# KarypisLab/SLIM

Hardware: AMD Instinct MI355X
Metric: item-columns solved/sec (whole node) (higher is better)
Workload: dtype f32

## Files before the change

slim_amd/csrc/cd_gramr.hpp:

```cpp
#pragma once
#include <utility>

#include "cd_tile.hpp"
#include "gram_pack.hpp"

#ifndef SLIM_GRAMR_AUX
#define SLIM_GRAMR_AUX 0
#endif
#ifndef SLIM_GRAMR_PROF
#define SLIM_GRAMR_PROF 0
#endif
#ifndef SLIM_GRAMR_FROM_PLANES
#define SLIM_GRAMR_FROM_PLANES 1
#endif
#ifndef SLIM_GRAMR_PREFETCH
#define SLIM_GRAMR_PREFETCH 0
#endif
#ifndef SLIM_GRAMR_LATE_GATHERS
#define SLIM_GRAMR_LATE_GATHERS 1
#endif
#ifndef SLIM_GRAMR_DRAIN
#define SLIM_GRAMR_DRAIN 0
#endif
#ifndef SLIM_GRAMR_SYNCROW
#define SLIM_GRAMR_SYNCROW 0
#endif

namespace slimamd {

typedef float gramr_v16 __attribute__((ext_vector_type(16)));

template <int N>
struct GramrRegs {
  gramr_v16 v;
  GramrRegs<N - 1> rest;
};
template <>
struct GramrRegs<0> {};
template <int I, int N>
__device__ __forceinline__ gramr_v16& gramr_reg(GramrRegs<N>& r) {
  if constexpr (I == 0) return r.v;
  else return gramr_reg<I - 1>(r.rest);
}
template <class F, int... Is>
__device__ __forceinline__ void static_for_impl(F&& f, std::integer_sequence<int, Is...>) {
  (f(std::integral_constant<int, Is>{}), ...);
}
template <int N, class F>
__device__ __forceinline__ void static_for(F&& f) {
  static_for_impl(f, std::make_integer_sequence<int, N>{});
}

template <int N, int KRA>
__device__ __forceinline__ float gramr_sel_from(GramrRegs<KRA>& gr, const int k, const int e) {
  if (k == N) {
    const gramr_v16 t = gramr_reg<N>(gr);
    asm volatile("" ::"v"(t));
    return t[e];
  }
  if constexpr (N + 1 < KRA) return gramr_sel_from<N + 1, KRA>(gr, k, e);
  return 0.0f;
}
template <int KRA>
__device__ __forceinline__ float gramr_sel(GramrRegs<KRA>& gr, const int k, const int e) {
  return gramr_sel_from<0, KRA>(gr, k, e);
}

#ifndef SLIM_GRAMR_ASMEXPORT
#define SLIM_GRAMR_ASMEXPORT 1
#endif
#define SLIM_GRAMR_EXPORT_ASM                                   \
  "s_mov_b32 %[sm0], m0\n\t"                                   \
  "s_mov_b64 %[sx], exec\n"                                     \
  "1:\n\t"                                                      \
  "s_ff1_i32_b64 %[sb], %[mine]\n\t"                            \
  "v_readlane_b32 %[sr], %[r], %[sb]\n\t"                       \
  "s_bitset0_b64 %[mine], %[sb]\n\t"                            \
  "s_bfe_u32 %[sl], %[sr], 0x60004\n\t"                         \
  "s_lshr_b32 %[sidx], %[sr], 13\n\t"                           \
  "s_and_b32 %[sr], %[sr], 15\n\t"                              \
  "s_lshl4_add_u32 %[sidx], %[sidx], %[sr]\n\t"                 \
  "s_set_gpr_idx_on %[sidx], gpr_idx(SRC0)\n\t"                 \
  "v_mov_b32 %[vt], v16\n\t"                                    \
  "s_set_gpr_idx_off\n\t"                                       \
  "v_readlane_b32 %[sv], %[vt], %[sl]\n\t"                      \
  "s_lshl_b64 exec, 1, %[sb]\n\t"                               \
  "v_mov_b32 %[res], %[sv]\n\t"                                 \
  "s_mov_b64 exec, %[sx]\n\t"                                   \
  "s_cmp_lg_u64 %[mine], 0\n\t"                                 \
  "s_cbranch_scc1 1b\n\t"                                       \
  "s_mov_b32 m0, %[sm0]\n"
#define SLIM_GRAMR_EXPORT_OUT                                                                           \
  [res] "+v"(res), [mine] "+s"(mine), [sb] "=&s"(sb), [sr] "=&s"(sr), [sl] "=&s"(sl), [sidx] "=&s"(sidx), \
      [sv] "=&s"(sv), [vt] "=&v"(vt), [sm0] "=&s"(sm0), [sx] "=&s"(sx)
template <int KRA>
__device__ __forceinline__ float gramr_export(GramrRegs<KRA>& gr, const int r, uint64_t mine) {
  float res = 0.0f, vt;
  int sb, sr, sl, sidx, sm0;
  float sv;
  uint64_t sx;
  static_assert(KRA == 1 || KRA == 3 || KRA == 6 || KRA == 10, "one operand list per instantiation");
  if constexpr (KRA == 1) {
    asm volatile(SLIM_GRAMR_EXPORT_ASM : SLIM_GRAMR_EXPORT_OUT : [r] "v"(r), "{v[16:31]}"(gramr_reg<0>(gr)) : "scc");
  } else if constexpr (KRA == 3) {
    asm volatile(SLIM_GRAMR_EXPORT_ASM
                 : SLIM_GRAMR_EXPORT_OUT
                 : [r] "v"(r), "{v[16:31]}"(gramr_reg<0>(gr)), "{v[32:47]}"(gramr_reg<1>(gr)),
                   "{v[48:63]}"(gramr_reg<2>(gr))
                 : "scc");
  } else if constexpr (KRA == 6) {
    asm volatile(SLIM_GRAMR_EXPORT_ASM
                 : SLIM_GRAMR_EXPORT_OUT
                 : [r] "v"(r), "{v[16:31]}"(gramr_reg<0>(gr)), "{v[32:47]}"(gramr_reg<1>(gr)),
                   "{v[48:63]}"(gramr_reg<2>(gr)), "{v[64:79]}"(gramr_reg<3>(gr)), "{v[80:95]}"(gramr_reg<4>(gr)),
                   "{v[96:111]}"(gramr_reg<5>(gr))
                 : "scc");
  } else {
    asm volatile(SLIM_GRAMR_EXPORT_ASM
                 : SLIM_GRAMR_EXPORT_OUT
                 : [r] "v"(r), "{v[16:31]}"(gramr_reg<0>(gr)), "{v[32:47]}"(gramr_reg<1>(gr)),
                   "{v[48:63]}"(gramr_reg<2>(gr)), "{v[64:79]}"(gramr_reg<3>(gr)), "{v[80:95]}"(gramr_reg<4>(gr)),
                   "{v[96:111]}"(gramr_reg<5>(gr)), "{v[112:127]}"(gramr_reg<6>(gr)),
                   "{v[128:143]}"(gramr_reg<7>(gr)), "{v[144:159]}"(gramr_reg<8>(gr)),
                   "{v[160:175]}"(gramr_reg<9>(gr))
                 : "scc");
  }
  return res;
}

constexpr int gramr_ring_bytes(int ah) { return (kGramrNT / 64) * (ah + 2) * 1024; }
constexpr int kGramrHdr = 1280;
constexpr int kGramrDump = SLIM_GRAMR_PREFETCH ? 256 : 0;
constexpr int gramr_hdr_bytes() { return (kGramrNT / 64) * (2 * kGramrHdr + kGramrDump); }

template <int KR, int KL, bool DMA = false, int WPS = ((KR <= 2 && KL == 0) ? 4 : 2), int AH = 2>
__global__ __launch_bounds__(kGramrNT, WPS) void cd_gramr_kernel(
    const DevMatrix A, const SolveArgs S, const GramPacked P) {
  constexpr int NT = kGramrNT, K = KR + KL;
  constexpr int kGramrAhead = AH, kGramrSlots = AH + 2;
  constexpr int KRA = KR > 0 ? KR : 1;
  constexpr int R0 = KR * kPackGroup;
  static_assert(KR <= 12, "register select covers 12 groups");
  static_assert(KR + KL <= 16, "one base byte per group in a 16-byte load");
  extern __shared__ __attribute__((aligned(16))) float g_lds[];
  __shared__ float s_gB[2][64];
  __shared__ int s_p, s_na;
  __shared__ unsigned long long s_D;
  __shared__ double s_e2[64], s_reg[64];
  __shared__ unsigned long long s_off;
  __shared__ int s_nz;

  const int tid = threadIdx.x;
  const int lane = tid & 63;
  const int wave = uni(tid >> 6);
  const int ncols = A.ncols;
#if !SLIM_GRAMR_FROM_PLANES
  const int n4 = S.ncols_pad >> 2;
#endif
  const int nchunks = P.nchunks;
  const float l1 = S.l1, l2 = S.l2;
#if !SLIM_GRAMR_FROM_PLANES
  const float* __restrict__ Gm = S.G;
  const int64_t ld = S.G_ld;
#endif
  float* const x = S.xslab + (int64_t)blockIdx.x * S.x_stride;
#if !SLIM_GRAMR_FROM_PLANES
  float4* const x4 = reinterpret_cast<float4*>(x);
#endif
  float4* const gl4 = reinterpret_cast<float4*>(g_lds);
  const int64_t* __restrict__ colptr = A.colptr;

  GramrRegs<KRA> gr;

  const uint32_t voff0 = 16u * (uint32_t)tid;
  const uint32_t vlast = 16u * (uint32_t)(nchunks - 1);
#if SLIM_GRAMR_DRAIN
#define SLIM_VMCNT(n) __builtin_amdgcn_s_waitcnt(0 | (7 << 4) | (15 << 8))
#else
#define SLIM_VMCNT(n) __builtin_amdgcn_s_waitcnt(((n) & 15) | (((n) >> 4) << 14) | (7 << 4) | (15 << 8))
#endif
  char* const ring_w = reinterpret_cast<char*>(g_lds) + KL * kPackGroup * 4 + wave * (kGramrSlots * 1024);
#if SLIM_GRAMR_PROF
  unsigned long long pt_first_v = 0, pt_mark_v = 0, pt_export_v = 0, pt_mark = 0;
  unsigned long long* const pt_first_p = &pt_first_v;
  unsigned long long* const pt_mark_p = &pt_mark_v;
#endif
  char* const hdr_w = reinterpret_cast<char*>(g_lds) + KL * kPackGroup * 4 + (DMA ? gramr_ring_bytes(AH) : 0) +
                      wave * (2 * kGramrHdr + kGramrDump);
  char* const dump_w = hdr_w + 2 * kGramrHdr;
  auto apply = [&](const uint8_t* __restrict__ plo, const uint8_t* __restrict__ phi,
                   const uint8_t* __restrict__ ph2, const uint8_t* __restrict__ pbase, const int hk,
                   const int h2k, const int cdiag, const int ediag, const float vdiag,
                   const float nd, const int rg, uint32_t (&gq)[4],
                   const uint8_t* __restrict__ plo_next) __attribute__((always_inline)) {
    const bool gin1 = rg < hk * kPackGroup, gin2 = rg < h2k * kPackGroup;
    auto gathers = [&]() __attribute__((always_inline)) {
      gq[0] = __hip_atomic_load(plo + rg, __ATOMIC_RELAXED, __HIP_MEMORY_SCOPE_WAVEFRONT);
      gq[1] = __hip_atomic_load(phi + (gin1 ? rg : 0), __ATOMIC_RELAXED, __HIP_MEMORY_SCOPE_WAVEFRONT);
      gq[2] = __hip_atomic_load(ph2 + (gin2 ? rg : 0), __ATOMIC_RELAXED, __HIP_MEMORY_SCOPE_WAVEFRONT);
      gq[3] = __hip_atomic_load(pbase + (((rg >> 4) & (NT - 1)) * 16 + (rg >> 13)), __ATOMIC_RELAXED,
                                __HIP_MEMORY_SCOPE_WAVEFRONT);
    };
    if constexpr (!(DMA && SLIM_GRAMR_LATE_GATHERS)) gathers();
    const int kdiag = cdiag / NT, tdiag = cdiag % NT;
    uint32_t bwords[4];
    if constexpr (DMA) {
      uint32_t vzb = voff0;
      asm volatile("" : "+v"(vzb));
      __builtin_amdgcn_global_load_lds(pbase + vzb, ring_w + (kGramrAhead + 1) * 1024, 16, 0, 0);
    } else {
      const uint4 bw = ld_off<uint4>(pbase, voff0);
      bwords[0] = bw.x;
      bwords[1] = bw.y;
      bwords[2] = bw.z;
      bwords[3] = bw.w;
    }
    auto consume = [&](auto kc, const uint4 lo, auto&& hi_of) __attribute__((always_inline)) {
      constexpr int k = decltype(kc)::value;
      float f[16];
      unpack16(lo, f);
      {
        typedef float gramr_v2 __attribute__((ext_vector_type(2)));
        const float bf = 16.0f * (float)((bwords[(k >> 2) & 3] >> (8 * (k & 3))) & 255u);
#pragma unroll
        for (int e = 0; e < 16; e += 2) {
          gramr_v2 v = {f[e], f[e + 1]};
          asm volatile("" : "+v"(v));
          v += (gramr_v2)(bf);
          f[e] = v.x;
          f[e + 1] = v.y;
        }
      }
      if (k < hk) {
        unpack16_add(hi_of(), 256.0f, f);
        if (k < h2k) {
          uint32_t vz = voff0;
          asm volatile("" : "+v"(vz));
          const uint32_t vo = min(vz + (uint32_t)(kPackGroup * k), vlast);
          unpack16_add(ld_off<uint4>(ph2, vo), 65536.0f, f);
        }
      }
      if (k == kdiag && tid == tdiag) {
#pragma unroll
        for (int e = 0; e < 16; ++e) f[e] = e == ediag ? vdiag : f[e];
      }
      if constexpr (k < KR) {
        gramr_v16& g = gramr_reg<k>(gr);
#pragma unroll
        for (int e = 0; e < 16; ++e) g[e] = fmaf(nd, f[e], g[e]);
        asm volatile("" : "+v"(g));
      } else {
        float4* const gp = gl4 + (k - KR) * 4 * NT + tid;
#pragma unroll
        for (int j = 0; j < 4; ++j) {
          float4 v = gp[j * NT];
          v.x = fmaf(nd, f[4 * j + 0], v.x);
          v.y = fmaf(nd, f[4 * j + 1], v.y);
          v.z = fmaf(nd, f[4 * j + 2], v.z);
          v.w = fmaf(nd, f[4 * j + 3], v.w);
          gp[j * NT] = v;
        }
      }
    };
    if constexpr (DMA) {
      constexpr int S = kGramrAhead + 1;
      uint4 h01[2];
      static_for<2>([&](auto kc) __attribute__((always_inline)) {
        constexpr int k = decltype(kc)::value;
        if constexpr (k < K) {
          if (k < hk) h01[k] = ld_off<uint4>(phi, min(voff0 + (uint32_t)(kPackGroup * k), vlast));
        }
      });
      auto request = [&](auto kc) __attribute__((always_inline)) {
        constexpr int k = decltype(kc)::value;
        uint32_t vz = voff0;
        asm volatile("" : "+v"(vz));
        const uint32_t vo = min(vz + (uint32_t)(kPackGroup * k), vlast);
        __builtin_amdgcn_global_load_lds(plo + vo, ring_w + (k % S) * 1024, 16, 0, SLIM_GRAMR_AUX);
      };
      static_for<(kGramrAhead < K ? kGramrAhead : K)>([&](auto kc) __attribute__((always_inline)) { request(kc); });
      constexpr int kLate = (SLIM_GRAMR_LATE_GATHERS ? 4 : 0) + (SLIM_GRAMR_PREFETCH ? 1 : 0);
      if constexpr (SLIM_GRAMR_LATE_GATHERS) gathers();
      if constexpr (SLIM_GRAMR_PREFETCH) {
        const int ln = lane < 8 * kGramrAhead ? lane : 0;
        const uint32_t po = min((uint32_t)(kPackGroup * (ln >> 3)) + 1024u * (uint32_t)wave + 128u * (uint32_t)(ln & 7), vlast);
        __builtin_amdgcn_global_load_lds(plo_next + po, dump_w, 4, 0, 0);
      }
      static_for<K>([&](auto kc) __attribute__((always_inline)) {
        constexpr int k = decltype(kc)::value;
        if constexpr (k + kGramrAhead < K) request(std::integral_constant<int, k + kGramrAhead>{});
        constexpr int ahead = (K - 1 - k) < kGramrAhead ? (K - 1 - k) : kGramrAhead;
        SLIM_VMCNT(ahead + (k < kGramrAhead ? kLate : 0));
        asm volatile("" ::: "memory");
        if constexpr (k == 0) {
          const uint4 bw = *reinterpret_cast<const uint4*>(ring_w + (kGramrAhead + 1) * 1024 + lane * 16);
          bwords[0] = bw.x;
          bwords[1] = bw.y;
          bwords[2] = bw.z;
          bwords[3] = bw.w;
        }
#if SLIM_GRAMR_PROF
        if constexpr (k == 0) *pt_first_p += __builtin_readcyclecounter() - *pt_mark_p;
#endif
        const uint4 lo = *reinterpret_cast<const uint4*>(ring_w + (k % S) * 1024 + lane * 16);
        consume(kc, lo, [&]() __attribute__((always_inline)) -> uint4 {
          if constexpr (k < 2) return h01[k];
          else {
            uint32_t vz = voff0;
            asm volatile("" : "+v"(vz));
            return ld_off<uint4>(phi, min(vz + (uint32_t)(kPackGroup * k), vlast));
          }
        });
        __builtin_amdgcn_sched_barrier(0);
      });
    } else {
      constexpr int GRP = 4;
      static_for<(K + GRP - 1) / GRP>([&](auto k0c) __attribute__((always_inline)) {
        constexpr int k0 = decltype(k0c)::value * GRP;
        uint4 l[GRP], h[GRP];
        static_for<GRP>([&](auto uc) __attribute__((always_inline)) {
          constexpr int u = decltype(uc)::value, k = k0 + u;
          if constexpr (k < K) {
            const uint32_t vo = min(voff0 + (uint32_t)(kPackGroup * k), vlast);
            l[u] = ld_off<uint4>(plo, vo);
            if (k < hk) h[u] = ld_off<uint4>(phi, vo);
          }
        });
        __builtin_amdgcn_sched_barrier(0);
        static_for<GRP>([&](auto uc) __attribute__((always_inline)) {
          constexpr int u = decltype(uc)::value, k = k0 + u;
          if constexpr (k < K)
            consume(std::integral_constant<int, k>{}, l[u], [&]() __attribute__((always_inline)) -> uint4 { return h[u]; });
          __builtin_amdgcn_sched_barrier(0);
        });
      });
    }
  };
#undef SLIM_VMCNT
  int nrows_read = 0, nhi16_read = 0;
  auto lds_index = [&](const int r) __attribute__((always_inline)) -> int {
    const int rr = r - R0;
    const int kk = rr >> 13, t = (rr >> 4) & (NT - 1), e = rr & 15;
    return ((kk * 4 + (e >> 2)) * NT + t) * 4 + (e & 3);
  };

  int gb_par = 0;
  auto fetch_g = [&](const bool want, const int r) __attribute__((always_inline)) -> float {
    float* const gb = s_gB[gb_par];
    gb_par ^= 1;
    const bool in_lds = r >= R0;
    const bool my_wave = (((r >> 4) & (NT - 1)) >> 6) == wave;
    if (KR > 0) {
      uint64_t mine = __ballot(want && !in_lds && my_wave);
#if SLIM_GRAMR_ASMEXPORT
      if (mine) {
        const bool own = want && !in_lds && my_wave;
        const float res = gramr_export<KRA>(gr, r, mine);
        if (own) gb[lane] = res;
      }
#else
      while (mine) {
        const int b = __builtin_ctzll(mine);
        mine &= mine - 1ull;
        const int rb = lane_bcast(r, b);
        const float v = gramr_sel<KRA>(gr, rb >> 13, rb & 15);
        if (lane == ((rb >> 4) & 63)) gb[b] = v;
      }
#endif
    }
    if (KL > 0 && want && in_lds && my_wave) gb[lane] = g_lds[lds_index(r)];
#if SLIM_GRAMR_PROF
    pt_export_v += __builtin_readcyclecounter() - pt_mark;
#endif
    asm volatile("" ::: "memory");
    __builtin_amdgcn_s_waitcnt(15 | (7 << 4) | (0 << 8) | (3 << 14));
    __builtin_amdgcn_s_barrier();
    asm volatile("" ::: "memory");
    return gb[lane];
  };

  for (;;) {
    if (tid == 0) {
      s_p = atomicAdd(S.queue, 1);
      s_na = 0;
      s_D = 0;
    }
    __syncthreads();
    const int p = s_p;
    if (p >= S.nwork) break;
    const int item = uni(S.order[p]);
    const int grp = p >> 5;
    const uint32_t gkey = (uint32_t)(grp * S.shard_count + S.shard_index);
    const int* __restrict__ ul = S.ulist + (int64_t)grp * S.u_stride;
    const int nunion = uni(S.tile_nunion[grp]);
#if SLIM_GRAMR_FROM_PLANES
    uint4 irec;
    {
      const uint4 mr = P.meta[item];
      irec = make_uint4(uni(mr.x), uni(mr.y), uni(mr.z), uni(mr.w));
    }
#endif
#if !SLIM_GRAMR_FROM_PLANES
    const float* __restrict__ arow = Gm + (int64_t)item * ld;
#endif

#if SLIM_GRAMR_FROM_PLANES
    {
      const int hk0 = (int)((irec.x >> 17) & 15u), h2k0 = (int)((irec.x >> 21) & 15u);
      const uint8_t* __restrict__ plo0 = P.lo + (int64_t)item * P.ldb;
      const uint8_t* __restrict__ phi0 = P.hi + (int64_t)irec.y * kPackGroup;
      const uint8_t* __restrict__ ph20 = phi0 + (int64_t)hk0 * kPackGroup;
      const uint8_t* __restrict__ pb0 = P.base + (int64_t)item * kPackGroup;
      int na = 0;
      int64_t dact = 0;
      for (int c = tid; c < nchunks; c += NT) {
        const int kg = c / NT;
        float f[16];
        unpack16(*reinterpret_cast<const uint4*>(plo0 + 16 * (int64_t)c), f);
        const float bf = 16.0f * (float)pb0[(c & (NT - 1)) * 16 + kg];
#pragma unroll
        for (int e = 0; e < 16; ++e) f[e] += bf;
        if (kg < hk0) unpack16_add(*reinterpret_cast<const uint4*>(phi0 + 16 * (int64_t)c), 256.0f, f);
        if (kg < h2k0) unpack16_add(*reinterpret_cast<const uint4*>(ph20 + 16 * (int64_t)c), 65536.0f, f);
        const int4* __restrict__ io = reinterpret_cast<const int4*>(P.item_of + 16 * (int64_t)c);
#pragma unroll
        for (int j = 0; j < 4; ++j) {
          const int4 q = io[j];
          const int it[4] = {q.x, q.y, q.z, q.w};
#pragma unroll
          for (int u = 0; u < 4; ++u) {
            if (it[u] >= 0) {
              const bool act = it[u] != item && f[4 * j + u] > l1;
              x[it[u]] = act ? 0.0f : kInactive;
              if (act) {
                ++na;
                dact += (int64_t)P.meta[it[u]].z;
              }
            }
          }
        }
      }
      na = (int)wave_sum((float)na);
      if (lane == 0 && na) atomicAdd(&s_na, na);
      if (dact) atomicAdd(&s_D, (unsigned long long)dact);
    }
#else
    {
      const float4* __restrict__ a4 = reinterpret_cast<const float4*>(arow);
      int na = 0;
      int64_t dact = 0;
      for (int c = tid; c < n4; c += NT) {
        const float4 a = a4[c];
        const int i0 = c << 2;
        float4 xs;
        const bool a0 = i0 + 0 < ncols && i0 + 0 != item && a.x > l1;
        const bool a1 = i0 + 1 < ncols && i0 + 1 != item && a.y > l1;
        const bool a2 = i0 + 2 < ncols && i0 + 2 != item && a.z > l1;
        const bool a3 = i0 + 3 < ncols && i0 + 3 != item && a.w > l1;
        xs.x = a0 ? 0.0f : kInactive;
        xs.y = a1 ? 0.0f : kInactive;
        xs.z = a2 ? 0.0f : kInactive;
        xs.w = a3 ? 0.0f : kInactive;
        na += (int)a0 + (int)a1 + (int)a2 + (int)a3;
        x4[c] = xs;
        if (a0 | a1 | a2 | a3) {
          const int64_t c0 = colptr[i0], c1 = colptr[i0 + 1];
          const int64_t c2 = i0 + 2 <= ncols ? colptr[i0 + 2] : c1, c3 = i0 + 3 <= ncols ? colptr[i0 + 3] : c2;
          const int64_t c4 = i0 + 4 <= ncols ? colptr[i0 + 4] : c3;
          dact += (a0 ? c1 - c0 : 0) + (a1 ? c2 - c1 : 0) + (a2 ? c3 - c2 : 0) + (a3 ? c4 - c3 : 0);
        }
      }
      na = (int)wave_sum((float)na);
      if (lane == 0 && na) atomicAdd(&s_na, na);
      if (dact) atomicAdd(&s_D, (unsigned long long)dact);
    }
#endif
    int64_t fe = 0, we = 0;
    auto warm_x = [&]() __attribute__((always_inline)) {
      if (S.icolptr != nullptr && item < S.incols) {
        __syncthreads();
        fe = uni(S.icolptr[item]);
        we = uni(S.icolptr[item + 1]);
        for (int64_t e = fe + tid; e < we; e += NT) {
          const int k = S.icolind[e];
          if (k < ncols && tile_active(x[k])) {
            const float v = S.icolval[e];
            x[k] = v < 0.0f ? 0.0f : v;
          }
        }
      }
    };
    warm_x();
    constexpr bool kCarry = K <= kGramrCarryMaxGroups;
    const bool carried = kCarry && S.g_load != nullptr;
    if (carried) {
      const float4* __restrict__ gs = reinterpret_cast<const float4*>(S.g_load + (int64_t)item * S.g_stride);
      static_for<KRA>([&](auto kc) __attribute__((always_inline)) {
        constexpr int k = decltype(kc)::value;
        gramr_v16 v;
#pragma unroll
        for (int j = 0; j < 4; ++j) {
          const float4 q = gs[(k * NT + tid) * 4 + j];
          v[4 * j] = q.x; v[4 * j + 1] = q.y; v[4 * j + 2] = q.z; v[4 * j + 3] = q.w;
        }
        gramr_reg<k>(gr) = v;
      });
#pragma unroll
      for (int k = 0; k < KL; ++k)
#pragma unroll
        for (int j = 0; j < 4; ++j) gl4[(k * 4 + j) * NT + tid] = gs[((KRA + k) * NT + tid) * 4 + j];
    } else {
    static_for<KRA>([&](auto kc) __attribute__((always_inline)) {
      gramr_reg<decltype(kc)::value>(gr) = (gramr_v16)(0.0f);
    });
#pragma unroll
    for (int k = 0; k < KL; ++k)
#pragma unroll
      for (int j = 0; j < 4; ++j) gl4[(k * 4 + j) * NT + tid] = make_float4(0.f, 0.f, 0.f, 0.f);
    }
    __syncthreads();

    int maxit = 0;
    {
      const int64_t cap = 50 * (uni(colptr[item + 1]) - uni(colptr[item]));
      maxit = cap < (int64_t)S.maxniters ? (int)cap : S.maxniters;
    }
    int niters = 0, conv = 0;
    nrows_read = 0;
    nhi16_read = 0;

    if (wave == 0) {
      s_e2[lane] = 0.0;
      s_reg[lane] = 0.0;
    }
    int phase = 0;
    bool init_row = !carried;
    if (carried) fe = we;
    int t = 0, p0 = 0;
    float dlt = 0.0f;
    PermCtx pc = perm_make(1u, 0u);
    int i_a = 0;
    int i_n = 0;
    int hw = 0;
    auto header_a = [&](const int q0) __attribute__((always_inline)) {
      const int pos = q0 + lane;
      i_a = pos < nunion ? ul[perm_index(pc, (uint32_t)pos)] : -1;
    };
    auto header_b = [&]() __attribute__((always_inline)) {
      i_n = i_a < 0 ? 0 : i_a;
      char* const hb = hdr_w + hw * kGramrHdr;
      __builtin_amdgcn_global_load_lds(x + i_n, hb, 4, 0, 0);
      __builtin_amdgcn_global_load_lds(P.meta + i_n, hb + 256, 16, 0, 0);
      hw ^= 1;
    };
    int ib = 0, wpos = 0, nz = 0;
    unsigned long long off = 0;
    bool fits = false;
    unsigned long long Uu = 0;
#if SLIM_GRAMR_PROF
    unsigned long long pt_fetch = 0, pt_dec = 0, pt_apply = 0;
    pt_first_v = 0;
    pt_export_v = 0;
#define SLIM_PT(acc) { const unsigned long long now_ = __builtin_readcyclecounter(); acc += now_ - pt_mark; pt_mark = now_; }
#else
#define SLIM_PT(acc)
#endif

    for (;;) {
      bool want = false;
      int r = 0, i = 0;
      uint4 mrow = make_uint4(0u, 0u, 0u, 0u);
      float xi = kInactive;
      bool part = false, keep = false;
      uint64_t mkeep = 0;
      if (phase == 1) {
        i = i_n;
        __builtin_amdgcn_s_waitcnt(0 | (7 << 4) | (15 << 8));
        asm volatile("" ::: "memory");
        {
          const char* const hcur = hdr_w + (hw ^ 1) * kGramrHdr;
          const bool valid = p0 + lane < nunion;
          int lz = lane;
          asm volatile("" : "+v"(lz));
          const float xv = *reinterpret_cast<const float*>(hcur + lz * 4);
          mrow = *reinterpret_cast<const uint4*>(hcur + 256 + lz * 16);
          r = (int)(mrow.x & 0x1FFFFu);
          xi = valid ? xv : kInactive;
        }
        asm volatile("" ::: "memory");
        part = tile_active(xi);
        header_b();
        header_a(p0 + 128);
        want = part;
      } else if (phase == 2) {
        i = ib + lane;
        xi = i < ncols ? x[i] : kInactive;
        const bool act = tile_active(xi);
        keep = act && fabsf(xi) > kEps;
        if (act && wave == 0)
          s_reg[lane] += 0.5 * (double)l2 * (double)xi * (double)xi + (double)l1 * (double)fabsf(xi);
        mkeep = __ballot(keep);
        if (mkeep == 0) {
          ib += 64;
          if (ib >= ncols) break;
          continue;
        }
        r = keep ? (int)(P.meta[i].x & 0x1FFFFu) : 0;
        want = keep;
      }
#if SLIM_GRAMR_PROF
      pt_mark = __builtin_readcyclecounter();
#endif
      const float g0 = fetch_g(want, r);
      SLIM_PT(pt_fetch)
      float gi = g0;
      uint64_t pend = 0;
      if (phase == 1) {
        pend = __ballot(part);
      }
      for (;;) {
        int row = 0;
        float nd = 0.0f;
        uint4 rec = make_uint4(0u, 0u, 0u, 0u);
        if (phase == 0) {
          bool have = false;
          if (init_row) {
            row = item;
            nd = 1.0f;
            have = true;
          } else {
            while (fe < we) {
              const int kk = uni(S.icolind[fe]);
              ++fe;
              if (kk < ncols) {
                const float xk = uni(x[kk]);
                if (xk > kEps) {
                  row = kk;
                  nd = -xk;
                  have = true;
                  break;
                }
              }
            }
          }
          if (!have) break;
        } else if (phase == 1) {
          if (pend == 0) break;
          const float xeff = (xi > kEps || xi < -kEps) ? xi : 0.0f;
          const float sq = __uint_as_float(mrow.w);
          const float cn = sqrtf(sq);
          const float num = cd_num(gi, xeff, sq);
          const float nx = num > l1 ? (num - l1) / cd_den(cn, l2) : 0.0f;
          const float neff = (nx > kEps || nx < -kEps) ? nx : 0.0f;
          const float d = neff - xeff;
          const uint64_t m = __ballot(part && nx != xi) & pend;
          if (m == 0) break;
          const int f = __builtin_ctzll(m);
          const float d_f = lane_bcast(d, f);
          const float nx_f = lane_bcast(nx, f), xi_f = lane_bcast(xi, f);
          dlt = fmaf(nx_f - xi_f, nx_f - xi_f, dlt);
          row = lane_bcast(i, f);
          if (wave == 0 && lane == f) x[row] = nx;
          pend = f == 63 ? 0ull : (pend & ~((2ull << f) - 1ull));
          if (d_f == 0.0f) continue;
          nd = -d_f;
          rec.x = (uint32_t)lane_bcast((int)mrow.x, f);
          rec.y = (uint32_t)lane_bcast((int)mrow.y, f);
          rec.z = (uint32_t)lane_bcast((int)mrow.z, f);
          rec.w = (uint32_t)lane_bcast((int)mrow.w, f);
          Uu += (unsigned long long)rec.z;
        } else {
          break;
        }
        if (phase == 0) {
          const uint4 mr = P.meta[row];
          rec.x = uni(mr.x);
          rec.y = uni(mr.y);
          rec.z = uni(mr.z);
          rec.w = uni(mr.w);
        }
        const int hk = (int)((rec.x >> 17) & 15u), h2k = (int)((rec.x >> 21) & 15u);
        const uint8_t* __restrict__ plo = P.lo + (int64_t)row * P.ldb;
        const uint8_t* __restrict__ phi = P.hi + (int64_t)rec.y * kPackGroup;
        const uint8_t* __restrict__ ph2 = phi + (int64_t)hk * kPackGroup;
        const uint8_t* __restrict__ pbase = P.base + (int64_t)row * kPackGroup;
        const bool in1 = r < hk * kPackGroup, in2 = r < h2k * kPackGroup;
        uint32_t gq[4];
        const int rdiag = (int)(rec.x & 0x1FFFFu);
        SLIM_PT(pt_dec)
#if SLIM_GRAMR_PROF
        pt_mark_v = pt_mark;
#endif
        const uint8_t* __restrict__ plo_next = plo;
        if (SLIM_GRAMR_PREFETCH && phase == 1) {
          const uint64_t cand = __ballot(part && xi != 0.0f) & pend;
          if (cand) plo_next = P.lo + (int64_t)lane_bcast(i, __builtin_ctzll(cand)) * P.ldb;
        }
        apply(plo, phi, ph2, pbase, hk, h2k, rdiag >> 4, rdiag & 15, __uint_as_float(rec.w), nd, r, gq, plo_next);
        float gsel = (float)gq[0] + 16.0f * (float)gq[3];
        gsel = in1 ? fmaf(256.0f, (float)gq[1], gsel) : gsel;
        gsel = in2 ? fmaf(65536.0f, (float)gq[2], gsel) : gsel;
        if (init_row) {
          init_row = false;
        } else {
          ++nrows_read;
          nhi16_read += min(hk * (kPackGroup / 16), nchunks) + min(h2k * (kPackGroup / 16), nchunks);
        }
        gi = fmaf(nd, gsel, gi);
#if SLIM_GRAMR_SYNCROW
        __syncthreads();
#endif
        SLIM_PT(pt_apply)
      }
      if (phase == 1) {
        p0 += 64;
        if (p0 < nunion) continue;
        if (dlt < S.opt_tol) {
          conv = 1;
          niters = t + 1;
        } else {
          ++t;
        }
      } else if (phase == 2) {
        if (keep) {
#if SLIM_GRAMR_FROM_PLANES
          float aty = 0.0f;
          if (wave == 0) {
            const int hk0 = (int)((irec.x >> 17) & 15u), h2k0 = (int)((irec.x >> 21) & 15u);
            const uint8_t* __restrict__ plo0 = P.lo + (int64_t)item * P.ldb;
            const uint8_t* __restrict__ phi0 = P.hi + (int64_t)irec.y * kPackGroup;
            const uint8_t* __restrict__ ph20 = phi0 + (int64_t)hk0 * kPackGroup;
            const uint8_t* __restrict__ pb0 = P.base + (int64_t)item * kPackGroup;
            const bool j1 = r < hk0 * kPackGroup, j2 = r < h2k0 * kPackGroup;
            aty = (float)plo0[r] + 16.0f * (float)pb0[((r >> 4) & (NT - 1)) * 16 + (r >> 13)];
            if (j1) aty = fmaf(256.0f, (float)phi0[r], aty);
            if (j2) aty = fmaf(65536.0f, (float)ph20[r], aty);
          }
          if (wave == 0) s_e2[lane] += (double)xi * ((double)aty + (double)g0);
#else
          if (wave == 0) s_e2[lane] += (double)xi * ((double)arow[i] + (double)g0);
#endif
          if (fits && wave == 0) {
            const int64_t dst = (int64_t)off + wpos + __popcll(mkeep & ((1ull << lane) - 1ull));
            S.out_ind[dst] = i;
            S.out_val[dst] = xi;
          }
        }
        wpos += __popcll(mkeep);
        ib += 64;
        if (ib >= ncols) break;
        continue;
      }
      bool sweep = false;
      if (!conv) {
        if (t >= maxit) {
          niters = maxit + 1;
        } else if (nunion == 0) {
          conv = 1;
          niters = t + 1;
        } else {
          sweep = true;
        }
      }
      if (sweep) {
        __syncthreads();
        phase = 1;
        p0 = 0;
        dlt = 0.0f;
        pc = perm_make((uint32_t)nunion, perm_key(S.seed, gkey, (uint32_t)t));
        header_a(0);
        header_b();
        header_a(64);
        continue;
      }
      if (wave == 0) {
        int cnt = 0;
        for (int jb = 0; jb < ncols; jb += 64) {
          const int j = jb + lane;
          const float xv = j < ncols ? x[j] : kInactive;
          cnt += __popcll(__ballot(tile_active(xv) && fabsf(xv) > kEps));
        }
        if (lane == 0) {
          s_off = atomicAdd(S.out_cursor, (unsigned long long)cnt);
          s_nz = cnt;
        }
      }
      __syncthreads();
      off = s_off;
      nz = s_nz;
      fits = (int64_t)(off + (unsigned long long)nz) <= S.out_cap;
      phase = 2;
      ib = 0;
      wpos = 0;
      if (ncols <= 0) break;
    }
    if (kCarry && S.g_save != nullptr) {
      float4* __restrict__ gs = reinterpret_cast<float4*>(S.g_save + (int64_t)item * S.g_stride);
      static_for<KRA>([&](auto kc) __attribute__((always_inline)) {
        constexpr int k = decltype(kc)::value;
        const gramr_v16 v = gramr_reg<k>(gr);
#pragma unroll
        for (int j = 0; j < 4; ++j)
          gs[(k * NT + tid) * 4 + j] = make_float4(v[4 * j], v[4 * j + 1], v[4 * j + 2], v[4 * j + 3]);
      });
#pragma unroll
      for (int k = 0; k < KL; ++k)
#pragma unroll
        for (int j = 0; j < 4; ++j) gs[((KRA + k) * NT + tid) * 4 + j] = gl4[(k * 4 + j) * NT + tid];
    }
    if (wave == 0) {
      double e2 = s_e2[lane], reg = s_reg[lane];
      for (int o = 32; o > 0; o >>= 1) {
        e2 += __shfl_xor(e2, o);
        reg += __shfl_xor(reg, o);
      }
      if (lane == 0) {
        const float err = (float)(0.5 * ((double)A.csq[item] - e2));
        if (!fits) atomicMax(S.overflow, 1);
        S.out_cnt[item] = fits ? nz : -nz - 1;
        S.out_off[item] = (int64_t)off;
        S.st_na[item] = s_na;
        S.st_sweeps[item] = niters;
        S.st_conv[item] = conv;
#if SLIM_GRAMR_PROF
        S.st_D[item] = (int64_t)pt_fetch;
        S.st_U[item] = (int64_t)pt_dec;
        S.st_B[item] = (int64_t)pt_apply;
        S.st_G[item] = (int)(pt_first_v >> 8);
        S.st_na[item] = (int)(pt_export_v >> 8);
#else
        S.st_D[item] = (int64_t)s_D * (int64_t)(conv ? niters : maxit);
        S.st_U[item] = (int64_t)Uu;
        S.st_G[item] = nrows_read;
        S.st_B[item] = (int64_t)nrows_read * (P.ldb + 16 * (int64_t)(nchunks < NT ? nchunks : NT)) + (int64_t)nhi16_read * 16 +
                       ((carried ? 4 : 0) + (kCarry && S.g_save != nullptr ? 4 : 0)) * S.g_stride;
#endif
        S.st_err[item] = err;
        S.st_obj[item] = err + (float)reg;
      }
    }
    __syncthreads();
  }
}

constexpr int kGramrUnionNT = 256;
#ifdef SLIM_GRAM_PACK_KERNELS
__global__ __launch_bounds__(kGramrUnionNT) void gramr_union_kernel(const DevMatrix A, const SolveArgs S,
                                                                     const GramPacked P) {
  constexpr int NT = kGramrUnionNT;
  constexpr int kWords = kGramrMaxGroups * kPackGroup / 32;
  __shared__ uint32_t s_bits[kWords];
  __shared__ int s_scan[NT];
  const int tid = threadIdx.x;
  const int grp = blockIdx.x;
  const int base = grp * 32;
  const int nprob = (S.nwork - base) < 32 ? (S.nwork - base) : 32;
  const int ncols = A.ncols;
  const int nwords = (ncols + 31) >> 5;
  const int nchunks = P.nchunks;
  int* __restrict__ ul = S.ulist + (int64_t)grp * S.u_stride;
  for (int w = tid; w < nwords; w += NT) s_bits[w] = 0u;
  __syncthreads();
  for (int q = 0; q < nprob; ++q) {
    const int it0 = uni(S.order[base + q]);
    const uint4 mr = P.meta[it0];
    const uint32_t rx = uni(mr.x), ry = uni(mr.y);
    const int hk = (int)((rx >> 17) & 15u), h2k = (int)((rx >> 21) & 15u);
    const uint8_t* __restrict__ plo = P.lo + (int64_t)it0 * P.ldb;
    const uint8_t* __restrict__ phi = P.hi + (int64_t)ry * kPackGroup;
    const uint8_t* __restrict__ ph2 = phi + (int64_t)hk * kPackGroup;
    const uint8_t* __restrict__ pb = P.base + (int64_t)it0 * kPackGroup;
    for (int c = tid; c < nchunks; c += NT) {
      const int kg = c / kGramrNT;
      float f[16];
      unpack16(*reinterpret_cast<const uint4*>(plo + 16 * (int64_t)c), f);
      const float bf = 16.0f * (float)pb[(c & (kGramrNT - 1)) * 16 + kg];
#pragma unroll
      for (int e = 0; e < 16; ++e) f[e] += bf;
      if (kg < hk) unpack16_add(*reinterpret_cast<const uint4*>(phi + 16 * (int64_t)c), 256.0f, f);
      if (kg < h2k) unpack16_add(*reinterpret_cast<const uint4*>(ph2 + 16 * (int64_t)c), 65536.0f, f);
      const int4* __restrict__ io = reinterpret_cast<const int4*>(P.item_of + 16 * (int64_t)c);
#pragma unroll
      for (int j = 0; j < 4; ++j) {
        const int4 qv = io[j];
        const int it[4] = {qv.x, qv.y, qv.z, qv.w};
#pragma unroll
        for (int u = 0; u < 4; ++u)
          if (it[u] >= 0 && it[u] != it0 && f[4 * j + u] > S.l1) atomicOr(&s_bits[it[u] >> 5], 1u << (it[u] & 31));
      }
    }
  }
  __syncthreads();
  const int W = (nwords + NT - 1) / NT;
  const int w0 = tid * W, w1 = min(nwords, w0 + W);
  int cnt = 0;
  for (int w = w0; w < w1; ++w) cnt += __popc(s_bits[w]);
  s_scan[tid] = cnt;
  __syncthreads();
  for (int o = 1; o < NT; o <<= 1) {
    const int v = tid >= o ? s_scan[tid - o] : 0;
    __syncthreads();
    s_scan[tid] += v;
    __syncthreads();
  }
  int pos = s_scan[tid] - cnt;
  for (int w = w0; w < w1; ++w) {
    uint32_t b = s_bits[w];
    while (b) {
      const int j = __builtin_ctz(b);
      b &= b - 1u;
      ul[pos++] = (w << 5) + j;
    }
  }
  if (tid == NT - 1) S.tile_nunion[grp] = s_scan[tid];
}
#endif

}
```

slim_amd/csrc/cd_wave.hpp:

```cpp
#pragma once
#include <hip/hip_runtime.h>

#include <cstdint>

#include "cd_perm.hpp"

namespace slimamd {

struct DevMatrix {
  int32_t nrows, ncols;
  int64_t nnz;
  const int64_t* rowptr;
  const int32_t* rowind;
  const float* rowval;
  const int64_t* colptr;
  const int32_t* colind;
  const float* colval;
  const float* cnorm;
  const float* csq;
};

struct SolveArgs {
  float l1, l2, opt_tol;
  int32_t maxniters;
  uint32_t seed;
  int32_t nnbrs;
  int32_t simtype;
  const int32_t* order;
  int32_t nwork;
  int32_t* queue;
  const int64_t* icolptr;
  const int32_t* icolind;
  const float* icolval;
  int32_t incols;
  float* slab;
  int64_t slab_stride;
  int32_t nrows_pad, ncols_pad;
  float* xslab;
  int64_t x_stride;
  int32_t* ulist;
  int64_t u_stride;
  int32_t ngroups;
  uint64_t* trace;
  int32_t cluster;
  const int32_t* ubounds;
  const int64_t* csplit;
  unsigned long long* mailbox;
  float* atypart;
  int32_t exact_gram;
  int32_t bm_shift, bm_words;
  int32_t nheavy;
  int32_t cluster_hi;
  const int32_t* ubounds_hi;
  const int64_t* csplit_hi;
  unsigned long long* mailbox_hi;
  int32_t* queue_hi;
  int64_t nnz_last;
  int32_t hi_prefetch;
  int32_t shard_count, shard_index;
  int32_t xcd_swizzle;
  float* gram;
  int32_t gram_mode;
  float* G;
  int64_t G_ld;
  int32_t* tile_nunion;
  const int32_t* gram_pos;
  int32_t gram_bits;
  int32_t gram_split_stride;
  int32_t gram_accum;
  const uint4* gview;
  const int64_t* gview_base;
  const uint16_t* gview_cnt;
  int32_t gview_ngroups;
  int32_t gview_range0;
  int32_t gview_sentinel;
  int32_t gram_part16;
  int32_t gram_store;
  int32_t gram_read;
  float* g_save;
  const float* g_load;
  int64_t g_stride;
  int32_t* out_cnt;
  int64_t* out_off;
  int32_t* out_ind;
  float* out_val;
  unsigned long long* out_cursor;
  int64_t out_cap;
  int32_t* overflow;
  int32_t* st_na;
  int32_t* st_sweeps;
  int32_t* st_conv;
  int64_t* st_G;
  int64_t* st_D;
  int64_t* st_U;
  int64_t* st_B;
  float* st_err;
  float* st_obj;
};

constexpr float kEps = 1e-7f;


__device__ __forceinline__ float cd_num(float g, float xeff, float sq) {
  float p = xeff * sq;
  asm volatile("" : "+v"(p));
  return g + p;
}
__device__ __forceinline__ float cd_den(float cn, float l2) { return fmaf(cn, cn, l2); }
__device__ __forceinline__ int uni(int v) { return __builtin_amdgcn_readfirstlane(v); }
__device__ __forceinline__ uint32_t uni(uint32_t v) {
  return (uint32_t)__builtin_amdgcn_readfirstlane((int)v);
}
__device__ __forceinline__ float uni(float v) {
  return __int_as_float(__builtin_amdgcn_readfirstlane(__float_as_int(v)));
}
__device__ __forceinline__ int64_t uni(int64_t v) {
  uint32_t lo = uni((uint32_t)v), hi = uni((uint32_t)((uint64_t)v >> 32));
  return (int64_t)(((uint64_t)hi << 32) | lo);
}
__device__ __forceinline__ int lane_bcast(int v, int src) {
  return __builtin_amdgcn_readlane(v, src);
}
__device__ __forceinline__ float lane_bcast(float v, int src) {
  return __int_as_float(__builtin_amdgcn_readlane(__float_as_int(v), src));
}
__device__ __forceinline__ int64_t lane_bcast(int64_t v, int src) {
  uint32_t lo = (uint32_t)__builtin_amdgcn_readlane((int)(uint32_t)v, src);
  uint32_t hi = (uint32_t)__builtin_amdgcn_readlane((int)(uint32_t)((uint64_t)v >> 32), src);
  return (int64_t)(((uint64_t)hi << 32) | lo);
}

template <int CTRL>
__device__ __forceinline__ float dpp_mov(float v) {
  return __int_as_float(
      __builtin_amdgcn_update_dpp(0, __float_as_int(v), CTRL, 0xF, 0xF, true));
}

__device__ __forceinline__ float wave_sum(float v) {
  v += dpp_mov<0xB1>(v);
  v += dpp_mov<0x4E>(v);
  v += dpp_mov<0x141>(v);
  v += dpp_mov<0x140>(v);
  return (lane_bcast(v, 0) + lane_bcast(v, 16)) + (lane_bcast(v, 32) + lane_bcast(v, 48));
}

template <bool USE_LDS>
__device__ __forceinline__ void wave_sync() {
  if (USE_LDS) {
    __builtin_amdgcn_fence(__ATOMIC_ACQ_REL, "wavefront");
    __builtin_amdgcn_wave_barrier();
  } else {
    __builtin_amdgcn_fence(__ATOMIC_ACQ_REL, "workgroup");
    __builtin_amdgcn_wave_barrier();
  }
}


template <bool USE_LDS, bool HAS_VAL>
__global__ __launch_bounds__(64) void cd_wave_kernel(const DevMatrix A, const SolveArgs S) {
  extern __shared__ __attribute__((aligned(16))) char smem[];
  const int lane = threadIdx.x;
  const uint64_t lane_lt = (1ull << lane) - 1ull;

  float* r;
  float* aty;
  float* x;
  if (USE_LDS) {
    r = reinterpret_cast<float*>(smem);
  } else {
    r = S.slab + (int64_t)blockIdx.x * S.slab_stride;
  }
  aty = r + S.nrows_pad;
  x = aty + S.ncols_pad;
  int* ids = reinterpret_cast<int*>(aty);

  const int nrows = A.nrows, ncols = A.ncols;
  const float l1 = S.l1, l2 = S.l2;

  for (;;) {
    int w = 0;
    if (lane == 0) w = atomicAdd(S.queue, 1);
    w = uni(w);
    if (w >= S.nwork) break;
    const int iC = uni(S.order[w]);
    const int64_t cs = uni(A.colptr[iC]), ce = uni(A.colptr[iC + 1]);

    for (int u = lane; u < nrows; u += 64) r[u] = 0.0f;
    for (int i = lane; i < ncols; i += 64) aty[i] = 0.0f;
    wave_sync<USE_LDS>();

    int64_t G = 0;
    if (S.exact_gram) {
      for (int64_t j = cs + lane; j < ce; j += 64) {
        const int u = A.colind[j];
        r[u] = HAS_VAL ? A.colval[j] : 1.0f;
        G += A.rowptr[u + 1] - A.rowptr[u];
      }
      for (int off = 32; off > 0; off >>= 1) G += __shfl_xor(G, off);
      wave_sync<USE_LDS>();
      for (int ib = 0; ib < ncols; ib += 64) {
        const int i = ib + lane;
        float acc = 0.0f;
        if (i < ncols) {
          const int64_t s = A.colptr[i], e = A.colptr[i + 1];
          bool co = false;
          for (int64_t k = s; k < e; ++k) {
            const float yv = r[A.colind[k]];
            acc += (HAS_VAL ? A.colval[k] : 1.0f) * yv;
            co = co || yv != 0.0f;
          }
          aty[i] = (acc == 0.0f && co) ? -0.0f : acc;
        }
      }
    } else {
    for (int64_t jb = cs; jb < ce; jb += 64) {
      const int64_t j = jb + lane;
      const bool ok = j < ce;
      const int u_l = ok ? A.colind[j] : 0;
      const float v_l = ok ? (HAS_VAL ? A.colval[j] : 1.0f) : 0.0f;
      const int64_t rs_l = ok ? A.rowptr[u_l] : 0;
      const int64_t re_l = ok ? A.rowptr[u_l + 1] : 0;
      if (ok) r[u_l] = v_l;
      const int cnt = (int)((ce - jb) < 64 ? (ce - jb) : 64);
      for (int k = 0; k < cnt; ++k) {
        const int64_t rs = lane_bcast(rs_l, k), re = lane_bcast(re_l, k);
        const float v = lane_bcast(v_l, k);
        G += re - rs;
        for (int64_t e = rs + lane; e < re; e += 64) {
          const float rv = HAS_VAL ? A.rowval[e] : 1.0f;
          atomicAdd(&aty[A.rowind[e]], v * rv);
        }
      }
    }
    }
    wave_sync<USE_LDS>();

    int na = 0;
    if (S.nnbrs > 0) {
      const float ninf = -__builtin_huge_valf();
      const float cn_c = A.cnorm[iC];
      for (int i = lane; i < ncols; i += 64) {
        const float a = aty[i];
        float sim = ninf;
        if ((a != 0.0f || __builtin_signbit(a)) && i != iC) {
          const float cn_i = A.cnorm[i];
          sim = S.simtype == 0 ? a / cn_i : (S.simtype == 1 ? a / ((cn_i + cn_c) - a) : a);
        }
        aty[i] = sim;
      }
      wave_sync<USE_LDS>();
      int* sel = reinterpret_cast<int*>(x);
      for (int round = 0; round < S.nnbrs; ++round) {
        float bs = ninf;
        int bi = 0x7fffffff;
        for (int i = lane; i < ncols; i += 64) {
          const float sv = aty[i];
          if (sv > bs) {
            bs = sv;
            bi = i;
          }
        }
#pragma unroll
        for (int off = 32; off > 0; off >>= 1) {
          const float os = __shfl_xor(bs, off);
          const int oi = __shfl_xor(bi, off);
          const bool take = os > bs || (os == bs && oi < bi);
          bs = take ? os : bs;
          bi = take ? oi : bi;
        }
        bs = uni(bs);
        bi = uni(bi);
        if (!(bs > ninf)) break;
        if (lane == 0) {
          sel[na] = bi;
          aty[bi] = ninf;
        }
        ++na;
        wave_sync<USE_LDS>();
      }
      int myid = 0, rank = 0;
      for (int b = 0; b < na; b += 64) {
        const int e = b + lane;
        myid = e < na ? sel[e] : 0;
        rank = 0;
        for (int o = 0; o < na; ++o) rank += (sel[o] < myid) ? 1 : 0;
        wave_sync<USE_LDS>();
        if (e < na) ids[rank] = myid;
      }
      wave_sync<USE_LDS>();
      for (int e = lane; e < na; e += 64) x[e] = 0.0f;
    } else
    for (int base = 0; base < ncols; base += 64) {
      const int i = base + lane;
      const float a = i < ncols ? aty[i] : 0.0f;
      const bool act = (i < ncols) && (i != iC) && (a > l1);
      const uint64_t m = __ballot(act);
      wave_sync<USE_LDS>();
      if (act) {
        const int slot = na + __popcll(m & lane_lt);
        ids[slot] = i;
        x[slot] = 0.0f;
      }
      na += __popcll(m);
    }
    wave_sync<USE_LDS>();

    if (S.nnbrs == 0 && S.icolptr != nullptr && iC < S.incols) {
      const int64_t ws = uni(S.icolptr[iC]), we = uni(S.icolptr[iC + 1]);
      for (int64_t e = ws + lane; e < we; e += 64) {
        const int k = S.icolind[e];
        int lo = 0, hi = na;
        while (lo < hi) {
          const int mid = (lo + hi) >> 1;
          if (ids[mid] < k) lo = mid + 1; else hi = mid;
        }
        if (lo < na && ids[lo] == k) x[lo] = fmaxf(S.icolval[e], 0.0f);
      }
      wave_sync<USE_LDS>();
      for (int q = 0; q < na; ++q) {
        const float xi = uni(x[q]);
        if (xi > kEps || xi < -kEps) {
          const int i = uni(ids[q]);
          const int64_t s = uni(A.colptr[i]), t = uni(A.colptr[i + 1]);
          for (int64_t e = s + lane; e < t; e += 64)
            r[A.colind[e]] -= xi * (HAS_VAL ? A.colval[e] : 1.0f);
          wave_sync<USE_LDS>();
        }
      }
    }

    const int64_t cap = 50 * (ce - cs);
    const int maxit = cap < (int64_t)S.maxniters ? (int)cap : S.maxniters;
    int t = 0, conv = 0;
    int64_t D = 0, U = 0;
    for (; t < maxit; ++t) {
      float dlt = 0.0f;
      const PermCtx pc = perm_make((uint32_t)na, perm_key(S.seed, (uint32_t)iC, (uint32_t)t));
      struct StageB { int64_t s, e; float cn, sq; };
      auto stage_a = [&](const int pp, int& q, int& i, float& xv) {
        q = (int)perm_index(pc, (uint32_t)pp);
        i = ids[q];
        xv = x[q];
      };
      auto stage_b = [&](const int i) -> StageB {
        StageB b;
        b.s = A.colptr[i];
        b.e = A.colptr[i + 1];
        b.cn = A.cnorm[i];
        b.sq = A.csq[i];
        return b;
      };
      int qa = 0, ia = 0, qb = 0, ib = 0, qc = 0, ic = 0;
      float xa = 0.f, xb = 0.f, xc = 0.f;
      StageB ba = {0, 0, 0.f, 0.f}, bb = {0, 0, 0.f, 0.f};
      int u0 = 0, u1 = 0;
      float v0 = 0.f, v1 = 0.f;
      auto stage_c = [&](const int64_t s, const int64_t e_end) {
        const int64_t k0 = s + lane, k1 = k0 + 64;
        u0 = k0 < e_end ? A.colind[k0] : 0;
        v0 = k0 < e_end ? (HAS_VAL ? A.colval[k0] : 1.0f) : 0.0f;
        u1 = k1 < e_end ? A.colind[k1] : 0;
        v1 = k1 < e_end ? (HAS_VAL ? A.colval[k1] : 1.0f) : 0.0f;
      };
      if (na > 0) {
        stage_a(0, qa, ia, xa);
        ba = stage_b(uni(ia));
        if (na > 1) {
          stage_a(1, qb, ib, xb);
          bb = stage_b(uni(ib));
        }
        if (na > 2) stage_a(2, qc, ic, xc);
        stage_c(uni(ba.s), uni(ba.e));
      }
      for (int p = 0; p < na; ++p) {
        const int q = uni(qa);
        const float xi = uni(xa);
        const int64_t s = uni(ba.s), e_end = uni(ba.e);
        const float cn = uni(ba.cn), sq = uni(ba.sq);
        const int cu0 = u0, cu1 = u1;
        const float cv0 = v0, cv1 = v1;
        qa = qb; ia = ib; xa = xb; ba = bb;
        qb = qc; ib = ic; xb = xc;
        if (p + 1 < na) stage_c(uni(ba.s), uni(ba.e));
        if (p + 2 < na) bb = stage_b(uni(ib));
        if (p + 3 < na) stage_a(p + 3, qc, ic, xc);

        float acc = cv0 * r[cu0] + cv1 * r[cu1];
        for (int64_t e = s + 128 + lane; e < e_end; e += 64) {
          const float v = HAS_VAL ? A.colval[e] : 1.0f;
          acc += v * r[A.colind[e]];
        }
        const float dot = wave_sum(acc);

        const float xeff = (xi > kEps || xi < -kEps) ? xi : 0.0f;
        const float num = dot + xeff * sq;
        const float nx = num > l1 ? (num - l1) / (cn * cn + l2) : 0.0f;
        const float neff = (nx > kEps || nx < -kEps) ? nx : 0.0f;
        const float d = neff - xeff;
        D += e_end - s;
        if (d != 0.0f) {
// ... 72 lines not shown
```

slim_amd/csrc/engine.hip:

```cpp
#include <hip/hip_runtime.h>

#include <algorithm>
#include <atomic>
#include <chrono>
#include <cmath>
#include <cstdio>
#include <cstdlib>
#include <cstring>
#include <functional>
#include <mutex>
#include <new>
#include <numeric>
#include <memory>
#include <string>
#include <thread>

#include <rocprim/device/device_radix_sort.hpp>

#include "tile_inst.hpp"
#include "gram_inst.hpp"
#include "gramr_inst.hpp"
#include "gram_sym.hpp"
#include "fslim_gram_inst.hpp"
#include "cd_wave.hpp"
#include "engine.hpp"
#include "hip_check.hpp"
#include "host_csr.hpp"

inline uint64_t slimgpu_next_uid() {
  static std::atomic<uint64_t> n{0};
  return ++n;
}

using slimamd::DeviceBuffer;

struct UserSplit {
  DeviceBuffer<int32_t> ubounds;
  DeviceBuffer<int64_t> csplit;
  int32_t nranges = 0, max_rows = 0;
};

struct slimgpu_matrix {
  const uint64_t uid = slimgpu_next_uid();
  int device = 0;
  hipStream_t stream = nullptr;
  int32_t nrows = 0, ncols = 0;
  int64_t nnz = 0;
  bool binary = false;
  bool owns_csr = false;
  bool exact_gram = false;
  bool nonpositive = false;
  bool merged = false;
  int64_t* d_rowptr = nullptr;
  int32_t* d_rowind = nullptr;
  float* d_rowval = nullptr;
  DeviceBuffer<int64_t> d_colptr;
  DeviceBuffer<int32_t> d_colind;
  DeviceBuffer<float> d_colval, d_cnorm, d_csq;
  std::vector<int64_t> h_cost;
  std::vector<int64_t> h_rowptr;
  UserSplit split[6];
  UserSplit gsplit;
  double setup_ms = 0;
  int num_cus = 256;
  std::vector<slimgpu_matrix*> replicas;
  DeviceBuffer<float> ws_gram;
  std::vector<int32_t> gram_order;
  int gram_geom[6] = {0, 0, 0, 0, 0, 0};
  DeviceBuffer<float> ws_G;
  DeviceBuffer<int32_t> ws_nunion;
  int64_t G_ld = 0;
  bool G_ready = false;
  double G_build_ms = 0, G_alloc_ms = 0, G_sums_ms = 0, G_sums_kernel_ms = 0, G_pack_ms = 0;
  DeviceBuffer<uint8_t> ws_Glo, ws_Ghi, ws_Gbase;
  DeviceBuffer<float> ws_Gdiag;
  DeviceBuffer<uint4> ws_Gmeta;
  DeviceBuffer<int64_t> ws_hioff, ws_hi2off;
  DeviceBuffer<int32_t> ws_hik, ws_hi2k, ws_rankof, ws_itemof;
  int64_t Gp_ldb = 0, Gp_pool_bytes = 0;
  int32_t Gp_nchunks = 0;
  bool Gp_ready = false, Gp_tried = false;
  bool Gf_dropped = false;
  double Gp_bytes_per_row = 0;
  int expect_solves = 0;
  std::vector<int32_t> last_order;
  DeviceBuffer<int32_t> ws_order, ws_cnt, ws_stat_i, ws_misc, ws_arena_i, ws_ulist;
  DeviceBuffer<int64_t> ws_off, ws_stat_l, ws_icolptr;
  DeviceBuffer<float> ws_stat_f, ws_arena_v, ws_slab, ws_xslab, ws_part, ws_icolval;
  DeviceBuffer<int32_t> ws_fn, ws_fid, ws_fslot;
  DeviceBuffer<float> ws_faty;
  DeviceBuffer<uint64_t> ws_trace;
  DeviceBuffer<uint4> ws_gview;
  DeviceBuffer<int64_t> ws_gvbase;
  DeviceBuffer<int32_t> ws_gvrows;
  DeviceBuffer<uint16_t> ws_gvcnt;
  DeviceBuffer<unsigned long long> ws_mailbox;
  DeviceBuffer<int32_t> ws_icolind;
  DeviceBuffer<uint32_t> ws_tkeys[2];
  DeviceBuffer<uint64_t> ws_tpay[2];
  DeviceBuffer<uint8_t> ws_ttmp;

  ~slimgpu_matrix() {
    (void)hipSetDevice(device);
    if (owns_csr) {
      (void)hipFree(d_rowptr);
      (void)hipFree(d_rowind);
      (void)hipFree(d_rowval);
    }
  }
};

struct slimgpu_model {
  int device = 0;
  int32_t n = 0;
  int64_t nnz = 0;
  int32_t max_row = 0;
  bool rows_sorted = true;
  DeviceBuffer<int64_t> d_colptr, d_rowptr;
  DeviceBuffer<int32_t> d_colind, d_rowind;
  DeviceBuffer<float> d_colval, d_rowval;
  mutable DeviceBuffer<float> d_gsave;
  mutable bool gsave_valid = false;
  int64_t gsave_stride = 0;
  double gsave_l1 = 0;
  uint64_t gsave_owner = 0;
  std::thread fetcher;
  bool fetch_begun = false;
  slim_csr_t* fetched = nullptr;
  int32_t fetch_status = 0;
  std::string fetch_error;
  double fetch_ms = 0;

  ~slimgpu_model() { (void)hipSetDevice(device); }
};

namespace slimamd {

namespace {

thread_local slimgpu_stats_t g_stats;
thread_local ColumnStats g_colstats;

struct InputError {
  std::string msg;
};

double now_ms() {
  using namespace std::chrono;
  return duration<double, std::milli>(steady_clock::now().time_since_epoch()).count();
}

void report(const HipFail& e, const char* what) {
  set_error(std::string(what) + ": HIP error '" + hipGetErrorString(e.code) + "' in " + e.where +
            " -- the SLIM CD path needs a gfx950 GPU; there is no CPU fallback");
}

void drop_screen_cache(slimgpu_matrix* m) {
  m->ws_gram.reset();
  m->gram_order.clear();
}

auto evict_cache(slimgpu_matrix* m) {
  return [m] {
    if (!m->ws_gram.get()) return false;
    drop_screen_cache(m);
    return true;
  };
}


__global__ void k_gview_rows(const int32_t* __restrict__ order, int32_t nwork, const int64_t* __restrict__ csplit,
                             int32_t stride, int32_t ngroups, int32_t nblocks, int32_t* __restrict__ rows,
                             uint16_t* __restrict__ cnt) {
  const int b = (int)blockIdx.x * ((int)blockDim.x >> 6) + ((int)threadIdx.x >> 6);
  if (b >= nblocks) return;
  const int r = b / ngroups, pl = (b % ngroups) * 64 + ((int)threadIdx.x & 63);
  int len = 0;
  if (pl < nwork) {
    const int64_t* const c = csplit + (int64_t)order[pl] * stride + r;
    len = (int)(c[1] - c[0]);
  }
  int n = (len + 7) >> 3;
  cnt[(int64_t)b * 64 + (threadIdx.x & 63)] = (uint16_t)n;
  for (int off = 32; off > 0; off >>= 1) n += __shfl_xor(n, off);
  if ((threadIdx.x & 63) == 0) rows[b] = n;
}

__global__ void k_gview_fill(const int32_t* __restrict__ order, int32_t nwork, const int64_t* __restrict__ csplit,
                             int32_t stride, const int32_t* __restrict__ ubounds, const int32_t* __restrict__ ci,
                             int32_t ngroups, int32_t nblocks, const int64_t* __restrict__ base, uint32_t sentinel,
                             uint4* __restrict__ view) {
  const int b = (int)blockIdx.x * ((int)blockDim.x >> 6) + ((int)threadIdx.x >> 6);
  if (b >= nblocks) return;
  const int lane = (int)threadIdx.x & 63;
  const int r = b / ngroups, pl = (b % ngroups) * 64 + lane;
  const int64_t end = base[b + 1];
  const int32_t u0 = ubounds[r];
  int64_t cs = 0;
  int len = 0;
  if (pl < nwork) {
    const int64_t* const c = csplit + (int64_t)order[pl] * stride + r;
    cs = c[0];
    len = (int)(c[1] - cs);
  }
  int64_t at = base[b];
  for (int c = 0;; ++c) {
    const bool mine = 8 * c < len;
    const uint64_t who = __ballot(mine);
    if (who == 0ull) break;
    if (mine) {
      const int64_t slot = at + __popcll(who & ((1ull << lane) - 1ull));
      uint32_t id[8];
#pragma unroll
      for (int j = 0; j < 8; ++j) id[j] = 8 * c + j < len ? (uint32_t)(ci[cs + 8 * c + j] - u0) : sentinel;
      if (slot < end)
        view[slot] = make_uint4(id[0] | (id[1] << 16), id[2] | (id[3] << 16), id[4] | (id[5] << 16),
                                id[6] | (id[7] << 16));
    }
    at += __popcll(who);
  }
}


__global__ void k_max_index(const int32_t* __restrict__ ind, int64_t n, int32_t* out) {
  int32_t m = -1;
  for (int64_t k = (int64_t)blockIdx.x * blockDim.x + threadIdx.x; k < n;
       k += (int64_t)gridDim.x * blockDim.x)
    m = max(m, ind[k]);
  for (int off = 32; off > 0; off >>= 1) m = max(m, __shfl_xor(m, off));
  if ((threadIdx.x & 63) == 0) atomicMax(out, m);
}

constexpr int kBadRowptr = 1;
constexpr int kBadColumn = 2;
constexpr int kDupEntry = 4;

__global__ void k_pack_rows(int32_t nrows, int32_t ncols, int64_t nnz,
                            const int64_t* __restrict__ rowptr,
                            const int32_t* __restrict__ rowind,
                            const float* __restrict__ rowval, uint32_t* __restrict__ keys,
                            uint64_t* __restrict__ payload, int32_t* __restrict__ flags) {
  const int lane = threadIdx.x & 63;
  const int64_t wave = ((int64_t)blockIdx.x * blockDim.x + threadIdx.x) >> 6;
  const int64_t nwaves = ((int64_t)gridDim.x * blockDim.x) >> 6;
  for (int64_t u = wave; u < nrows; u += nwaves) {
    int64_t s = rowptr[u], e = rowptr[u + 1];
    if (s < 0 || e < s || e > nnz || (u == 0 && s != 0)) {
      if (lane == 0) atomicOr(flags, kBadRowptr);
      continue;
    }
    for (int64_t k = s + lane; k < e; k += 64) {
      if ((uint32_t)rowind[k] >= (uint32_t)ncols) atomicOr(flags, kBadColumn);
      keys[k] = (uint32_t)rowind[k];
      const uint32_t bits = rowval ? __float_as_uint(rowval[k]) : 0x3F800000u;
      payload[k] = ((uint64_t)(uint32_t)u << 32) | bits;
    }
  }
}

__global__ void k_unpack_cols(int64_t nnz, const uint64_t* __restrict__ payload,
                              int32_t* __restrict__ colind, float* __restrict__ colval) {
  for (int64_t k = (int64_t)blockIdx.x * blockDim.x + threadIdx.x; k < nnz;
       k += (int64_t)gridDim.x * blockDim.x) {
    const uint64_t p = payload[k];
    colind[k] = (int32_t)(p >> 32);
    if (colval) colval[k] = __uint_as_float((uint32_t)p);
  }
}

__global__ void k_check_dups(int64_t nnz, const uint32_t* __restrict__ keys,
                             const uint64_t* __restrict__ payload, int32_t* __restrict__ flags) {
  for (int64_t k = (int64_t)blockIdx.x * blockDim.x + threadIdx.x + 1; k < nnz;
       k += (int64_t)gridDim.x * blockDim.x)
    if (keys[k] == keys[k - 1] && (payload[k] >> 32) == (payload[k - 1] >> 32))
      atomicOr(flags, kDupEntry);
}

__global__ void k_col_offsets(int64_t nnz, int32_t ncols, const uint32_t* __restrict__ keys,
                              int64_t* __restrict__ colptr) {
  for (int64_t k = (int64_t)blockIdx.x * blockDim.x + threadIdx.x; k <= nnz;
       k += (int64_t)gridDim.x * blockDim.x) {
    const int64_t lo = k == 0 ? 0 : (int64_t)keys[k - 1] + 1;
    const int64_t hi = k == nnz ? (int64_t)ncols : (int64_t)keys[k];
    for (int64_t c = lo; c <= hi; ++c) colptr[c] = k;
  }
}

__global__ void k_col_scalars(int32_t ncols, const int64_t* __restrict__ colptr,
                              const int32_t* __restrict__ colind,
                              const float* __restrict__ colval,
                              const int64_t* __restrict__ rowptr, float* __restrict__ csq,
                              float* __restrict__ cnorm, int64_t* __restrict__ cost,
                              int32_t* __restrict__ inexact) {
  const int lane = threadIdx.x & 63;
  const int64_t wave = ((int64_t)blockIdx.x * blockDim.x + threadIdx.x) >> 6;
  const int64_t nwaves = ((int64_t)gridDim.x * blockDim.x) >> 6;
  for (int64_t c = wave; c < ncols; c += nwaves) {
    const int64_t s = colptr[c], e = colptr[c + 1];
    float ss = 0.0f;
    int64_t g = 0;
    for (int64_t k = s + lane; k < e; k += 64) {
      const float v = colval ? colval[k] : 1.0f;
      ss += v * v;
      if (v != rintf(v) || fabsf(v) > 2048.0f) atomicOr(inexact, 1);
      if (!(v > 0.0f)) atomicOr(inexact, 2);
      const int32_t u = colind[k];
      g += rowptr[u + 1] - rowptr[u];
    }
    for (int off = 32; off > 0; off >>= 1) {
      ss += __shfl_xor(ss, off);
      g += __shfl_xor(g, off);
    }
    if (lane == 0) {
      if (!colval) ss = (float)(e - s);
      if (!(ss < 16777216.0f)) atomicOr(inexact, 1);
      csq[c] = ss;
      cnorm[c] = sqrtf(ss);
      cost[c] = g;
    }
  }
}

__global__ void k_col_split(int32_t ncols, int32_t K, const int32_t* __restrict__ ubounds,
                            const int64_t* __restrict__ colptr,
                            const int32_t* __restrict__ colind, int64_t* __restrict__ csplit) {
  const int64_t n = (int64_t)ncols * (K + 1);
  for (int64_t t = (int64_t)blockIdx.x * blockDim.x + threadIdx.x; t < n;
       t += (int64_t)gridDim.x * blockDim.x) {
    const int32_t c = (int32_t)(t / (K + 1)), j = (int32_t)(t % (K + 1));
    int64_t lo = colptr[c], hi = colptr[c + 1];
    if (j == K) {
      lo = hi;
    } else if (j > 0) {
      const int32_t ub = ubounds[j];
      while (lo < hi) {
        const int64_t mid = (lo + hi) >> 1;
        if (colind[mid] < ub) lo = mid + 1; else hi = mid;
      }
    }
    csplit[t] = lo;
  }
}

__global__ void k_gather_columns(int32_t ncols, const int64_t* __restrict__ colptr,
                                 const int64_t* __restrict__ src_off, const int32_t* __restrict__ src_ind,
                                 const float* __restrict__ src_val, int32_t* __restrict__ colind,
                                 float* __restrict__ colval) {
  const int lane = threadIdx.x & 63;
  const int64_t wave = ((int64_t)blockIdx.x * blockDim.x + threadIdx.x) >> 6;
  const int64_t nwaves = ((int64_t)gridDim.x * blockDim.x) >> 6;
  for (int64_t c = wave; c < ncols; c += nwaves) {
    const int64_t d = colptr[c], n = colptr[c + 1] - d, s = src_off[c];
    for (int64_t k = lane; k < n; k += 64) {
      colind[d + k] = src_ind[s + k];
      colval[d + k] = src_val[s + k];
    }
  }
}


int grid_for(int64_t n, int block, int cap_blocks) {
  int64_t g = (n + block - 1) / block;
  if (g < 1) g = 1;
  if (g > cap_blocks) g = cap_blocks;
  return (int)g;
}

void pick_device(slimgpu_matrix* m, const LearnOptions& opt) {
  (void)hipGetLastError();
  int count = 0;
  HIP_TRY(hipGetDeviceCount(&count));
  if (count <= 0) throw HipFail{hipErrorNoDevice, "hipGetDeviceCount"};
  if (opt.device >= 0) {
    HIP_TRY(hipSetDevice(opt.device));
    m->device = opt.device;
  } else {
    HIP_TRY(hipGetDevice(&m->device));
  }
  hipDeviceProp_t prop;
  HIP_TRY(hipGetDeviceProperties(&prop, m->device));
  m->num_cus = prop.multiProcessorCount > 0 ? prop.multiProcessorCount : 256;
  HIP_TRY(hipStreamCreateWithFlags(&m->stream, hipStreamNonBlocking));
}

struct SortBufs {
  uint32_t *keys_in, *keys_out;
  uint64_t *pay_in, *pay_out;
};

void pack_entries(slimgpu_matrix* m, int32_t n, int32_t ncols, int64_t nnz, const int64_t* ptr,
                  const int32_t* ind, const float* val, const SortBufs& b, int32_t* flags) {
  hipLaunchKernelGGL(k_pack_rows, dim3(grid_for((int64_t)n * 64, 256, m->num_cus * 16)), dim3(256), 0,
                     m->stream, n, ncols, nnz, ptr, ind, val, b.keys_in, b.pay_in, flags);
  HIP_TRY(hipGetLastError());
}

template <class TmpFor>
void sort_entries(slimgpu_matrix* m, int32_t ncols, int64_t nnz, const SortBufs& b, TmpFor&& tmp_for,
                  int32_t* dups, int64_t* o_ptr, int32_t* o_ind, float* o_val) {
  hipStream_t st = m->stream;
  const int cap = m->num_cus * 16;
  unsigned bits = 1;
  while ((1ull << bits) < (unsigned long long)ncols) ++bits;
  size_t tmp_bytes = 0;
  HIP_TRY(rocprim::radix_sort_pairs(nullptr, tmp_bytes, b.keys_in, b.keys_out, b.pay_in, b.pay_out,
                                    (size_t)nnz, 0u, bits, st));
  void* tmp = tmp_for(tmp_bytes ? tmp_bytes : 1);
  HIP_TRY(rocprim::radix_sort_pairs(tmp, tmp_bytes, b.keys_in, b.keys_out, b.pay_in, b.pay_out,
                                    (size_t)nnz, 0u, bits, st));
  if (dups) {
    hipLaunchKernelGGL(k_check_dups, dim3(grid_for(nnz, 256, cap)), dim3(256), 0, st, nnz,
                       b.keys_out, b.pay_out, dups);
    HIP_TRY(hipGetLastError());
  }
  hipLaunchKernelGGL(k_unpack_cols, dim3(grid_for(nnz, 256, cap)), dim3(256), 0, st, nnz,
                     b.pay_out, o_ind, o_val);
  HIP_TRY(hipGetLastError());
  hipLaunchKernelGGL(k_col_offsets, dim3(grid_for(nnz + 1, 256, cap)), dim3(256), 0, st, nnz,
                     ncols, b.keys_out, o_ptr);
  HIP_TRY(hipGetLastError());
}

void build_column_view(slimgpu_matrix* m) {
  hipStream_t st = m->stream;
  const int64_t nnz = m->nnz;
  m->d_colptr = DeviceBuffer<int64_t>((size_t)m->ncols + 1);
  m->d_colind = DeviceBuffer<int32_t>((size_t)nnz + 64);
  if (!m->binary) m->d_colval = DeviceBuffer<float>((size_t)nnz);
  m->d_cnorm = DeviceBuffer<float>((size_t)m->ncols);
  m->d_csq = DeviceBuffer<float>((size_t)m->ncols);
  DeviceBuffer<int64_t> d_cost((size_t)m->ncols);

  if (nnz > 0) {
    if (nnz > 0xFFFFFFF0ll) throw HipFail{hipErrorInvalidValue, "nnz >= 2^32 not supported"};
    DeviceBuffer<uint32_t> keys_in((size_t)nnz), keys_out((size_t)nnz);
    DeviceBuffer<uint64_t> pay_in((size_t)nnz), pay_out((size_t)nnz);
    const SortBufs b{keys_in.get(), keys_out.get(), pay_in.get(), pay_out.get()};
    DeviceBuffer<int32_t> d_flags(1);
    HIP_TRY(hipMemsetAsync(d_flags.get(), 0, sizeof(int32_t), st));
    pack_entries(m, m->nrows, m->ncols, nnz, m->d_rowptr, m->d_rowind, m->d_rowval, b, d_flags.get());
    int32_t h_flags = 0;
    HIP_TRY(hipMemcpyAsync(&h_flags, d_flags.get(), sizeof(int32_t), hipMemcpyDeviceToHost, st));
    HIP_TRY(hipStreamSynchronize(st));
    if (h_flags)
      throw InputError{h_flags & kBadRowptr
                           ? "rowptr is not a non-decreasing offset array ending at nnz"
                           : "item id outside [0, ncols)"};
    DeviceBuffer<uint8_t> tmp;
    sort_entries(m, m->ncols, nnz, b, [&](size_t bytes) { return (tmp = DeviceBuffer<uint8_t>(bytes)).get(); },
                 d_flags.get(), m->d_colptr.get(), m->d_colind.get(), m->d_colval.get());
    HIP_TRY(hipMemcpyAsync(&h_flags, d_flags.get(), sizeof(int32_t), hipMemcpyDeviceToHost, st));
    HIP_TRY(hipStreamSynchronize(st));
    if (h_flags & kDupEntry)
      throw InputError{"duplicate (user, item) entries in the rating matrix (SLIM_GPU_DUPLICATES=sum "
                       "merges them while a host matrix is staged)"};
  } else {
    HIP_TRY(hipMemsetAsync(m->d_colptr.get(), 0, sizeof(int64_t) * ((size_t)m->ncols + 1), st));
  }
  DeviceBuffer<int32_t> d_inexact(1);
  HIP_TRY(hipMemsetAsync(d_inexact.get(), 0, sizeof(int32_t), st));
  hipLaunchKernelGGL(k_col_scalars, dim3(grid_for((int64_t)m->ncols * 64, 256, m->num_cus * 16)),
                     dim3(256), 0, st, m->ncols, m->d_colptr.get(), m->d_colind.get(), m->d_colval.get(),
                     m->d_rowptr, m->d_csq.get(), m->d_cnorm.get(), d_cost.get(), d_inexact.get());
  HIP_TRY(hipGetLastError());
  int32_t h_inexact = 0;
  HIP_TRY(hipMemcpyAsync(&h_inexact, d_inexact.get(), sizeof(int32_t), hipMemcpyDeviceToHost, st));
  m->h_cost.resize((size_t)m->ncols);
  HIP_TRY(hipMemcpyAsync(m->h_cost.data(), d_cost.get(), sizeof(int64_t) * (size_t)m->ncols,
                         hipMemcpyDeviceToHost, st));
  HIP_TRY(hipStreamSynchronize(st));
  m->exact_gram = (h_inexact & 1) != 0;
  m->nonpositive = (h_inexact & 2) != 0;
}

void transpose_on_device(slimgpu_matrix* m, int32_t n, int64_t nnz, const int64_t* d_ptr,
                         const int32_t* d_ind, const float* d_val, DeviceBuffer<int64_t>& o_ptr,
                         DeviceBuffer<int32_t>& o_ind, DeviceBuffer<float>& o_val) {
  o_ptr = DeviceBuffer<int64_t>((size_t)n + 1);
  o_ind = DeviceBuffer<int32_t>((size_t)std::max<int64_t>(nnz, 1));
  o_val = DeviceBuffer<float>((size_t)std::max<int64_t>(nnz, 1));
  if (nnz <= 0) {
    HIP_TRY(hipMemsetAsync(o_ptr.get(), 0, sizeof(int64_t) * ((size_t)n + 1), m->stream));
    return;
  }
  if (nnz > 0xFFFFFFF0ll) throw HipFail{hipErrorInvalidValue, "model nnz >= 2^32 not supported"};
  const auto evict = evict_cache(m);
  const SortBufs b{m->ws_tkeys[0].reserve((size_t)nnz, evict), m->ws_tkeys[1].reserve((size_t)nnz, evict),
                   m->ws_tpay[0].reserve((size_t)nnz, evict), m->ws_tpay[1].reserve((size_t)nnz, evict)};
  int32_t* d_flags = m->ws_misc.reserve(16, evict);
  pack_entries(m, n, n, nnz, d_ptr, d_ind, d_val, b, d_flags);
  sort_entries(m, n, nnz, b, [&](size_t bytes) { return m->ws_ttmp.reserve(bytes, evict); }, nullptr,
               o_ptr.get(), o_ind.get(), o_val.get());
}

void ensure_split(slimgpu_matrix* m, UserSplit& s, int nr, bool even_share) {
  if (s.nranges == nr) return;
  s.ubounds.reset();
  s.csplit.reset();
  s.nranges = 0;
  std::vector<int32_t> ub((size_t)nr + 1, 0);
  ub[(size_t)nr] = m->nrows;
  if (nr > 1) {
    if (m->h_rowptr.empty()) {
      m->h_rowptr.resize((size_t)m->nrows + 1);
      HIP_TRY(hipMemcpy(m->h_rowptr.data(), m->d_rowptr, sizeof(int64_t) * ((size_t)m->nrows + 1),
                        hipMemcpyDeviceToHost));
    }
    for (int j = 1; j < nr; ++j) {
      const int64_t want = even_share ? m->nnz / nr * j : (int64_t)((double)m->nnz / nr * j);
      ub[(size_t)j] = (int32_t)(std::lower_bound(m->h_rowptr.begin(), m->h_rowptr.end(), want) -
                                m->h_rowptr.begin());
      ub[(size_t)j] = std::min(std::max(ub[(size_t)j], ub[(size_t)j - 1]), m->nrows);
    }
  }
  int32_t mx = 1;
  for (int j = 0; j < nr; ++j) mx = std::max(mx, ub[(size_t)j + 1] - ub[(size_t)j]);
  s.max_rows = mx;
  s.ubounds = DeviceBuffer<int32_t>((size_t)nr + 1);
  HIP_TRY(hipMemcpy(s.ubounds.get(), ub.data(), sizeof(int32_t) * ((size_t)nr + 1), hipMemcpyHostToDevice));
  s.csplit = DeviceBuffer<int64_t>((size_t)m->ncols * ((size_t)nr + 1));
  hipLaunchKernelGGL(k_col_split, dim3(grid_for((int64_t)m->ncols * (nr + 1), 256, m->num_cus * 8)), dim3(256), 0,
                     m->stream, m->ncols, nr, s.ubounds.get(), m->d_colptr.get(), m->d_colind.get(),
                     s.csplit.get());
  HIP_TRY(hipGetLastError());
  HIP_TRY(hipStreamSynchronize(m->stream));
  s.nranges = nr;
}

void ensure_cluster_split(slimgpu_matrix* m, int lg) { ensure_split(m, m->split[lg], 1 << lg, true); }

void destroy(slimgpu_matrix* m) {
  if (!m) return;
  for (slimgpu_matrix* r : m->replicas) destroy(r);
  (void)hipSetDevice(m->device);
  if (m->stream) (void)hipStreamDestroy(m->stream);
  delete m;
}

}

slimgpu_stats_t& last_stats() { return g_stats; }
ColumnStats& last_column_stats() { return g_colstats; }

LearnOptions decode_options(const int32_t* io, const double* dopt) {
  LearnOptions o;
  auto geti = [&](int idx, int32_t def) { return (!io || io[idx] == -1) ? def : io[idx]; };
  auto getd = [&](int idx, double def) { return (!dopt || dopt[idx] == -1) ? def : dopt[idx]; };
  o.nthreads = geti(SLIM_OPTION_NTHREADS, 1);
  o.nnbrs = geti(SLIM_OPTION_NNBRS, 0);
  o.simtype = geti(SLIM_OPTION_SIMTYPE, SLIM_SIMTYPE_COS);
  o.dbglvl = geti(SLIM_OPTION_DBGLVL, 0);
  o.algo = geti(SLIM_OPTION_ALGO, SLIM_ALGO_CD);
  o.ordered = geti(SLIM_OPTION_ORDERED, 0);
  o.maxniters = geti(SLIM_OPTION_MAXNITERS, 10000);
  o.l1r = getd(SLIM_OPTION_L1R, 1.0);
  o.l2r = getd(SLIM_OPTION_L2R, 1.0);
  o.optTol = getd(SLIM_OPTION_OPTTOL, 1e-7);
  o.col_begin = geti(SLIM_OPTION_GPU_COLBEGIN, 0);
  o.col_end = geti(SLIM_OPTION_GPU_COLEND, -1);
  o.seed = (uint32_t)geti(SLIM_OPTION_GPU_SEED, 1);
  o.device = geti(SLIM_OPTION_GPU_DEVICE, -1);
  o.kernel = geti(SLIM_OPTION_GPU_KERNEL, SLIMGPU_KERNEL_AUTO);
  o.cluster = geti(SLIM_OPTION_GPU_CLUSTER, 0);
  o.heavy_tiles = geti(SLIM_OPTION_GPU_HEAVYTILES, -1);
  o.heavy_cluster = geti(SLIM_OPTION_GPU_HEAVYCLUSTER, 0);
  o.ngpus = std::max(1, geti(SLIM_OPTION_GPU_NGPUS, 1));
  o.shard_count = std::max(1, geti(SLIM_OPTION_GPU_SHARDCOUNT, 1));
  o.shard_index = geti(SLIM_OPTION_GPU_SHARDINDEX, 0);
  return o;
}

int32_t device_count() {
  int n = 0;
  if (hipGetDeviceCount(&n) != hipSuccess) return 0;
  return n;
}

namespace {
template <class Fill>
slimgpu_matrix_t* make_matrix(const char* who, int32_t* status, Fill&& fill) {
  slimgpu_matrix* m = nullptr;
  try {
    m = new slimgpu_matrix();
    fill(m);
    if (status) *status = SLIM_OK;
    return m;
  } catch (const HipFail& e) {
    report(e, who);
    if (status) *status = status_of(e);
  } catch (const InputError& e) {
    set_error(std::string(who) + ": " + e.msg);
    if (status) *status = SLIM_ERROR_INPUT;
  } catch (const std::bad_alloc&) {
    set_error(std::string(who) + ": out of host memory");
    if (status) *status = SLIM_ERROR_MEMORY;
  }
  destroy(m);
  return nullptr;
}
}

slimgpu_matrix_t* matrix_from_host(int32_t nrows, const ssize_t* rowptr, const int32_t* rowind,
                                   const float* rowval, const LearnOptions& opt,
                                   int32_t* status) {
  if (nrows < 0 || !rowptr || (rowptr[nrows] > 0 && !rowind)) {
    set_error("SLIMGPU_MatrixFromHost: bad CSR arguments");
    if (status) *status = SLIM_ERROR_INPUT;
    return nullptr;
  }
  const double t0 = now_ms();
  std::vector<int64_t> mptr;
  std::vector<int32_t> mind;
  std::vector<float> mval;
  try {
  if (const char* e = std::getenv("SLIM_GPU_DUPLICATES"); e && std::strcmp(e, "sum") == 0 && nrows > 0) {
    bool any = false;
    std::vector<std::pair<int32_t, float>> row;
    mptr.assign((size_t)nrows + 1, 0);
    mind.reserve((size_t)rowptr[nrows]);
    if (rowval) mval.reserve((size_t)rowptr[nrows]);
    for (int32_t u = 0; u < nrows; ++u) {
      const int64_t s0 = rowptr[u], e0 = rowptr[u + 1];
      row.clear();
      for (int64_t k = s0; k < e0; ++k) row.emplace_back(rowind[k], rowval ? rowval[k] : 1.0f);
      bool sorted = true;
      for (size_t k = 1; k < row.size(); ++k) sorted = sorted && row[k - 1].first < row[k].first;
      if (!sorted) {
        std::stable_sort(row.begin(), row.end(),
                         [](const auto& a, const auto& b) { return a.first < b.first; });
        size_t w = 0;
        for (size_t k = 0; k < row.size(); ++k) {
          if (w > 0 && row[w - 1].first == row[k].first) {
            if (rowval) row[w - 1].second += row[k].second;
            any = true;
          } else {
            row[w++] = row[k];
          }
        }
        row.resize(w);
      }
      for (const auto& pr : row) {
        mind.push_back(pr.first);
        if (rowval) mval.push_back(pr.second);
      }
      mptr[(size_t)u + 1] = (int64_t)mind.size();
    }
    if (any) {
      rowptr = reinterpret_cast<const ssize_t*>(mptr.data());
      rowind = mind.data();
      if (rowval) rowval = mval.data();
    }
  }
  } catch (const std::bad_alloc&) {
    set_error("SLIMGPU_MatrixFromHost: out of host memory while merging repeated pairs");
    if (status) *status = SLIM_ERROR_MEMORY;
    return nullptr;
  }
  return make_matrix("SLIMGPU_MatrixFromHost", status, [&](slimgpu_matrix* m) {
    pick_device(m, opt);
    m->nrows = nrows;
    m->nnz = rowptr[nrows];
    m->binary = rowval == nullptr;
    m->merged = !mptr.empty() && rowptr == reinterpret_cast<const ssize_t*>(mptr.data());
    m->ncols = max_index_plus_one(m->nnz, rowind);
    if (m->ncols <= 0) m->ncols = 1;
    m->owns_csr = true;
    m->d_rowptr = DeviceBuffer<int64_t>((size_t)nrows + 1).release();
    m->d_rowind = DeviceBuffer<int32_t>((size_t)m->nnz).release();
    m->d_rowval = m->binary ? nullptr : DeviceBuffer<float>((size_t)m->nnz).release();
    static_assert(sizeof(ssize_t) == sizeof(int64_t), "LP64 expected");
    HIP_TRY(hipMemcpyAsync(m->d_rowptr, rowptr, sizeof(int64_t) * ((size_t)nrows + 1),
                           hipMemcpyHostToDevice, m->stream));
    if (m->nnz > 0) {
      HIP_TRY(hipMemcpyAsync(m->d_rowind, rowind, sizeof(int32_t) * (size_t)m->nnz,
                             hipMemcpyHostToDevice, m->stream));
      if (!m->binary)
        HIP_TRY(hipMemcpyAsync(m->d_rowval, rowval, sizeof(float) * (size_t)m->nnz,
                               hipMemcpyHostToDevice, m->stream));
    }
    build_column_view(m);
    m->setup_ms = now_ms() - t0;
  });
}

slimgpu_matrix_t* matrix_from_device(int32_t nrows, int32_t ncols, const int64_t* d_rowptr,
                                     const int32_t* d_rowind, const float* d_rowval,
                                     const LearnOptions& opt, int32_t* status) {
  if (nrows < 0 || !d_rowptr) {
    set_error("SLIMGPU_MatrixFromDevice: bad CSR arguments");
    if (status) *status = SLIM_ERROR_INPUT;
    return nullptr;
  }
  const double t0 = now_ms();
  return make_matrix("SLIMGPU_MatrixFromDevice", status, [&](slimgpu_matrix* m) {
    pick_device(m, opt);
    m->nrows = nrows;
    m->owns_csr = false;
    m->d_rowptr = const_cast<int64_t*>(d_rowptr);
    m->d_rowind = const_cast<int32_t*>(d_rowind);
    m->d_rowval = const_cast<float*>(d_rowval);
    m->binary = d_rowval == nullptr;
    HIP_TRY(hipMemcpy(&m->nnz, d_rowptr + nrows, sizeof(int64_t), hipMemcpyDeviceToHost));
    if (ncols <= 0) {
      DeviceBuffer<int32_t> d_max(1);
      int32_t init = -1;
      HIP_TRY(hipMemcpy(d_max.get(), &init, sizeof(int32_t), hipMemcpyHostToDevice));
      if (m->nnz > 0) {
        hipLaunchKernelGGL(k_max_index, dim3(grid_for(m->nnz, 256, m->num_cus * 8)), dim3(256), 0,
                           m->stream, m->d_rowind, m->nnz, d_max.get());
        HIP_TRY(hipGetLastError());
        HIP_TRY(hipStreamSynchronize(m->stream));
      }
      HIP_TRY(hipMemcpy(&init, d_max.get(), sizeof(int32_t), hipMemcpyDeviceToHost));
      ncols = init + 1;
    }
    m->ncols = ncols > 0 ? ncols : 1;
    build_column_view(m);
    m->setup_ms = now_ms() - t0;
  });
}

void matrix_free(slimgpu_matrix_t* m) { destroy(m); }

slimgpu_matrix_t* matrix_clone_to_device(const slimgpu_matrix_t* src, int32_t device,
                                         int32_t* status) {
  const double t0 = now_ms();
  return make_matrix("SLIMGPU_MatrixFromHost (device-to-device copy of the staged matrix)", status,
                     [&](slimgpu_matrix* m) {
    (void)hipGetLastError();
    LearnOptions o;
    o.device = device;
    pick_device(m, o);
    m->nrows = src->nrows;
    m->ncols = src->ncols;
    m->nnz = src->nnz;
    m->binary = src->binary;
    m->exact_gram = src->exact_gram;
    m->nonpositive = src->nonpositive;
    m->merged = src->merged;
    m->owns_csr = true;
    m->h_cost = src->h_cost;
    const size_t nz = (size_t)std::max<int64_t>(m->nnz, 1);
    m->d_rowptr = DeviceBuffer<int64_t>((size_t)m->nrows + 1).release();
    m->d_rowind = DeviceBuffer<int32_t>(nz).release();
    m->d_rowval = m->binary ? nullptr : DeviceBuffer<float>(nz).release();
    m->d_colptr = DeviceBuffer<int64_t>((size_t)m->ncols + 1);
    m->d_colind = DeviceBuffer<int32_t>(nz + 64);
    if (!m->binary) m->d_colval = DeviceBuffer<float>(nz);
    m->d_cnorm = DeviceBuffer<float>((size_t)m->ncols);
    m->d_csq = DeviceBuffer<float>((size_t)m->ncols);
    int can_peer = m->device == src->device ? 1 : 0;
    if (!can_peer) {
      if (hipDeviceCanAccessPeer(&can_peer, m->device, src->device) != hipSuccess) can_peer = 0;
      (void)hipGetLastError();
    }
    if (const char* e = std::getenv("SLIM_GPU_PEER")) can_peer = can_peer && std::atoi(e) != 0;
    void* bounce = nullptr;
    const size_t bounce_bytes = size_t(256) << 20;
    struct BounceFree {
      void** p;
      ~BounceFree() {
        if (*p) (void)hipHostFree(*p);
      }
    } bounce_guard{&bounce};
    auto peer = [&](void* dst, const void* from, size_t bytes) {
      if (bytes == 0 || !dst || !from) return;
      if (can_peer) {
        HIP_TRY(hipMemcpyPeerAsync(dst, m->device, from, src->device, bytes, m->stream));
        return;
      }
      if (!bounce) HIP_TRY(hipHostMalloc(&bounce, bounce_bytes, hipHostMallocDefault));
      for (size_t off = 0; off < bytes; off += bounce_bytes) {
        const size_t n = std::min(bounce_bytes, bytes - off);
        HIP_TRY(hipSetDevice(src->device));
        HIP_TRY(hipMemcpy(bounce, static_cast<const char*>(from) + off, n, hipMemcpyDeviceToHost));
        HIP_TRY(hipSetDevice(m->device));
        HIP_TRY(hipMemcpy(static_cast<char*>(dst) + off, bounce, n, hipMemcpyHostToDevice));
      }
    };
    peer(m->d_rowptr, src->d_rowptr, sizeof(int64_t) * ((size_t)m->nrows + 1));
    peer(m->d_colptr.get(), src->d_colptr.get(), sizeof(int64_t) * ((size_t)m->ncols + 1));
    peer(m->d_cnorm.get(), src->d_cnorm.get(), sizeof(float) * (size_t)m->ncols);
    peer(m->d_csq.get(), src->d_csq.get(), sizeof(float) * (size_t)m->ncols);
    if (m->nnz > 0) {
      peer(m->d_rowind, src->d_rowind, sizeof(int32_t) * (size_t)m->nnz);
      peer(m->d_colind.get(), src->d_colind.get(), sizeof(int32_t) * (size_t)m->nnz);
      peer(m->d_rowval, src->d_rowval, sizeof(float) * (size_t)m->nnz);
      peer(m->d_colval.get(), src->d_colval.get(), sizeof(float) * (size_t)m->nnz);
    }
    HIP_TRY(hipStreamSynchronize(m->stream));
    m->setup_ms = now_ms() - t0;
  });
}

void matrix_add_replica(slimgpu_matrix_t* m, slimgpu_matrix_t* replica) {
  m->replicas.push_back(replica);
}
const std::vector<slimgpu_matrix_t*>& matrix_replicas(const slimgpu_matrix_t* m) {
  return m->replicas;
}
void matrix_adopt_csr(slimgpu_matrix_t* m) { m->owns_csr = true; }
int32_t matrix_device(const slimgpu_matrix_t* m) { return m ? m->device : -1; }
void matrix_set_setup_ms(slimgpu_matrix_t* m, double ms) { m->setup_ms = ms; }

int32_t matrix_info(const slimgpu_matrix_t* m, int32_t* nrows, int32_t* ncols, int64_t* nnz) {
  if (!m) return SLIM_ERROR_INPUT;
  if (nrows) *nrows = m->nrows;
  if (ncols) *ncols = m->ncols;
  if (nnz) *nnz = m->nnz;
  return SLIM_OK;
}

double matrix_setup_ms(const slimgpu_matrix_t* m) { return m ? m->setup_ms : 0.0; }

void matrix_expect_solves(slimgpu_matrix_t* m, int32_t n) {
  if (!m) return;
  m->expect_solves = n;
  for (slimgpu_matrix* r : m->replicas) r->expect_solves = n;
}

int32_t matrix_column_cost(const slimgpu_matrix_t* m, int64_t* cost) {
  if (!m || !cost) return SLIM_ERROR_INPUT;
  std::memcpy(cost, m->h_cost.data(), sizeof(int64_t) * m->h_cost.size());
  return SLIM_OK;
}

int32_t matrix_get_column_view(const slimgpu_matrix_t* m, int64_t* colptr, int32_t* colind,
                               float* colval, float* cnorms) {
  if (!m) return SLIM_ERROR_INPUT;
  try {
    HIP_TRY(hipSetDevice(m->device));
    if (colptr)
      HIP_TRY(hipMemcpy(colptr, m->d_colptr.get(), sizeof(int64_t) * ((size_t)m->ncols + 1),
                        hipMemcpyDeviceToHost));
    if (colind && m->nnz)
      HIP_TRY(hipMemcpy(colind, m->d_colind.get(), sizeof(int32_t) * (size_t)m->nnz,
                        hipMemcpyDeviceToHost));
    if (colval && m->nnz && m->d_colval.get())
      HIP_TRY(hipMemcpy(colval, m->d_colval.get(), sizeof(float) * (size_t)m->nnz,
// ... 334 lines not shown
  m->G_alloc_ms = alloc_ms;
  m->G_sums_ms = t_sums - tb - alloc_ms;
  m->G_sums_kernel_ms = sums_kernel_ms;
  m->G_pack_ms = now_ms() - t_sums;
  if (trace_level >= 1)
    std::fprintf(stderr, "[trace] G = R^T R (%d x %d, %.2f GB) built in %.1f ms: allocation %.1f, sums %.1f "
                 "(kernel %.1f), byte planes %.1f\n", m->ncols, m->ncols,
                 sizeof(float) * (double)m->ncols * (double)m->G_ld * 1e-9, m->G_build_ms, m->G_alloc_ms,
                 m->G_sums_ms, sums_kernel_ms, m->G_pack_ms);
  return SLIM_OK;
}

void finish_path(slimgpu_matrix* m, const LearnOptions& opt, int32_t nwork, const slim_csr_t* imodel,
                 const slimgpu_model* warm_dev, Path& p) {
  p.exact_gram = m->exact_gram || std::getenv("SLIM_GPU_EXACT_GRAM") || (opt.nnbrs > 0 && m->nonpositive);
  if (p.kernel == SLIMGPU_KERNEL_AUTO)
    p.kernel = p.lds_need <= 64 * 1024 ? SLIMGPU_KERNEL_WAVE_LDS : SLIMGPU_KERNEL_TILE;
  if (p.kernel == SLIMGPU_KERNEL_WAVE_LDS && p.lds_need > 160 * 1024)
    throw Refusal{SLIM_ERROR_INPUT, "SLIMGPU_Learn: work vectors do not fit the 160 KiB LDS of a CU"};
  if (p.kernel < SLIMGPU_KERNEL_WAVE_LDS || p.kernel > SLIMGPU_KERNEL_GRAM_FSLIM)
    throw Refusal{SLIM_ERROR_INPUT, "SLIMGPU_Learn: unknown kernel selection"};
  if (p.use_fgram) {
    p.f_stride = std::max(64, round_up(std::min(opt.nnbrs, m->ncols - 1), 64));
    p.f_ustride = (int)std::min<int64_t>((int64_t)32 * p.f_stride, p.ncols_pad);
    p.f_block = p.f_stride <= kFslimBlockMaxStride;
    if (const char* e = std::getenv("SLIM_GPU_FSLIM_BLOCK")) p.f_block = p.f_block && std::atoi(e) != 0;
    p.f_tab_n = p.f_block ? round_up(p.f_ustride, 8) : 0;
    p.f_wave_lds = fslim_wave_lds(p.f_stride, p.f_block, p.f_tab_n);
    p.f_waves = (int)std::max<size_t>(1, std::min<size_t>(p.f_block ? kFslimMaxWaves : 4, (size_t(150) << 10) / p.f_wave_lds));
    p.fn_f = fslim_solve_fn(p.f_block);
    p.f_union_lds = fslim_union_lds(m->ncols);
    if (p.f_union_lds > (size_t(150) << 10))
      throw Refusal{SLIM_ERROR_INPUT, "SLIMGPU_Learn: the item-space FSLIM kernel's item bitmap does not fit the LDS of a CU"};
    HIP_TRY(hipFuncSetAttribute(reinterpret_cast<const void*>(fslim_union_fn()),
                                hipFuncAttributeMaxDynamicSharedMemorySize, (int)p.f_union_lds));
    const size_t lds = p.f_wave_lds * (size_t)p.f_waves;
    int per_cu = 0;
    HIP_TRY(hipFuncSetAttribute(reinterpret_cast<const void*>(p.fn_f), hipFuncAttributeMaxDynamicSharedMemorySize, (int)lds));
    HIP_TRY(hipOccupancyMaxActiveBlocksPerMultiprocessor(&per_cu, reinterpret_cast<const void*>(p.fn_f), 64 * p.f_waves, lds));
    if (per_cu < 1)
      throw Refusal{SLIM_ERROR, "SLIMGPU_Learn: the item-space FSLIM kernel does not fit a compute unit of this device"};
    p.nwaves = std::max(1, std::min((nwork + p.f_waves - 1) / p.f_waves, m->num_cus * per_cu));
    if (warm_dev && warm_dev->device != m->device)
      throw Refusal{SLIM_ERROR_INPUT, "SLIMGPU_LearnResident: the warm-start model lives on another device"};
    p.has_imodel = false;
    if (p.trace_level >= 1)
      std::fprintf(stderr, "[trace] item-space FSLIM: form %s, lists of %d, %d wavefronts per workgroup (%zu KB of LDS "
                   "each), %d workgroups per CU\n", p.f_block ? "block in LDS" : "gathered", p.f_stride, p.f_waves,
                   p.f_wave_lds >> 10, per_cu);
    return;
  }
  p.use_lds = p.kernel == SLIMGPU_KERNEL_WAVE_LDS;
  if (p.use_gram && p.gram_v == 0)
    if (const char* e = std::getenv("SLIM_GPU_GRAM_NW")) p.gram_nw = std::atoi(e) == 8 ? 8 : 16;
  if (p.use_gram && m->G_ready && !m->Gp_tried && !m->Gf_dropped) {
    (void)pack_gram(m);
    drop_float_gram(m);
  }
  size_t gramr_lds = 0;
  bool gramr_ring = false;
  int gramr_wps = 0;
  bool gramr_dma = (m->Gp_nchunks + kGramrNT - 1) / kGramrNT > 6;
  if (const char* e = std::getenv("SLIM_GPU_GRAMR_DMA")) gramr_dma = std::atoi(e) != 0;
  if (p.use_gram && m->Gp_ready && !std::getenv("SLIM_GPU_NO_GRAMR"))
    p.fn_r = gramr_kernel(m->Gp_nchunks, gramr_dma, &p.gramr_kr, &p.gramr_kl, &gramr_lds, &gramr_ring, &gramr_wps);
  p.use_gramr = p.fn_r != nullptr;
  if (p.use_gram && !p.use_gramr && m->Gf_dropped)
    throw Refusal{SLIM_ERROR, "SLIMGPU_Learn: the floats of G were dropped and the byte-plane kernel cannot run this solve"};
  if (p.use_gramr) {
    p.gram_nw = kGramrNT / 64;
    p.gram_v = 1;
  }
  p.gram_lds = p.use_gramr ? gramr_lds : (p.gram_v > 0 ? sizeof(float) * (size_t)p.ncols_pad : 0);
  if (p.use_gram && p.trace_level >= 1) {
    if (p.use_gramr)
      std::fprintf(stderr, "[trace] item-space kernel: packed <%d,%d>, %s loads, WPS %d\n", p.gramr_kr, p.gramr_kl,
                   gramr_ring ? "ring" : "register", gramr_wps);
    else
      std::fprintf(stderr, "[trace] item-space kernel: float <%d,%d>\n", p.gram_nw, p.gram_v);
  }
  p.tileP = p.kernel == SLIMGPU_KERNEL_TILE16 ? 16 : 32;
  if (p.kernel == SLIMGPU_KERNEL_TILE && ((int64_t)p.nrows_pad + 64) * 128 >= (int64_t(1) << 32)) p.tileP = 16;
  p.use_tile = p.kernel == SLIMGPU_KERNEL_TILE || p.kernel == SLIMGPU_KERNEL_TILE16;
  if (p.use_tile && ((int64_t)p.nrows_pad + 64) * 4 * p.tileP >= (int64_t(1) << 32)) {
    p.use_tile = false;
    p.kernel = SLIMGPU_KERNEL_WAVE_HBM;
  }
  if (p.use_tile && p.tileP == 16 && opt.nnbrs > 0) {
    p.use_tile = false;
    p.kernel = SLIMGPU_KERNEL_WAVE_HBM;
  }
  if (p.use_tile) p.kernel = p.tileP == 32 ? SLIMGPU_KERNEL_TILE : SLIMGPU_KERNEL_TILE16;
  if (opt.build_G && !p.use_tile)
    throw Refusal{SLIM_ERROR_INPUT, "SLIMGPU_Learn: G = R^T R is built by the tile kernel, which this matrix cannot use"};
  p.fn = p.use_gram ? gram_kernel(p.gram_nw, p.gram_v) : pick_kernel(p.use_lds, !m->binary);
  p.tileNW = (nwork + p.tileP - 1) / p.tileP >= 2 * m->num_cus ? 8 : 16;
  p.req_cluster = opt.cluster;
  if (opt.build_G && p.use_tile && p.tileP == 32 && m->binary && !std::getenv("SLIM_GPU_NO_GBITS")) {
    ensure_cluster_split(m, 5);
    const size_t need = sizeof(uint32_t) * (size_t)(round_up(m->split[5].max_rows, 64) + 64);
    size_t words_cap = 148 * 1024;
    if (test_hook("SLIM_GPU_TEST_GBITS_ROWS"))
      words_cap = sizeof(uint32_t) * (size_t)(round_up(std::max(64, std::atoi(std::getenv("SLIM_GPU_TEST_GBITS_ROWS"))), 64) + 64);
    if (need <= words_cap && m->num_cus >= 32) {
      p.gram_bits_lds = need;
      p.req_cluster = 32;
      p.tileNW = 16;
    } else if (m->num_cus >= 32 && !std::getenv("SLIM_GPU_NO_GPASSES")) {
      const int64_t rows_cap = (int64_t)(words_cap / sizeof(uint32_t)) - 128;
      int np = (int)((m->split[5].max_rows + rows_cap - 1) / rows_cap);
      for (; np <= 64; ++np) {
        ensure_split(m, m->gsplit, 32 * np, false);
        const size_t need_p = sizeof(uint32_t) * (size_t)(round_up(m->gsplit.max_rows, 64) + 64);
        if (need_p <= words_cap) {
          p.gram_bits_lds = need_p;
          p.req_cluster = 32;
          p.tileNW = 16;
          p.gram_passes = np;
          if (p.trace_level >= 1)
            std::fprintf(stderr, "[trace] G builder: %d user passes (32 members x %d users at most, %zu KB of words)\n",
                         np, m->gsplit.max_rows, need_p >> 10);
          break;
        }
      }
    }
  }
  if (const char* e = std::getenv("SLIM_GPU_TILE_NW")) p.tileNW = std::atoi(e) == 16 ? 16 : 8;
  if (warm_dev && warm_dev->device != m->device)
    throw Refusal{SLIM_ERROR_INPUT, "SLIMGPU_LearnResident: the warm-start model lives on another device"};
  p.has_imodel = warm_dev ? warm_dev->n > 0 : (imodel && imodel->colptr && imodel->ncols > 0);
  bool row_fold = true;
  if (const char* e = std::getenv("SLIM_GPU_FOLD")) row_fold = std::strcmp(e, "col") != 0;
  if (p.use_tile) {
    const bool prof = p.trace_level >= 2;
    const bool val = !m->binary;
    const bool nw16 = p.tileNW == 16;
    const char* form = "colfold";
    bool profiled = false;
    if (p.tileP == 32 && opt.nnbrs > 0) {
      p.fn = tile_kernel_p32_fslim(val, nw16);
      form = "fslim";
    } else if (p.tileP == 32 && !prof && !p.has_imodel) {
      p.fn = tile_kernel_p32_cold(val, nw16);
      form = "cold";
    } else if (p.tileP == 32 && !prof && row_fold) {
      p.fn = tile_kernel_p32_rowfold(val, nw16);
      form = "rowfold";
    } else if (p.tileP == 32) {
      p.fn = nw16 ? tile_kernel_p32_nw16(val, prof) : tile_kernel_p32_nw8(val, prof);
      profiled = prof;
    } else {
      p.fn = nw16 ? tile_kernel_p16_nw16(val, prof) : tile_kernel_p16_nw8(val, prof);
      profiled = prof;
    }
    if (p.trace_level >= 1)
      std::fprintf(stderr, "[trace] tile kernel: P %d, %d wavefronts, form %s, %s%s\n", p.tileP, nw16 ? 16 : 8,
                   form, val ? "valued" : "binary", profiled ? ", profiled" : "");
  }
  int waves_per_cu;
  if (p.use_gram) {
    int per_cu = 0;
    const void* kfn = p.use_gramr ? reinterpret_cast<const void*>(p.fn_r) : reinterpret_cast<const void*>(p.fn);
    HIP_TRY(hipFuncSetAttribute(kfn, hipFuncAttributeMaxDynamicSharedMemorySize, (int)p.gram_lds));
    HIP_TRY(hipOccupancyMaxActiveBlocksPerMultiprocessor(&per_cu, kfn, 64 * p.gram_nw, p.gram_lds));
    if (per_cu < 1)
      throw Refusal{SLIM_ERROR, "SLIMGPU_Learn: the item-space kernel does not fit a compute unit of this device"};
    waves_per_cu = per_cu;
  } else if (p.use_lds) {
    waves_per_cu = (int)std::min<size_t>(16, (160 * 1024) / std::max<size_t>(p.lds_need, 1));
    if (waves_per_cu < 1) waves_per_cu = 1;
    if (p.lds_need > 64 * 1024)
      HIP_TRY(hipFuncSetAttribute(reinterpret_cast<const void*>(p.fn),
                                  hipFuncAttributeMaxDynamicSharedMemorySize, (int)p.lds_need));
  } else {
    waves_per_cu = 8;
  }
  p.nwaves = std::max(1, std::min(nwork, m->num_cus * waves_per_cu));
  if (!p.use_gram && !p.use_tile && p.trace_level >= 1)
    std::fprintf(stderr, "[trace] wave kernel: %s, %s, sums %s, %d wavefronts, %zu bytes of LDS\n",
                 p.use_lds ? "lds" : "hbm", m->binary ? "binary" : "valued", p.exact_gram ? "ordered" : "atomic",
                 p.nwaves, p.use_lds ? p.lds_need : (size_t)0);
  p.wg_slots = m->num_cus * (16 / p.tileNW);
  if (p.use_tile) {
    int per_cu = 0;
    const size_t worst_lds = std::max<size_t>(kBitmapBytes, p.gram_bits_lds);
    HIP_TRY(hipFuncSetAttribute(reinterpret_cast<const void*>(p.fn),
                                hipFuncAttributeMaxDynamicSharedMemorySize, (int)worst_lds));
    HIP_TRY(hipOccupancyMaxActiveBlocksPerMultiprocessor(&per_cu, reinterpret_cast<const void*>(p.fn),
                                                         64 * p.tileNW, worst_lds));
    if (opt.build_G && per_cu >= 1) {
      const size_t stage = (size_t)kGramStageBytes * (size_t)p.tileNW;
      const char* e = std::getenv("SLIM_GPU_GREAD");
      if (e && std::atoi(e) == 0) {
        p.gram_stage_why = "SLIM_GPU_GREAD=0";
      } else if (p.tileP != 32) {
        p.gram_stage_why = "16-item tiles";
      } else if (stage > worst_lds) {
        hipFuncAttributes fa{};
        HIP_TRY(hipFuncGetAttributes(&fa, reinterpret_cast<const void*>(p.fn)));
        int per_cu_s = 0;
        if (fa.sharedSizeBytes + stage <= (size_t)160 * 1024) {
          HIP_TRY(hipFuncSetAttribute(reinterpret_cast<const void*>(p.fn),
                                      hipFuncAttributeMaxDynamicSharedMemorySize, (int)stage));
          HIP_TRY(hipOccupancyMaxActiveBlocksPerMultiprocessor(&per_cu_s, reinterpret_cast<const void*>(p.fn),
                                                               64 * p.tileNW, stage));
        }
        if (per_cu_s >= std::min(per_cu, 16 / p.tileNW)) {
          p.gram_stage_lds = stage;
          per_cu = per_cu_s;
        } else {
          p.gram_stage_why = "no room in LDS";
        }
      } else {
        p.gram_stage_lds = stage;
      }
    }
    if (per_cu < 1)
      throw Refusal{SLIM_ERROR, "SLIMGPU_Learn: the tile kernel does not fit a compute unit of this device"};
    p.wg_slots = m->num_cus * std::min(per_cu, 16 / p.tileNW);
  }
}

struct TileGeom {
  bool force_k1 = false;
  int clusterK = 1, cluster_lg = 0, nclusters = 0;
  int clusterHi = 0, hi_lg = 0, nheavy = 0, nclusters_hi = 0;
  size_t tile_r = 0, tile_x = 0, tile_u = 0;
  int nwaves = 0;
};

TileGeom plan_tiles(slimgpu_matrix* m, const LearnOptions& opt, const Path& p,
                    const std::vector<int32_t>& order, bool force_k1) {
  const int32_t ncols = m->ncols, nwork = (int32_t)order.size();
  const int tileP = p.tileP;
  TileGeom t;
  t.force_k1 = force_k1;
  int auto_heavy = 0;
  const int ngroups_all = (nwork + tileP - 1) / tileP;
  const int req = p.req_cluster;
  if (force_k1) {
    t.clusterK = 1;
  } else if (req == 1 || req == 2 || req == 4 || req == 8 || req == 16 || req == 32) {
    t.clusterK = req;
  } else {
    int cap = 1;
    while (cap < 16 && (m->nnz / std::max(ncols, 1)) / (2 * cap) >= 512) cap *= 2;
    if (opt.heavy_tiles < 0 && p.tileNW == 16 && ngroups_all >= 16) {
      auto tile_cost = [&](int gI) {
        int64_t c = 0;
        for (int k = gI * tileP; k < std::min((gI + 1) * tileP, nwork); ++k) c += m->h_cost[order[(size_t)k]];
        return c;
      };
      const int64_t med = tile_cost(ngroups_all / 2);
      while (auto_heavy < ngroups_all / 16 && tile_cost(auto_heavy) >= 12 * med) ++auto_heavy;
    }
    const int64_t fill = auto_heavy > 0 ? 4 : 8;
    while (t.clusterK < cap && (int64_t)ngroups_all * t.clusterK < fill * (int64_t)p.wg_slots) t.clusterK *= 2;
  }
  while (t.clusterK > 1 && p.wg_slots / t.clusterK < 1) t.clusterK /= 2;
  for (t.cluster_lg = 0; (1 << t.cluster_lg) < t.clusterK; ++t.cluster_lg) {}
  ensure_cluster_split(m, t.cluster_lg);
  t.tile_r = (size_t)(round_up(m->split[t.cluster_lg].max_rows, 64) + 64) * tileP;
  if (opt.build_G && p.gram_bits_lds && t.clusterK == 32 && !force_k1) t.tile_r = (size_t)64 * tileP;
  t.tile_x = (size_t)p.ncols_pad * tileP;
  t.tile_u = (size_t)p.ncols_pad;
  t.nclusters = std::max(1, std::min(ngroups_all, p.wg_slots / t.clusterK));
  t.nheavy = std::min(opt.heavy_tiles < 0 ? auto_heavy : opt.heavy_tiles, ngroups_all);
  t.clusterHi = opt.heavy_cluster;
  if (const char* e = std::getenv("SLIM_GPU_HEAVY")) {
    int a = 0, b = 0;
    if (std::sscanf(e, "%d,%d", &a, &b) == 2) {
      t.nheavy = std::min(std::max(a, 0), ngroups_all);
      t.clusterHi = b;
    }
  }
  if (t.clusterHi != 2 && t.clusterHi != 4 && t.clusterHi != 8 && t.clusterHi != 16 && t.clusterHi != 32)
    t.clusterHi = std::max(16, std::min(4 * t.clusterK, kTileKMax));
  if (t.clusterHi <= t.clusterK || t.nclusters * t.clusterK < t.clusterHi || force_k1) t.nheavy = 0;
  if (t.nheavy > 0) {
    for (t.hi_lg = 0; (1 << t.hi_lg) < t.clusterHi; ++t.hi_lg) {}
    ensure_cluster_split(m, t.hi_lg);
    t.nclusters_hi = t.nclusters * t.clusterK / t.clusterHi;
    t.tile_r = std::max(t.tile_r, (size_t)(round_up(m->split[t.hi_lg].max_rows, 64) + 64) * tileP);
  }
  size_t free_b = 0, total_b = 0;
  HIP_TRY(hipMemGetInfo(&free_b, &total_b));
  const size_t per_cl = ((t.tile_r + 2 * t.tile_x) * sizeof(float) + t.tile_u * sizeof(int32_t)) * t.clusterK;
  const size_t have = free_b + m->ws_slab.bytes() + m->ws_xslab.bytes() + m->ws_ulist.bytes() +
                      m->ws_part.bytes() + m->ws_gram.bytes();
  const size_t budget = have > (size_t(6) << 30) ? have - (size_t(6) << 30) : have / 2;
  if ((size_t)t.nclusters * per_cl > budget) {
    t.nclusters = (int)std::max<size_t>(1, budget / per_cl);
    t.nclusters_hi = t.nclusters * t.clusterK / std::max(t.clusterHi, 1);
    if (t.nclusters_hi < 1) t.nheavy = 0;
  }
  t.nwaves = t.nclusters * t.clusterK;
  return t;
}

size_t mailbox_stride(int tileP) { return 2 * (size_t)kTileKMax * (size_t)tileP + 8; }

struct Slabs {
  float *slab = nullptr, *xslab = nullptr, *part = nullptr;
  int32_t *ulist = nullptr, *nunion = nullptr;
  unsigned long long* mailbox = nullptr;
  size_t mailbox_words = 0;
  int bm_shift = 0, bm_words = 1;
  size_t tile_lds = 0;
  bool gram_words = false;
  int32_t *f_n = nullptr, *f_id = nullptr, *f_slot = nullptr;
  float* f_aty = nullptr;
  int f_slice_tiles = 0;
};

Slabs alloc_slabs(slimgpu_matrix* m, const LearnOptions& opt, const Path& p, const TileGeom& t, int32_t nwork,
                  int nwaves) {
  Slabs s;
  const auto evict = evict_cache(m);
  if (p.use_fgram) {
    const size_t ngroups0 = std::max<size_t>(1, ((size_t)nwork + 31) / 32);
    const size_t per_tile = (size_t)32 * (size_t)p.f_stride * 12;
    size_t free_b = 0, total_b = 0;
    HIP_TRY(hipMemGetInfo(&free_b, &total_b));
    const size_t have = free_b + m->ws_fid.bytes() + m->ws_faty.bytes() + m->ws_fslot.bytes();
    size_t tiles = ngroups0;
    if (tiles * per_tile > have / 4) tiles = std::max<size_t>(1, have / 4 / per_tile);
    if (const char* e = std::getenv("SLIM_GPU_FSLIM_SLICE_TILES"); e && std::atoi(e) > 0)
      tiles = std::min<size_t>(tiles, (size_t)std::atoi(e));
    s.f_slice_tiles = (int)tiles;
    const size_t npos = std::min<size_t>((size_t)std::max(nwork, 1), tiles * 32);
    s.f_n = m->ws_fn.reserve(npos, evict);
    s.f_id = m->ws_fid.reserve(npos * (size_t)p.f_stride, evict);
    s.f_aty = m->ws_faty.reserve(npos * (size_t)p.f_stride, evict);
    s.f_slot = m->ws_fslot.reserve(npos * (size_t)p.f_stride, evict);
    s.ulist = m->ws_ulist.reserve((size_t)p.f_ustride * tiles, evict);
    s.nunion = m->ws_nunion.reserve(tiles, evict);
  } else if (p.use_gram) {
    const size_t ngroups0 = ((size_t)nwork + 31) / 32;
    s.xslab = m->ws_xslab.reserve((size_t)p.ncols_pad * (size_t)nwaves, evict);
    if (p.gram_v == 0) s.slab = m->ws_slab.reserve((size_t)p.ncols_pad * (size_t)nwaves, evict);
    s.ulist = m->ws_ulist.reserve((size_t)p.ncols_pad * ngroups0, evict);
    s.nunion = m->ws_nunion.reserve(ngroups0, evict);
  } else if (p.use_tile) {
    s.mailbox_words = (size_t)(std::max(t.nclusters, 1) + t.nclusters_hi) * mailbox_stride(p.tileP);
    s.slab = m->ws_slab.reserve(t.tile_r * (size_t)nwaves, evict);
    s.xslab = m->ws_xslab.reserve(t.tile_x * (size_t)nwaves, evict);
    s.ulist = m->ws_ulist.reserve(t.tile_u * (size_t)nwaves, evict);
    s.mailbox = m->ws_mailbox.reserve(s.mailbox_words, evict);
    s.part = m->ws_part.reserve(t.tile_x * (size_t)nwaves, evict);
    const int64_t range = (int64_t)(t.tile_r / (size_t)p.tileP);
    auto words_at = [&](int sh) { return ((range >> sh) + 1 + 31) / 32; };
    while (words_at(s.bm_shift) * 4 > kBitmapBytes) ++s.bm_shift;
    s.bm_words = (int)words_at(s.bm_shift);
    if (opt.nnbrs > 0) s.bm_words = std::max(s.bm_words, p.tileP * 256);
    s.tile_lds = sizeof(uint32_t) * (size_t)s.bm_words;
    if (p.gram_bits_lds && t.clusterK == 32 && !t.force_k1) {
      s.bm_shift = 0;
      s.bm_words = (int)(p.gram_bits_lds / sizeof(uint32_t));
      s.tile_lds = p.gram_bits_lds;
      s.gram_words = true;
    }
    if (opt.build_G) s.tile_lds = std::max(s.tile_lds, p.gram_stage_lds);
  } else if (!p.use_lds) {
    s.slab = m->ws_slab.reserve(p.vec_floats * (size_t)nwaves);
  }
  return s;
}

struct ArenaSeg {
  const int32_t* ind;
  const float* val;
  int64_t n;
  DeviceBuffer<int32_t> own_i;
  DeviceBuffer<float> own_v;
};

struct Launch {
  Path p;
  TileGeom t;
  Slabs s;
  int nwaves = 1;
  int32_t *order = nullptr, *cnt = nullptr, *sti = nullptr, *misc = nullptr;
  int64_t *off = nullptr, *stl = nullptr;
  float* stf = nullptr;
  const int64_t* icolptr = nullptr;
  const int32_t* icolind = nullptr;
  const float* icolval = nullptr;
  int32_t incols = 0;
  int gram_mode = 0;
  float* gram = nullptr;
  int gram_geom[6] = {0, 0, 0, 0, 0, 0};
  int gram_pass = 0;
  DeviceBuffer<float> carry;
  int64_t carry_stride = 0;
  bool carry_from_warm = false;
  bool cluster_fallback = false;
  int64_t arena_cap = 0;
  int32_t G_block = 0;
  bool gview_tried = false;
  const uint4* gview = nullptr;
  const int64_t* gview_base = nullptr;
  const uint16_t* gview_cnt = nullptr;
  int32_t gview_ngroups = 0, gview_sentinel = 0;
  size_t gview_bytes = 0;
  double gview_ms = 0;
  const char* gview_why = "";
};

void prepare_launch(slimgpu_matrix* m, const LearnOptions& opt, const std::vector<int32_t>& order,
                    const slim_csr_t* imodel, const slimgpu_model* warm_dev, bool resident, bool all_columns,
                    Launch& L) {
  const int32_t ncols = m->ncols, nwork = (int32_t)order.size();
  const Path& p = L.p;
  hipStream_t stream = m->stream;
  L.nwaves = p.nwaves;
  if (p.use_tile) {
    L.t = plan_tiles(m, opt, p, order, false);
    L.nwaves = L.t.nwaves;
  }
  L.order = m->ws_order.reserve((size_t)nwork);
  L.cnt = m->ws_cnt.reserve((size_t)ncols);
  L.off = m->ws_off.reserve((size_t)ncols);
  L.sti = m->ws_stat_i.reserve(3 * (size_t)ncols);
  L.stl = m->ws_stat_l.reserve(4 * (size_t)ncols);
  L.stf = m->ws_stat_f.reserve(2 * (size_t)ncols);
  L.misc = m->ws_misc.reserve(16);
  L.s = alloc_slabs(m, opt, p, L.t, nwork, L.nwaves);

  L.arena_cap = std::max<int64_t>(1 << 20, (int64_t)nwork * std::min<int64_t>(ncols, 8192));
  if (const char* env_cap = std::getenv("SLIM_GPU_ARENA")) L.arena_cap = std::max<int64_t>(1, std::atoll(env_cap));

  if (p.has_imodel && warm_dev) {
    L.incols = warm_dev->n;
    L.icolptr = warm_dev->d_colptr.get();
    L.icolind = warm_dev->d_colind.get();
    L.icolval = warm_dev->d_colval.get();
  } else if (p.has_imodel) {
    L.incols = imodel->ncols;
    const int64_t innz = imodel->colptr[L.incols];
    int64_t* cp = m->ws_icolptr.reserve((size_t)L.incols + 1);
    int32_t* ci = m->ws_icolind.reserve((size_t)innz);
    float* cv = m->ws_icolval.reserve((size_t)innz);
    HIP_TRY(hipMemcpyAsync(cp, imodel->colptr, sizeof(int64_t) * ((size_t)L.incols + 1),
                           hipMemcpyHostToDevice, stream));
    if (innz > 0) {
      HIP_TRY(hipMemcpyAsync(ci, imodel->colind, sizeof(int32_t) * (size_t)innz, hipMemcpyHostToDevice, stream));
      HIP_TRY(hipMemcpyAsync(cv, imodel->colval, sizeof(float) * (size_t)innz, hipMemcpyHostToDevice, stream));
    }
    L.icolptr = cp;
    L.icolind = ci;
    L.icolval = cv;
  }
  HIP_TRY(hipMemsetAsync(L.cnt, 0, sizeof(int32_t) * (size_t)ncols, stream));
  HIP_TRY(hipMemsetAsync(L.off, 0, sizeof(int64_t) * (size_t)ncols, stream));
  HIP_TRY(hipMemsetAsync(L.sti, 0, sizeof(int32_t) * 3 * (size_t)ncols, stream));
  HIP_TRY(hipMemsetAsync(L.stl, 0, sizeof(int64_t) * 4 * (size_t)ncols, stream));
  HIP_TRY(hipMemsetAsync(L.stf, 0, sizeof(float) * 2 * (size_t)ncols, stream));

  const TileGeom& t = L.t;
  const int geom[6] = {p.tileP, t.clusterK, t.nheavy > 0 ? t.clusterHi : 0, t.nheavy, opt.shard_count,
                       opt.shard_index};
  std::copy(geom, geom + 6, L.gram_geom);
  if (p.use_tile && !opt.build_G && !std::getenv("SLIM_GPU_NO_GRAM")) {
    const size_t ngroups0 = ((size_t)nwork + p.tileP - 1) / p.tileP;
    const size_t need = ngroups0 * t.tile_x * sizeof(float);
    if (!m->gram_order.empty() && m->gram_order == order && m->ws_gram.bytes() >= need &&
        std::equal(geom, geom + 6, m->gram_geom)) {
      L.gram_mode = 2;
      L.gram = m->ws_gram.get();
    } else {
      size_t free_b = 0, total_b = 0;
      HIP_TRY(hipMemGetInfo(&free_b, &total_b));
      if (need <= (size_t(32) << 30) && need <= (free_b + m->ws_gram.bytes()) / 4) {
        m->gram_order.clear();
        L.gram = m->ws_gram.reserve(need / sizeof(float));
        L.gram_mode = 1;
      }
    }
  }

  const int carry_groups = std::max(p.gramr_kr, 1) + p.gramr_kl;
  if (resident && p.use_gramr && carry_groups <= kGramrCarryMaxGroups && all_columns && nwork == ncols &&
      opt.shard_count == 1 && !std::getenv("SLIM_GPU_NO_CARRY")) {
    L.carry_stride = (int64_t)carry_groups * 8192;
    const size_t carry_bytes = sizeof(float) * (size_t)ncols * (size_t)L.carry_stride;
    if (warm_dev && warm_dev->d_gsave.get() && warm_dev->gsave_owner == m->uid &&
        warm_dev->gsave_stride == L.carry_stride && warm_dev->n == ncols) {
      L.carry_from_warm = warm_dev->gsave_valid && warm_dev->gsave_l1 == opt.l1r;
      L.carry = std::move(warm_dev->d_gsave);
      warm_dev->gsave_valid = false;
    } else {
      size_t free_b = 0, total_b = 0;
      HIP_TRY(hipMemGetInfo(&free_b, &total_b));
      if (carry_bytes <= (size_t(8) << 30) && carry_bytes * 4 <= free_b)
        L.carry = DeviceBuffer<float>((size_t)ncols * (size_t)L.carry_stride);
    }
  }
}

SolveArgs solve_args(slimgpu_matrix* m, const LearnOptions& opt, Launch& L, const std::vector<int32_t>& pending,
                     int attempt, int32_t* d_ai, float* d_av) {
  const Path& p = L.p;
  const TileGeom& t = L.t;
  const int32_t ncols = m->ncols, npend = (int32_t)pending.size();
  hipStream_t stream = m->stream;
  SolveArgs S;
  S.l1 = (float)opt.l1r;
  S.l2 = (float)opt.l2r;
  S.opt_tol = (float)opt.optTol;
  S.maxniters = opt.maxniters;
  S.seed = opt.seed;
  S.nnbrs = opt.nnbrs;
  S.simtype = opt.simtype;
  S.order = L.order;
  S.nwork = npend;
  S.queue = L.misc;
  S.icolptr = L.icolptr;
  S.icolind = L.icolind;
  S.icolval = L.icolval;
  S.incols = L.incols;
  S.slab = L.s.slab;
  S.slab_stride = p.use_tile ? (int64_t)t.tile_r : (int64_t)p.vec_floats;
  S.nrows_pad = p.nrows_pad;
  S.ncols_pad = p.ncols_pad;
  S.xslab = L.s.xslab;
  S.x_stride = (int64_t)t.tile_x;
  S.ulist = L.s.ulist;
  S.u_stride = (int64_t)t.tile_u;
  S.ngroups = (npend + p.tileP - 1) / p.tileP;
  if (opt.build_G && opt.G_rows_end >= 0) S.ngroups = (L.G_block + p.tileP - 1) / p.tileP;
  S.cluster = t.clusterK;
  S.ubounds = p.use_tile ? m->split[t.cluster_lg].ubounds.get() : nullptr;
  S.csplit = p.use_tile ? m->split[t.cluster_lg].csplit.get() : nullptr;
  S.mailbox = L.s.mailbox;
  S.exact_gram = p.exact_gram ? 1 : 0;
  S.atypart = L.s.part;
  S.bm_shift = L.s.bm_shift;
  S.bm_words = L.s.bm_words;
  S.nheavy = p.use_tile ? t.nheavy : 0;
  S.cluster_hi = t.clusterHi;
  S.ubounds_hi = t.nheavy > 0 ? m->split[t.hi_lg].ubounds.get() : nullptr;
  S.csplit_hi = t.nheavy > 0 ? m->split[t.hi_lg].csplit.get() : nullptr;
  S.mailbox_hi = L.s.mailbox ? L.s.mailbox + (size_t)std::max(t.nclusters, 1) * mailbox_stride(p.tileP) : nullptr;
  S.queue_hi = L.misc + 4;
  S.hi_prefetch = 1;
  S.shard_count = opt.shard_count;
  S.shard_index = opt.shard_index;
  S.nnz_last = m->nnz > 0 ? m->nnz - 1 : 0;
  S.xcd_swizzle = 0;
  S.gram_mode = (attempt == 0 && !L.cluster_fallback) ? L.gram_mode : 0;
  S.gram = L.gram;
  S.G = m->ws_G.get();
  S.G_ld = m->G_ld;
  S.tile_nunion = L.s.nunion;
  S.gram_pos = nullptr;
  S.gram_bits = (p.gram_bits_lds && t.clusterK == 32 && L.s.gram_words) ? 2 : 0;
  if (const char* e = std::getenv("SLIM_GPU_GBITS"); e && S.gram_bits) S.gram_bits = std::atoi(e) == 1 ? 1 : 2;
  S.gram_split_stride = t.clusterK + 1;
  S.gram_accum = 0;
  S.gram_store = 0;
  S.gram_read = 0;
  S.gview = nullptr;
  S.gview_base = nullptr;
  S.gview_cnt = nullptr;
  S.gview_ngroups = 0;
  S.gview_range0 = 0;
  S.gview_sentinel = 0;
  S.gram_part16 = S.gram_bits == 2 ? 1 : 0;
  if (const char* e = std::getenv("SLIM_GPU_GPART16"); e && std::atoi(e) == 0) S.gram_part16 = 0;
  S.g_save = nullptr;
  S.g_load = nullptr;
  S.g_stride = 0;
  if (L.carry.get()) {
    S.g_save = L.carry.get();
    S.g_stride = L.carry_stride;
    S.g_load = (L.carry_from_warm && attempt == 0) ? L.carry.get() : nullptr;
  }
  if (L.p.gram_passes > 1) {
    if (S.gram_bits) {
      S.ubounds = m->gsplit.ubounds.get() + 32 * L.gram_pass;
      S.csplit = m->gsplit.csplit.get() + 32 * L.gram_pass;
      S.gram_split_stride = 32 * L.p.gram_passes + 1;
      S.gram_accum = L.gram_pass > 0;
    } else {
      L.p.gram_passes = 1;
      L.gram_pass = 0;
    }
  }
  if (opt.build_G) {
    if (npend != ncols)
      throw Refusal{SLIM_ERROR, "SLIMGPU_Learn: internal: G = R^T R must be built over all columns at once"};
    std::vector<int32_t> pos((size_t)ncols, 0);
    for (int32_t k = 0; k < npend; ++k) pos[(size_t)pending[(size_t)k]] = k;
    int32_t* d_pos = m->ws_nunion.reserve((size_t)ncols, evict_cache(m));
    HIP_TRY(hipMemcpyAsync(d_pos, pos.data(), sizeof(int32_t) * (size_t)ncols, hipMemcpyHostToDevice, stream));
    HIP_TRY(hipStreamSynchronize(stream));
    S.gram_pos = d_pos;
    S.gram_mode = 3;
    S.gram_store = opt.G_rows_end >= 0 ? 1 : 2;
    if (const char* e = std::getenv("SLIM_GPU_GLINES"); e && std::atoi(e) >= 0 && std::atoi(e) < S.gram_store)
      S.gram_store = std::atoi(e);
    S.gram_read = (S.gram_store != 0 && p.gram_stage_lds && L.s.tile_lds >= p.gram_stage_lds) ? 1 : 0;
  }
  if (p.use_gram) {
    S.slab_stride = (int64_t)p.ncols_pad;
    S.x_stride = (int64_t)p.ncols_pad;
    S.u_stride = (int64_t)p.ncols_pad;
    S.ngroups = (npend + 31) / 32;
  }
  if (p.use_fgram) {
    S.u_stride = (int64_t)p.f_ustride;
    S.ngroups = (npend + 31) / 32;
  }
  if (const char* e = std::getenv("SLIM_GPU_HI_PREFETCH")) S.hi_prefetch = std::atoi(e);
  if (p.use_tile)
    HIP_TRY(hipMemsetAsync(L.s.mailbox, 0, sizeof(unsigned long long) * L.s.mailbox_words, stream));
  S.trace = nullptr;
  if (p.use_tile && p.trace_level >= 1) {
    S.trace = m->ws_trace.reserve(16 * (size_t)S.ngroups);
    HIP_TRY(hipMemsetAsync(S.trace, 0, sizeof(uint64_t) * 16 * (size_t)S.ngroups, stream));
  }
  S.out_cnt = L.cnt;
  S.out_off = L.off;
  S.out_ind = d_ai;
  S.out_val = d_av;
  S.out_cursor = reinterpret_cast<unsigned long long*>(L.misc + 2);
  S.out_cap = L.arena_cap;
  S.overflow = L.misc + 1;
  S.st_na = L.sti;
  S.st_sweeps = L.sti + ncols;
  S.st_conv = L.sti + 2 * (size_t)ncols;
  S.st_G = L.stl;
  S.st_D = L.stl + ncols;
  S.st_U = L.stl + 2 * (size_t)ncols;
  S.st_B = L.stl + 3 * (size_t)ncols;
  S.st_err = L.stf;
  S.st_obj = L.stf + ncols;
  return S;
}

void build_gview(slimgpu_matrix* m, Launch& L, const SolveArgs& S, const int32_t* d_colind) {
  L.gview_tried = true;
  if (const char* e = std::getenv("SLIM_GPU_GVIEW"); e && std::atoi(e) == 0) {
    L.gview_why = " (SLIM_GPU_GVIEW=0)";
    return;
  }
  hipStream_t stream = m->stream;
  const double t0 = now_ms();
  const int nranges = 32 * L.p.gram_passes;
  const int ngroups = (S.nwork + 63) / 64;
  const int sentinel = S.bm_words - 64;
  if ((int64_t)nranges * ngroups >= (int64_t(1) << 31) || sentinel >= 65536 || sentinel < 0) {
    L.gview_why = " (ranges beyond 16-bit ids)";
    return;
  }
  const int nblocks = nranges * ngroups;
  try {
    int32_t* d_rows = m->ws_gvrows.reserve((size_t)nblocks);
    int64_t* d_base = m->ws_gvbase.reserve((size_t)nblocks + 1);
    uint16_t* d_cnt = m->ws_gvcnt.reserve((size_t)nblocks * 64);
    const dim3 grid((unsigned)((nblocks + 3) / 4)), block(256);
    hipLaunchKernelGGL(k_gview_rows, grid, block, 0, stream, S.order, S.nwork, S.csplit, S.gram_split_stride, ngroups,
                       nblocks, d_rows, d_cnt);
    HIP_TRY(hipGetLastError());
    std::vector<int32_t> rows((size_t)nblocks);
    HIP_TRY(hipMemcpyAsync(rows.data(), d_rows, sizeof(int32_t) * rows.size(), hipMemcpyDeviceToHost, stream));
    HIP_TRY(hipStreamSynchronize(stream));
    std::vector<int64_t> base((size_t)nblocks + 1, 0);
    for (int b = 0; b < nblocks; ++b) base[(size_t)b + 1] = base[(size_t)b] + rows[(size_t)b];
    const int64_t total = base[(size_t)nblocks];
    uint4* d_view = m->ws_gview.reserve((size_t)std::max<int64_t>(total, 1), evict_cache(m));
    HIP_TRY(hipMemcpyAsync(d_base, base.data(), sizeof(int64_t) * base.size(), hipMemcpyHostToDevice, stream));
    hipLaunchKernelGGL(k_gview_fill, grid, block, 0, stream, S.order, S.nwork, S.csplit, S.gram_split_stride, S.ubounds,
                       d_colind, ngroups, nblocks, d_base, (uint32_t)sentinel, d_view);
    HIP_TRY(hipGetLastError());
    HIP_TRY(hipStreamSynchronize(stream));
    L.gview = d_view;
    L.gview_base = d_base;
    L.gview_cnt = d_cnt;
    L.gview_ngroups = ngroups;
    L.gview_sentinel = sentinel;
    L.gview_bytes = (size_t)total * 16;
    L.gview_ms = now_ms() - t0;
  } catch (const HipFail& e) {
    if (e.code != hipErrorOutOfMemory) throw;
    (void)hipGetLastError();
    m->ws_gview.reset();
    L.gview_why = " (no room for the 16-bit view)";
  }
}

void print_tile_trace(const slimgpu_matrix* m, const Launch& L, const SolveArgs& S, const std::vector<int32_t>& pending,
                      int launch_waves, float ms) {
  const int clusterK = L.t.clusterK, tileP = L.p.tileP, npend = (int)pending.size();
  std::vector<uint64_t> tr(16 * (size_t)S.ngroups);
  HIP_TRY(hipMemcpy(tr.data(), S.trace, sizeof(uint64_t) * tr.size(), hipMemcpyDeviceToHost));
  uint64_t t0 = ~0ull, t1 = 0;
  double busy = 0, setup = 0, sweeps = 0, fold = 0;
  std::vector<double> dur;
  for (int gI = 0; gI < S.ngroups; ++gI) {
    const uint64_t* e = &tr[8 * (size_t)gI];
    t0 = std::min(t0, e[0]);
    t1 = std::max(t1, e[3]);
    const double wk = double(e[6]) / clusterK;
    busy += double(e[3] - e[0]) * wk;
    setup += double(e[1] - e[0]) * wk;
    sweeps += double(e[2] - e[1]) * wk;
    fold += double(e[7] - e[1]) * wk;
    dur.push_back(double(e[3] - e[0]) * 1e-5);
  }
  std::sort(dur.begin(), dur.end());
  const double span = double(t1 - t0);
  std::fprintf(stderr,
               "[trace] tiles %d (%d heavy, clusters of %d) on %d workgroups (clusters of %d): span %.2f ms (event %.2f ms), busy/"
               "(span*wgs) %.2f, setup %.1f%% sweeps %.1f%% (fold %.1f%%) of busy; tile ms min %.2f med "
               "%.2f p90 %.2f max %.2f\n",
               S.ngroups, S.nheavy, S.nheavy > 0 ? L.t.clusterHi : 0, launch_waves, clusterK, span * 1e-5, ms,
               busy * clusterK / (span * launch_waves), 100 * setup / busy, 100 * sweeps / busy,
               100 * fold / busy,
               dur.front(), dur[dur.size() / 2], dur[dur.size() * 9 / 10], dur.back());
  if (S.ngroups >= 16) {
    std::fprintf(stderr, "[trace] tile cost -> ms, queue order:");
    for (int k = 0; k < 19; ++k) {
      const int gI = k < 12 ? k : (int)((int64_t)S.ngroups * (k - 11) / 8) - (k == 19 ? 1 : 0);
      if (gI >= S.ngroups) break;
      double c = 0;
      for (int j = gI * tileP; j < std::min((gI + 1) * tileP, npend); ++j)
        c += (double)m->h_cost[pending[(size_t)j]];
      std::fprintf(stderr, " [%d] %.3g -> %.0f", gI, c,
                   double(tr[8 * (size_t)gI + 3] - tr[8 * (size_t)gI]) * 1e-5);
    }
    std::fprintf(stderr, "\n");
  }
  if (L.p.trace_level >= 2) {
    double ph[7] = {0, 0, 0, 0, 0, 0, 0};
    for (int gI = 0; gI < S.ngroups; ++gI)
      for (int k = 0; k < 7; ++k) ph[k] += double(tr[8 * (size_t)S.ngroups + 8 * (size_t)gI + k]);
    const double tot = ph[0] + ph[1] + ph[2] + ph[3] + ph[4];
    std::fprintf(stderr,
                 "[trace] visit phases (shader clocks/visit): loads %.0f reduce+barrier %.0f "
                 "math %.0f stores %.0f closing barrier %.0f | total %.0f; visits %.0f, "
                 "%.1f%% with update\n",
                 ph[0] / ph[5], ph[1] / ph[5], ph[2] / ph[5], ph[3] / ph[5], ph[4] / ph[5],
                 tot / ph[5], ph[5], 100 * ph[6] / ph[5]);
  }
}

struct Entries {
  std::vector<int32_t> cnt;
  std::vector<int64_t> off;
  int64_t total = 0;
  std::vector<int32_t> ind;
  std::vector<float> val;
  std::vector<ArenaSeg> segs;
  double kernel_ms = 0, d2h_ms = 0;
};

Entries run_launches(slimgpu_matrix* m, const LearnOptions& opt, const std::vector<int32_t>& order, bool resident,
                     Launch& L) {
  const int32_t ncols = m->ncols;
  hipStream_t stream = m->stream;
  const Path& p = L.p;
  struct EventPair {
    hipEvent_t a = nullptr, b = nullptr;
    ~EventPair() {
      if (a) (void)hipEventDestroy(a);
      if (b) (void)hipEventDestroy(b);
    }
  } events;
  HIP_TRY(hipEventCreate(&events.a));
  HIP_TRY(hipEventCreate(&events.b));
  const hipEvent_t ev0 = events.a, ev1 = events.b;
  DevMatrix A;
  A.nrows = m->nrows;
  A.ncols = ncols;
  A.nnz = m->nnz;
  A.rowptr = m->d_rowptr;
  A.rowind = m->d_rowind;
  A.rowval = m->d_rowval;
  A.colptr = m->d_colptr.get();
  A.colind = m->d_colind.get();
  A.colval = m->d_colval.get();
  A.cnorm = m->d_cnorm.get();
  A.csq = m->d_csq.get();
  GramPacked P{};
  if (p.use_gramr) {
    P.lo = m->ws_Glo.get();
    P.ldb = m->Gp_ldb;
    P.hi = m->ws_Ghi.get();
    P.hi_off = m->ws_hioff.get();
    P.hi_k = m->ws_hik.get();
    P.hi2_off = m->ws_hi2off.get();
    P.hi2_k = m->ws_hi2k.get();
    P.base = m->ws_Gbase.get();
    P.diag = m->ws_Gdiag.get();
    P.meta = m->ws_Gmeta.get();
    P.rank_of = m->ws_rankof.get();
    P.item_of = m->ws_itemof.get();
    P.nchunks = m->Gp_nchunks;
  }

  struct DropView {
    slimgpu_matrix* m;
    ~DropView() {
      m->ws_gview.reset();
      m->ws_gvbase.reset();
      m->ws_gvrows.reset();
      m->ws_gvcnt.reset();
    }
  } drop_view{m};

  Entries E;
  E.cnt.assign((size_t)ncols, 0);
  E.off.assign((size_t)ncols, 0);
  std::vector<int32_t> h_cnt((size_t)ncols, 0);
  std::vector<int64_t> h_off((size_t)ncols, 0);
  std::vector<int32_t> pending = order;
  for (int attempt = 0; attempt < 8 && !pending.empty(); ++attempt) {
    const int32_t npend = (int32_t)pending.size();
    int32_t* d_ai = m->ws_arena_i.reserve((size_t)L.arena_cap, evict_cache(m));
    float* d_av = m->ws_arena_v.reserve((size_t)L.arena_cap, evict_cache(m));
    if (L.gram_mode != 0 && m->ws_gram.get() != L.gram) {
      L.gram_mode = 0;
      L.gram = nullptr;
    }
    HIP_TRY(hipMemcpyAsync(L.order, pending.data(), sizeof(int32_t) * (size_t)npend, hipMemcpyHostToDevice, stream));
    HIP_TRY(hipMemsetAsync(L.misc, 0, sizeof(int32_t) * 16, stream));
    if (attempt > 0) L.t.nheavy = 0;
    SolveArgs S = solve_args(m, opt, L, pending, attempt, d_ai, d_av);
    const int clusterK = L.t.clusterK;
    if (opt.build_G && S.gram_bits == 2 && !L.gview_tried) build_gview(m, L, S, A.colind);
    if (opt.build_G && S.gram_bits == 2 && L.gview) {
      S.gview = L.gview;
      S.gview_base = L.gview_base;
      S.gview_cnt = L.gview_cnt;
      S.gview_ngroups = L.gview_ngroups;
      S.gview_range0 = 32 * L.gram_pass;
      S.gview_sentinel = L.gview_sentinel;
    }
    if (opt.build_G && p.trace_level >= 1) {
      const bool in_passes = S.gram_bits != 0 && p.gram_passes > 1;
      std::fprintf(stderr, "[trace] G builder: form %s, clusters of %d, pass %d of %d, %d users at most per member\n",
                   S.gram_bits == 2 ? "bits2" : (S.gram_bits == 1 ? "bits1" : "lines"), clusterK, L.gram_pass + 1,
                   p.gram_passes, in_passes ? m->gsplit.max_rows : m->split[L.t.cluster_lg].max_rows);
      if (S.gview)
        std::fprintf(stderr, "[trace] G builder: ids from view, %zu bytes = %.3f x 2 bytes per nnz, built in %.1f ms\n",
                     L.gview_bytes, (double)L.gview_bytes / (2.0 * (double)std::max<int64_t>(m->nnz, 1)), L.gview_ms);
      else
        std::fprintf(stderr, "[trace] G builder: ids from csc%s\n", S.gram_bits == 2 ? L.gview_why : "");
      if (S.gram_read)
        std::fprintf(stderr, "[trace] G builder: sums read once, %zu of %zu bytes of LDS hold the staging tiles\n",
                     p.gram_stage_lds, L.s.tile_lds);
      else if (S.gram_store != 0)
        std::fprintf(stderr, "[trace] G builder: sums read in rounds (%s)\n", p.gram_stage_why);
    }

    const int launch_waves = p.use_tile ? std::max(1, std::min((npend + p.tileP - 1) / p.tileP, L.t.nclusters)) * clusterK
                                        : std::max(1, std::min(npend, L.nwaves));
    HIP_TRY(hipEventRecord(ev0, stream));
    if (p.use_gramr)
      hipLaunchKernelGGL(gramr_union_fn(), dim3(S.ngroups), dim3(gramr_union_threads()), 0, stream, A, S, P);
    else if (p.use_gram)
      hipLaunchKernelGGL(gram_union_fn(), dim3(S.ngroups), dim3(64), 0, stream, A, S);
    if (S.nheavy > 0 && launch_waves < L.t.clusterHi) S.nheavy = 0;
    int launch_now = launch_waves;
    if (p.use_tile && clusterK > 1 && !L.cluster_fallback && test_hook("SLIM_GPU_TEST_DROP_MEMBER")) {
      launch_now -= 1;
      S.nheavy = 0;
    }
    const int nxcd = m->num_cus % 32 == 0 ? m->num_cus / 32 : 1;
    if (p.use_tile && clusterK > 1 && nxcd == 8 && launch_now % 8 == 0 &&
        (launch_now / 8) % clusterK == 0 && (S.nheavy == 0 || (launch_now / 8) % L.t.clusterHi == 0)) {
      S.xcd_swizzle = 1;
      if (const char* e = std::getenv("SLIM_GPU_XCD")) S.xcd_swizzle = std::atoi(e) != 0;
    }
    if (p.use_fgram) {
      FslimArgs F{};
      F.stride = p.f_stride;
      F.nbr_n = L.s.f_n;
      F.nbr_id = L.s.f_id;
      F.nbr_aty = L.s.f_aty;
      F.nbr_slot = L.s.f_slot;
      F.wave_lds = (int32_t)p.f_wave_lds;
      F.tab_n = p.f_tab_n;
      const int slice = L.s.f_slice_tiles * 32;
      for (int pos0 = 0; pos0 < npend; pos0 += slice) {
        F.pos0 = pos0;
        F.npos = std::min(slice, npend - pos0);
        if (pos0 > 0) HIP_TRY(hipMemsetAsync(L.misc, 0, sizeof(int32_t), stream));
        hipLaunchKernelGGL(fslim_select_fn(), dim3(F.npos), dim3(kFslimSelectThreads), 0, stream, A, S, F);
        hipLaunchKernelGGL(fslim_union_fn(), dim3((F.npos + 31) / 32), dim3(kFslimUnionThreads), p.f_union_lds, stream,
                           A, S, F);
        hipLaunchKernelGGL(p.fn_f, dim3(std::max(1, std::min((F.npos + p.f_waves - 1) / p.f_waves, L.nwaves))),
                           dim3(64 * p.f_waves), p.f_wave_lds * (size_t)p.f_waves, stream, A, S, F);
        HIP_TRY(hipGetLastError());
      }
    } else if (p.use_gramr)
      hipLaunchKernelGGL(p.fn_r, dim3(launch_now), dim3(kGramrNT), p.gram_lds, stream, A, S, P);
    else
      hipLaunchKernelGGL(p.fn, dim3(launch_now), dim3(p.use_gram ? 64 * p.gram_nw : (p.use_tile ? 64 * p.tileNW : 64)),
                         p.use_gram ? p.gram_lds : (p.use_lds ? p.lds_need : (p.use_tile ? L.s.tile_lds : 0)),
                         stream, A, S);
    HIP_TRY(hipGetLastError());
    HIP_TRY(hipEventRecord(ev1, stream));

    int32_t h_misc[4];
    HIP_TRY(hipMemcpyAsync(h_misc, L.misc, sizeof(h_misc), hipMemcpyDeviceToHost, stream));
    HIP_TRY(hipMemcpyAsync(h_cnt.data(), L.cnt, sizeof(int32_t) * (size_t)ncols, hipMemcpyDeviceToHost, stream));
    HIP_TRY(hipMemcpyAsync(h_off.data(), L.off, sizeof(int64_t) * (size_t)ncols, hipMemcpyDeviceToHost, stream));
    HIP_TRY(hipStreamSynchronize(stream));
    float ms = 0;
    HIP_TRY(hipEventElapsedTime(&ms, ev0, ev1));
    E.kernel_ms += ms;
    if (S.trace) print_tile_trace(m, L, S, pending, launch_waves, ms);

    if (h_misc[1] == 2) {
      if (!L.cluster_fallback && (clusterK > 1 || L.t.nheavy > 0)) {
        L.cluster_fallback = true;
        std::fprintf(stderr, "[slim-gpu] tile cluster timed out (workgroups not co-resident); "
                             "re-solving %d columns without clusters\n", npend);
        L.t = plan_tiles(m, opt, p, order, true);
        L.nwaves = L.t.nwaves;
        L.s = alloc_slabs(m, opt, p, L.t, (int32_t)order.size(), L.nwaves);
        --attempt;
        continue;
      }
      throw Refusal{SLIM_ERROR, "SLIMGPU_Learn: a tile cluster timed out waiting for a member workgroup "
                                "(were all workgroups resident?)"};
    }
    if (p.gram_passes > 1 && ++L.gram_pass < p.gram_passes) {
      --attempt;
      continue;
    }
    if (opt.build_G && S.gram_store == 2) {
      const unsigned nb = (unsigned)((ncols + kSymB - 1) / kSymB);
      int logp = 0;
      while ((1 << logp) < p.tileP) ++logp;
      HIP_TRY(hipEventRecord(ev0, stream));
      hipLaunchKernelGGL(gram_sym_fn(), dim3(nb, nb), dim3(kSymNT), 0, stream, S.G, S.G_ld, ncols, S.gram_pos, logp);
      HIP_TRY(hipGetLastError());
      HIP_TRY(hipEventRecord(ev1, stream));
      HIP_TRY(hipStreamSynchronize(stream));
      float sym_ms = 0;
      HIP_TRY(hipEventElapsedTime(&sym_ms, ev0, ev1));
      E.kernel_ms += sym_ms;
      if (p.trace_level >= 1)
        std::fprintf(stderr, "[trace] G builder: mirror half filled in %.2f ms (%u x %u blocks of %d)\n", sym_ms, nb, nb,
                     kSymB);
    }
    if (S.gram_mode == 1) {
      m->gram_order = order;
      std::copy(L.gram_geom, L.gram_geom + 6, m->gram_geom);
    }
    unsigned long long cursor;
    std::memcpy(&cursor, h_misc + 2, sizeof(cursor));
    const int64_t used = std::min<int64_t>((int64_t)cursor, L.arena_cap);
    const int64_t base = E.total;
    const double t_d2h = now_ms();
    if (resident) {
      E.segs.push_back({d_ai, d_av, used, {}, {}});
    } else {
      E.ind.resize((size_t)(base + used));
      E.val.resize((size_t)(base + used));
      if (used > 0) {
        HIP_TRY(hipMemcpyAsync(E.ind.data() + base, d_ai, sizeof(int32_t) * (size_t)used, hipMemcpyDeviceToHost, stream));
        HIP_TRY(hipMemcpyAsync(E.val.data() + base, d_av, sizeof(float) * (size_t)used, hipMemcpyDeviceToHost, stream));
        HIP_TRY(hipStreamSynchronize(stream));
      }
    }
    E.d2h_ms += now_ms() - t_d2h;
    E.total += used;

    std::vector<int32_t> again;
    int64_t need = 0;
    for (int32_t c : pending) {
      if (h_cnt[c] >= 0) {
        E.cnt[c] = h_cnt[c];
        E.off[c] = base + h_off[c];
      } else {
        again.push_back(c);
        need += -(int64_t)h_cnt[c] - 1;
      }
    }
    pending.swap(again);
    if (!pending.empty()) L.arena_cap = std::max<int64_t>(L.arena_cap, need + 1024);
    if (resident && !pending.empty() && used > 0) {
      ArenaSeg& sg = E.segs.back();
      sg.own_i = DeviceBuffer<int32_t>((size_t)used);
      sg.own_v = DeviceBuffer<float>((size_t)used);
      HIP_TRY(hipMemcpyAsync(sg.own_i.get(), sg.ind, sizeof(int32_t) * (size_t)used, hipMemcpyDeviceToDevice, stream));
      HIP_TRY(hipMemcpyAsync(sg.own_v.get(), sg.val, sizeof(float) * (size_t)used, hipMemcpyDeviceToDevice, stream));
      HIP_TRY(hipStreamSynchronize(stream));
      sg.ind = sg.own_i.get();
      sg.val = sg.own_v.get();
    }
  }
  if (!pending.empty()) throw Refusal{SLIM_ERROR_MEMORY, "SLIMGPU_Learn: output arena overflow persisted"};
  return E;
}

struct Counters {
  std::vector<float> err, obj;
  int64_t gram_rows = 0;
  double gram_bytes = 0;
};

Counters read_counters(const slimgpu_matrix* m, const Launch& L, const std::vector<int32_t>& requested,
                       ColumnStats& cs) {
  const size_t ncols = (size_t)m->ncols;
  cs.nacols.assign(ncols, 0);
  cs.sweeps.assign(ncols, 0);
  cs.conv.assign(ncols, 0);
  cs.G.assign(ncols, 0);
  cs.D.assign(ncols, 0);
  cs.U.assign(ncols, 0);
  Counters k;
  k.err.resize(ncols);
  k.obj.resize(ncols);
  HIP_TRY(hipMemcpy(cs.nacols.data(), L.sti, sizeof(int32_t) * ncols, hipMemcpyDeviceToHost));
  HIP_TRY(hipMemcpy(cs.sweeps.data(), L.sti + ncols, sizeof(int32_t) * ncols, hipMemcpyDeviceToHost));
  HIP_TRY(hipMemcpy(cs.conv.data(), L.sti + 2 * ncols, sizeof(int32_t) * ncols, hipMemcpyDeviceToHost));
  HIP_TRY(hipMemcpy(cs.G.data(), L.stl, sizeof(int64_t) * ncols, hipMemcpyDeviceToHost));
  if (L.p.use_gram) {
    for (int32_t c : requested) k.gram_rows += cs.G[(size_t)c];
    if (L.p.use_gramr) {
      std::vector<int64_t> hb(ncols);
      HIP_TRY(hipMemcpy(hb.data(), L.stl + 3 * ncols, sizeof(int64_t) * ncols, hipMemcpyDeviceToHost));
      for (int32_t c : requested) k.gram_bytes += (double)hb[(size_t)c];
    } else {
      k.gram_bytes = (double)k.gram_rows * 4.0 * (double)L.p.ncols_pad;
    }
  }
  if (L.p.use_tile || L.p.use_gram || L.p.use_fgram)
    for (int32_t c : requested) cs.G[(size_t)c] = m->h_cost[(size_t)c];
  HIP_TRY(hipMemcpy(cs.D.data(), L.stl + ncols, sizeof(int64_t) * ncols, hipMemcpyDeviceToHost));
  HIP_TRY(hipMemcpy(cs.U.data(), L.stl + 2 * ncols, sizeof(int64_t) * ncols, hipMemcpyDeviceToHost));
  HIP_TRY(hipMemcpy(k.err.data(), L.stf, sizeof(float) * ncols, hipMemcpyDeviceToHost));
  HIP_TRY(hipMemcpy(k.obj.data(), L.stf + ncols, sizeof(float) * ncols, hipMemcpyDeviceToHost));
  return k;
}

slim_csr_t* assemble_host_model(int32_t ncols, const Entries& E, int64_t tnnz, bool row_view) {
  ssize_t* colptr = static_cast<ssize_t*>(std::malloc(sizeof(ssize_t) * ((size_t)ncols + 1)));
  int32_t* colind = static_cast<int32_t*>(std::malloc(sizeof(int32_t) * (size_t)std::max<int64_t>(tnnz, 1)));
  float* colval = static_cast<float*>(std::malloc(sizeof(float) * (size_t)std::max<int64_t>(tnnz, 1)));
  if (!colptr || !colind || !colval) {
    std::free(colptr); std::free(colind); std::free(colval);
    throw Refusal{SLIM_ERROR_MEMORY, "SLIMGPU_Learn: out of host memory for the model"};
  }
  colptr[0] = 0;
  for (int32_t c = 0; c < ncols; ++c) {
    const int64_t n = E.cnt[c];
    if (n > 0) {
      std::memcpy(colind + colptr[c], E.ind.data() + E.off[c], sizeof(int32_t) * (size_t)n);
      std::memcpy(colval + colptr[c], E.val.data() + E.off[c], sizeof(float) * (size_t)n);
    }
    colptr[c + 1] = colptr[c] + n;
  }
  return model_from_columns(ncols, colptr, colind, colval, row_view);
}

std::unique_ptr<slimgpu_model> assemble_resident_model(slimgpu_matrix* m, const LearnOptions& opt, Entries& E,
                                                       int64_t tnnz, Launch& L, bool row_view,
                                                       double* t_columns_done) {
  const int32_t ncols = m->ncols;
  hipStream_t stream = m->stream;
  std::unique_ptr<slimgpu_model> dm(new slimgpu_model());
  dm->device = m->device;
  dm->n = ncols;
  dm->nnz = tnnz;
  std::vector<int64_t> h_colptr((size_t)ncols + 1, 0);
  for (int32_t c = 0; c < ncols; ++c) h_colptr[(size_t)c + 1] = h_colptr[(size_t)c] + E.cnt[(size_t)c];
  const int32_t* src_i = E.segs.empty() ? nullptr : E.segs[0].ind;
  const float* src_v = E.segs.empty() ? nullptr : E.segs[0].val;
  DeviceBuffer<int32_t> cat_i;
  DeviceBuffer<float> cat_v;
  if (E.segs.size() > 1) {
    cat_i = DeviceBuffer<int32_t>((size_t)std::max<int64_t>(E.total, 1));
    cat_v = DeviceBuffer<float>((size_t)std::max<int64_t>(E.total, 1));
    int64_t at = 0;
    for (const ArenaSeg& sg : E.segs) {
      if (sg.n > 0) {
        HIP_TRY(hipMemcpyAsync(cat_i.get() + at, sg.ind, sizeof(int32_t) * (size_t)sg.n, hipMemcpyDeviceToDevice, stream));
        HIP_TRY(hipMemcpyAsync(cat_v.get() + at, sg.val, sizeof(float) * (size_t)sg.n, hipMemcpyDeviceToDevice, stream));
      }
      at += sg.n;
    }
    src_i = cat_i.get();
    src_v = cat_v.get();
  }
  dm->d_colptr = DeviceBuffer<int64_t>((size_t)ncols + 1);
  dm->d_colind = DeviceBuffer<int32_t>((size_t)std::max<int64_t>(tnnz, 1));
  dm->d_colval = DeviceBuffer<float>((size_t)std::max<int64_t>(tnnz, 1));
  int64_t* d_src = m->ws_off.reserve((size_t)ncols, evict_cache(m));
  HIP_TRY(hipMemcpyAsync(dm->d_colptr.get(), h_colptr.data(), sizeof(int64_t) * ((size_t)ncols + 1),
                         hipMemcpyHostToDevice, stream));
  HIP_TRY(hipMemcpyAsync(d_src, E.off.data(), sizeof(int64_t) * (size_t)ncols, hipMemcpyHostToDevice, stream));
  if (tnnz > 0) {
    hipLaunchKernelGGL(k_gather_columns, dim3(grid_for((int64_t)ncols * 64, 256, m->num_cus * 16)), dim3(256),
                       0, stream, ncols, dm->d_colptr.get(), d_src, src_i, src_v, dm->d_colind.get(),
                       dm->d_colval.get());
    HIP_TRY(hipGetLastError());
  }
  *t_columns_done = now_ms();
  if (row_view) {
    transpose_on_device(m, ncols, tnnz, dm->d_colptr.get(), dm->d_colind.get(), dm->d_colval.get(), dm->d_rowptr,
                        dm->d_rowind, dm->d_rowval);
    int32_t* d_facts = m->ws_misc.reserve(2);
    int32_t facts[2] = {0, 0};
    HIP_TRY(hipMemsetAsync(d_facts, 0, sizeof(facts), stream));
    queue_row_facts(stream, m->num_cus, ncols, dm->d_rowptr.get(), dm->d_rowind.get(), d_facts);
    HIP_TRY(hipMemcpyAsync(facts, d_facts, sizeof(facts), hipMemcpyDeviceToHost, stream));
    HIP_TRY(hipStreamSynchronize(stream));
    dm->max_row = facts[0];
    dm->rows_sorted = facts[1] == 0;
  }
  HIP_TRY(hipStreamSynchronize(stream));
  if (L.carry.get()) {
    dm->d_gsave = std::move(L.carry);
    dm->gsave_valid = true;
    dm->gsave_stride = L.carry_stride;
    dm->gsave_l1 = opt.l1r;
    dm->gsave_owner = m->uid;
  }
  return dm;
}

void print_progress(const slimgpu_matrix* m, const slim_csr_t* model, const std::vector<int32_t>& requested,
                    const ColumnStats& cs, const Counters& k) {
  const int32_t ncols = m->ncols;
  const ssize_t* colptr = model->colptr;
  const int32_t* colind = model->colind;
  const float* colval = model->colval;
  std::vector<int64_t> hp((size_t)m->nrows + 1);
  std::vector<int32_t> hi((size_t)std::max<int64_t>(m->nnz, 1));
  std::vector<float> hv(m->binary ? 0 : (size_t)std::max<int64_t>(m->nnz, 1));
  std::vector<int64_t> hcp((size_t)ncols + 1);
  HIP_TRY(hipMemcpy(hp.data(), m->d_rowptr, sizeof(int64_t) * hp.size(), hipMemcpyDeviceToHost));
  HIP_TRY(hipMemcpy(hcp.data(), m->d_colptr.get(), sizeof(int64_t) * hcp.size(), hipMemcpyDeviceToHost));
  if (m->nnz > 0) {
    HIP_TRY(hipMemcpy(hi.data(), m->d_rowind, sizeof(int32_t) * (size_t)m->nnz, hipMemcpyDeviceToHost));
    if (!m->binary)
      HIP_TRY(hipMemcpy(hv.data(), m->d_rowval, sizeof(float) * (size_t)m->nnz, hipMemcpyDeviceToHost));
  }
  std::vector<int32_t> sorted = requested;
  std::sort(sorted.begin(), sorted.end());
  std::vector<double> xd((size_t)ncols, 0.0);
  std::vector<float> scores;
  for (int32_t c : sorted) {
    double nrm1 = 0.0;
    for (ssize_t e = colptr[c]; e < colptr[c + 1]; ++e) {
      xd[(size_t)colind[e]] = colval[e];
      nrm1 += colval[e];
    }
    scores.clear();
    for (int32_t u = 0; u < m->nrows; ++u) {
      bool has = false;
      double r = 0.0;
      for (int64_t e = hp[(size_t)u]; e < hp[(size_t)u + 1]; ++e) {
        if (hi[(size_t)e] == c) has = true;
        r += xd[(size_t)hi[(size_t)e]] * (m->binary ? 1.0 : (double)hv[(size_t)e]);
      }
      if (!has) scores.push_back((float)r);
    }
    const size_t ntop = std::min<size_t>(10, scores.size());
    std::partial_sort(scores.begin(), scores.begin() + (ptrdiff_t)ntop, scores.end(), std::greater<float>());
    float a0 = 0.0f;
    for (size_t j = 0; j < ntop; ++j) a0 += scores[j];
    for (ssize_t e = colptr[c]; e < colptr[c + 1]; ++e) xd[(size_t)colind[e]] = 0.0;
    const size_t i = (size_t)c;
    std::printf("Col: %5d %5zd rs: %3d nits: %4d nnz: %4d rsd: %.2le obj: %.2le ff: %.3lf nrm1: "
                "%.3lf a0s: %.3lf tmr: %.2le\n",
                c, (ssize_t)(hcp[i + 1] - hcp[i]), cs.conv[i], cs.sweeps[i], (int)(colptr[c + 1] - colptr[c]),
                (double)k.err[i], (double)k.obj[i], k.obj[i] != 0 ? (double)k.err[i] / (double)k.obj[i] : 0.0,
                nrm1, ntop ? (double)a0 / (double)ntop : 0.0, 0.0);
  }
  std::fflush(stdout);
}

slimgpu_stats_t solve_stats(slimgpu_matrix* m, const Launch& L, const Entries& E, const Counters& k,
                            const ColumnStats& cs, const std::vector<int32_t>& requested, int64_t tnnz) {
  const Path& p = L.p;
  slimgpu_stats_t st;
  std::memset(&st, 0, sizeof(st));
  st.ncols_solved = (int32_t)requested.size();
  st.kernel = p.kernel;
  st.nwaves = L.nwaves;
  st.lds_bytes = p.use_lds ? (int32_t)p.lds_need : 0;
  st.setup_ms = m->setup_ms;
  st.kernel_ms = E.kernel_ms;
  for (int32_t c : requested) {
    st.G += cs.G[c];
    st.D += cs.D[c];
    st.U += cs.U[c];
    st.sweeps += cs.sweeps[c];
    st.error += k.err[c];
    st.objval += k.obj[c];
  }
  st.nnzW = tnnz;
  st.alg_bytes = m->binary ? 4.0 * st.G + 8.0 * st.D + 4.0 * st.U + 8.0 * st.nnzW
                           : 8.0 * st.G + 12.0 * st.D + 4.0 * st.U + 8.0 * st.nnzW;
  if (p.use_gram || p.use_fgram) {
    st.gram_build_ms = m->G_build_ms;
    st.gram_alloc_ms = m->G_alloc_ms;
    st.gram_sums_ms = m->G_sums_ms;
    st.gram_sums_kernel_ms = m->G_sums_kernel_ms;
    st.gram_pack_ms = m->G_pack_ms;
    m->G_build_ms = m->G_alloc_ms = m->G_sums_ms = m->G_sums_kernel_ms = m->G_pack_ms = 0.0;
  }
  st.gram_rows = k.gram_rows;
  st.gram_bytes = k.gram_bytes;
  return st;
}

}

slim_csr_t* learn_cd(slimgpu_matrix_t* m, const LearnOptions& opt, const slim_csr_t* imodel,
                     int32_t* status, const int32_t* columns, int32_t ncolumns, bool row_view,
                     ResidentIO* rio) {
  const double t_begin = now_ms();
  auto fail = [&](int32_t code) -> slim_csr_t* {
    if (status) *status = code;
    return nullptr;
  };
  if (!m) {
    set_error("SLIMGPU_Learn: null matrix");
    return fail(SLIM_ERROR_INPUT);
  }
  try {
    const WorkList w = work_list(m, opt, columns, ncolumns);
    const std::vector<int32_t>& requested = w.order;
    const int32_t nwork = (int32_t)requested.size();
    (void)hipGetLastError();
    HIP_TRY(hipSetDevice(m->device));
    static std::recursive_mutex device_lock[64];
    std::lock_guard<std::recursive_mutex> solve_guard(device_lock[m->device & 63]);

    const slimgpu_model* warm_dev = rio ? rio->warm : nullptr;
    const bool resident = rio && rio->out;
    const char* trace_env = std::getenv("SLIM_GPU_TRACE");
    Launch L;
    L.G_block = w.G_block;
    L.p = choose_kernel(m, opt, nwork);
    L.p.trace_level = trace_env ? std::atoi(trace_env) : 0;
    if ((L.p.use_gram || L.p.use_fgram) && !m->G_ready) {
      if (const int32_t st = gram_for_solve(m, opt, L.p.trace_level, L.p.use_fgram); st != SLIM_OK) return fail(st);
    }
    finish_path(m, opt, nwork, imodel, warm_dev, L.p);
    prepare_launch(m, opt, requested, imodel, warm_dev, resident, columns == nullptr, L);
    const double t_prep_done = now_ms();

    Entries E = run_launches(m, opt, requested, resident, L);
    const double t_kernel_done = now_ms();
    ColumnStats& cs = g_colstats;
    const Counters k = read_counters(m, L, requested, cs);
    const double t_counters_done = now_ms();
    int64_t tnnz = 0;
    for (int32_t c = 0; c < m->ncols; ++c) tnnz += E.cnt[c];
    slim_csr_t* model = nullptr;
    double t_columns_done = t_counters_done;
    if (resident) {
      *rio->out = assemble_resident_model(m, opt, E, tnnz, L, row_view, &t_columns_done).release();
    } else {
      model = assemble_host_model(m->ncols, E, tnnz, row_view);
      t_columns_done = now_ms();
    }
    if (L.p.trace_level >= 1)
      std::fprintf(stderr, "[slim_gpu trace] host phases: prep %.0f ms, launches + D2H %.0f ms (kernel %.0f, D2H of "
                   "%lld entries %.0f), counters %.0f ms, columns %.0f ms, row view %.0f ms\n",
                   t_prep_done - t_begin, t_kernel_done - t_prep_done, E.kernel_ms, (long long)E.total, E.d2h_ms,
                   t_counters_done - t_kernel_done, t_columns_done - t_counters_done, now_ms() - t_columns_done);
    if ((opt.dbglvl & SLIM_DBG_PROGRESS) && model) print_progress(m, model, requested, cs, k);

    slimgpu_stats_t st = solve_stats(m, L, E, k, cs, requested, tnnz);
    st.gather_ms = now_ms() - t_kernel_done;
    if (!opt.build_G) m->last_order = requested;
    st.total_ms = now_ms() - t_begin;
    g_stats = st;
    if (opt.dbglvl & SLIM_DBG_INFO)
      std::printf("Done estimation: loss: %.5le, fit: %.5le, ffrac: %.3lf,  #nzs: %zd\n", st.objval,
                  st.error, st.objval != 0 ? st.error / st.objval : 0.0, (ssize_t)tnnz);
    if (status) *status = SLIM_OK;
    return model;
  } catch (const Refusal& r) {
    set_error(r.msg);
    return fail(r.status);
  } catch (const HipFail& e) {
    report(e, "SLIMGPU_Learn");
    return fail(status_of(e));
  } catch (const std::bad_alloc&) {
    set_error("SLIMGPU_Learn: out of host memory");
    return fail(SLIM_ERROR_MEMORY);
  }
}

slimgpu_model* learn_resident(slimgpu_matrix_t* m, const LearnOptions& opt, const slimgpu_model* warm,
                              int32_t* status) {
  if (m && !m->replicas.empty()) {
    set_error("SLIMGPU_LearnResident: a model resident in HBM belongs to one device (ngpus = 1)");
    if (status) *status = SLIM_ERROR_INPUT;
    return nullptr;
  }
  slimgpu_model* out = nullptr;
  ResidentIO rio;
  rio.warm = warm;
  rio.out = &out;
  int32_t st = SLIM_ERROR;
  (void)learn_cd(m, opt, nullptr, &st, nullptr, 0, true, &rio);
  if (status) *status = st;
  if (st != SLIM_OK && out) {
    model_free(out);
    out = nullptr;
  }
  return out;
}

slimgpu_model* model_from_host(slimgpu_matrix_t* m, const slim_csr_t* W, int32_t* status) {
  auto fail = [&](int32_t st, const std::string& why) {
    set_error("SLIMGPU_ModelFromHost: " + why);
    if (status) *status = st;
    return static_cast<slimgpu_model*>(nullptr);
  };
  if (!m || !W || !W->rowptr || W->nrows < 0 || W->ncols < 0)
    return fail(SLIM_ERROR_INPUT, "bad arguments (a staged matrix, a model handle with a row view)");
  if (!m->replicas.empty()) return fail(SLIM_ERROR_INPUT, "a model resident in HBM belongs to one device (ngpus = 1)");
  const int32_t n = std::max(W->nrows, W->ncols);
  const int64_t nnz = W->rowptr[W->nrows];
  if (W->rowptr[0] != 0) return fail(SLIM_ERROR_INPUT, "the row pointer does not start at 0");
  for (int32_t r = 0; r < W->nrows; ++r)
    if (W->rowptr[r + 1] < W->rowptr[r]) return fail(SLIM_ERROR_INPUT, "the row pointer descends");
  if (nnz > 0 && (!W->rowind || !W->rowval)) return fail(SLIM_ERROR_INPUT, "the model has no values");
  for (int64_t j = 0; j < nnz; ++j)
    if (W->rowind[j] < 0 || W->rowind[j] >= n) return fail(SLIM_ERROR_INPUT, "an item id outside the model");
  try {
    (void)hipGetLastError();
    HIP_TRY(hipSetDevice(m->device));
    hipStream_t stream = m->stream;
    std::unique_ptr<slimgpu_model> dm(new slimgpu_model());
    dm->device = m->device;
    dm->n = n;
    dm->nnz = nnz;
    std::vector<int64_t> h_ptr((size_t)n + 1, nnz);
    for (int32_t r = 0; r <= W->nrows; ++r) h_ptr[(size_t)r] = W->rowptr[r];
    dm->d_rowptr = DeviceBuffer<int64_t>((size_t)n + 1);
    dm->d_rowind = DeviceBuffer<int32_t>((size_t)std::max<int64_t>(nnz, 1));
    dm->d_rowval = DeviceBuffer<float>((size_t)std::max<int64_t>(nnz, 1));
    HIP_TRY(hipMemcpyAsync(dm->d_rowptr.get(), h_ptr.data(), sizeof(int64_t) * ((size_t)n + 1), hipMemcpyHostToDevice,
                           stream));
    if (nnz > 0) {
      HIP_TRY(hipMemcpyAsync(dm->d_rowind.get(), W->rowind, sizeof(int32_t) * (size_t)nnz, hipMemcpyHostToDevice, stream));
      HIP_TRY(hipMemcpyAsync(dm->d_rowval.get(), W->rowval, sizeof(float) * (size_t)nnz, hipMemcpyHostToDevice, stream));
    }
    int32_t* d_facts = m->ws_misc.reserve(16);
    int32_t facts[2] = {0, 0};
    HIP_TRY(hipMemsetAsync(d_facts, 0, sizeof(facts), stream));
    queue_row_facts(stream, m->num_cus, n, dm->d_rowptr.get(), dm->d_rowind.get(), d_facts);
    HIP_TRY(hipMemcpyAsync(facts, d_facts, sizeof(facts), hipMemcpyDeviceToHost, stream));
    HIP_TRY(hipStreamSynchronize(stream));
    if (facts[1] != 0) return fail(SLIM_ERROR_INPUT, "the item ids of a model row do not ascend strictly");
    dm->max_row = facts[0];
    dm->rows_sorted = true;
    transpose_on_device(m, n, nnz, dm->d_rowptr.get(), dm->d_rowind.get(), dm->d_rowval.get(), dm->d_colptr,
                        dm->d_colind, dm->d_colval);
    HIP_TRY(hipStreamSynchronize(stream));
    if (status) *status = SLIM_OK;
    return dm.release();
  } catch (const HipFail& e) {
    report(e, "SLIMGPU_ModelFromHost");
    if (status) *status = status_of(e);
    return nullptr;
  } catch (const std::bad_alloc&) {
    return fail(SLIM_ERROR_MEMORY, "out of host memory");
  }
}

int32_t model_row_view(const slimgpu_model* w, DeviceRowView* out) {
  if (!w || !w->d_rowptr.get() || !out) {
    set_error("resident model: no row view");
    return SLIM_ERROR_INPUT;
  }
  out->nrows = out->ncols = w->n;
  out->nnz = w->nnz;
  out->max_row = w->max_row;
  out->rows_sorted = w->rows_sorted;
  out->device = w->device;
  out->d_ptr = w->d_rowptr.get();
  out->d_ind = w->d_rowind.get();
  out->d_val = w->d_rowval.get();
  return SLIM_OK;
}

int32_t matrix_csr_view(const slimgpu_matrix_t* m, DeviceCsrView* out) {
  if (!m || !m->d_rowptr || !out) {
    set_error("staged matrix: no CSR on the device");
    return SLIM_ERROR_INPUT;
  }
  out->device = m->device;
  out->stream = m->stream;
  out->num_cus = m->num_cus;
  out->nrows = m->nrows;
  out->ncols = m->ncols;
  out->nnz = m->nnz;
  out->merged = m->merged;
  out->d_ptr = m->d_rowptr;
  out->d_ind = m->d_rowind;
  out->d_val = m->binary ? nullptr : m->d_rowval;
  return SLIM_OK;
}

int64_t model_nnz(const slimgpu_model* w) { return w ? w->nnz : -1; }
int32_t model_ncols(const slimgpu_model* w) { return w ? w->n : -1; }

namespace {
void fetch_now(slimgpu_model* w) {
  const double t0 = now_ms();
  ssize_t *cp = nullptr, *rp = nullptr;
  int32_t *ci = nullptr, *ri = nullptr;
  float *cv = nullptr, *rv = nullptr;
  hipStream_t cs = nullptr;
  try {
    HIP_TRY(hipSetDevice(w->device));
    static_assert(sizeof(ssize_t) == sizeof(int64_t), "offsets travel as they are");
    const size_t n1 = (size_t)w->n + 1, nz = (size_t)std::max<int64_t>(w->nnz, 1);
    cp = static_cast<ssize_t*>(std::malloc(sizeof(ssize_t) * n1));
    rp = static_cast<ssize_t*>(std::malloc(sizeof(ssize_t) * n1));
    ci = static_cast<int32_t*>(std::malloc(sizeof(int32_t) * nz));
    ri = static_cast<int32_t*>(std::malloc(sizeof(int32_t) * nz));
    cv = static_cast<float*>(std::malloc(sizeof(float) * nz));
    rv = static_cast<float*>(std::malloc(sizeof(float) * nz));
    if (!cp || !rp || !ci || !ri || !cv || !rv) throw std::bad_alloc();
    HIP_TRY(hipStreamCreateWithFlags(&cs, hipStreamNonBlocking));
    HIP_TRY(hipMemcpyAsync(cp, w->d_colptr.get(), sizeof(int64_t) * n1, hipMemcpyDeviceToHost, cs));
    HIP_TRY(hipMemcpyAsync(rp, w->d_rowptr.get(), sizeof(int64_t) * n1, hipMemcpyDeviceToHost, cs));
    if (w->nnz > 0) {
      HIP_TRY(hipMemcpyAsync(ci, w->d_colind.get(), sizeof(int32_t) * (size_t)w->nnz, hipMemcpyDeviceToHost, cs));
      HIP_TRY(hipMemcpyAsync(cv, w->d_colval.get(), sizeof(float) * (size_t)w->nnz, hipMemcpyDeviceToHost, cs));
      HIP_TRY(hipMemcpyAsync(ri, w->d_rowind.get(), sizeof(int32_t) * (size_t)w->nnz, hipMemcpyDeviceToHost, cs));
      HIP_TRY(hipMemcpyAsync(rv, w->d_rowval.get(), sizeof(float) * (size_t)w->nnz, hipMemcpyDeviceToHost, cs));
    }
    HIP_TRY(hipStreamSynchronize(cs));
    (void)hipStreamDestroy(cs);
    cs = nullptr;
    slim_csr_t* hm = model_from_columns(w->n, cp, ci, cv, false);
    if (!hm) throw std::bad_alloc();
    hm->rowptr = rp;
    hm->rowind = ri;
    hm->rowval = rv;
    w->fetched = hm;
    w->fetch_status = SLIM_OK;
  } catch (const HipFail& e) {
    w->fetch_error = "SLIMGPU_ModelFetch: " + e.where + ": " + hipGetErrorString(e.code);
    w->fetch_status = SLIM_ERROR;
  } catch (const std::bad_alloc&) {
    w->fetch_error = "SLIMGPU_ModelFetch: out of host memory";
    w->fetch_status = SLIM_ERROR_MEMORY;
  }
  if (w->fetch_status != SLIM_OK) {
    if (cs) (void)hipStreamDestroy(cs);
    std::free(cp); std::free(rp); std::free(ci); std::free(ri); std::free(cv); std::free(rv);
  }
  w->fetch_ms = now_ms() - t0;
}
}

int32_t model_fetch_begin(slimgpu_model* w) {
  if (!w || !w->d_rowptr.get()) {
    set_error("SLIMGPU_ModelFetchBegin: null model");
    return SLIM_ERROR_INPUT;
  }
  if (w->fetch_begun) return SLIM_OK;
  w->fetch_begun = true;
  w->fetched = nullptr;
  w->fetch_status = SLIM_OK;
  try {
    w->fetcher = std::thread(fetch_now, w);
  } catch (const std::system_error&) {
    w->fetch_begun = false;
  }
  return SLIM_OK;
}

slim_csr_t* model_fetch(slimgpu_model* w, int32_t* status, double* ms) {
  if (!w || !w->d_rowptr.get()) {
    set_error("SLIMGPU_ModelFetch: null model");
    if (status) *status = SLIM_ERROR_INPUT;
    return nullptr;
  }
  if (w->fetch_begun) {
    if (w->fetcher.joinable()) w->fetcher.join();
    w->fetch_begun = false;
  } else {
    fetch_now(w);
  }
  slim_csr_t* hm = w->fetched;
  w->fetched = nullptr;
  if (w->fetch_status != SLIM_OK) set_error(w->fetch_error);
  if (status) *status = w->fetch_status;
  if (ms) *ms = w->fetch_ms;
  return hm;
}

void model_free(slimgpu_model* w) {
  if (!w) return;
  if (w->fetcher.joinable()) w->fetcher.join();
  if (w->fetched) csr_free(w->fetched);
  delete w;
}

int32_t gram_build_rows(slimgpu_matrix_t* m, int32_t row_begin, int32_t row_end) {
  if (!m || row_begin < 0 || row_end > m->ncols || row_begin > row_end) {
    set_error("SLIMGPU_MatrixGramBuildRows: rows outside [0, ncols)");
    return SLIM_ERROR_INPUT;
  }
  try {
    HIP_TRY(hipSetDevice(m->device));
    const size_t G_bytes = sizeof(float) * (size_t)m->ncols * (size_t)gram_ld(m->ncols);
    const bool fresh = m->G_ready || m->ws_G.bytes() < G_bytes;
    if (fresh) {
      size_t free_b = 0, total_b = 0;
      HIP_TRY(hipMemGetInfo(&free_b, &total_b));
      if (G_bytes + (size_t(8) << 30) > free_b + m->ws_G.bytes() + m->ws_gram.bytes()) {
        set_error("SLIMGPU_MatrixGramBuildRows: G = R^T R (4 ncols^2 bytes) does not fit the free HBM");
        return SLIM_ERROR_MEMORY;
      }
      m->G_ready = false;
      m->Gp_ready = false;
      m->Gp_tried = false;
    }
    LearnOptions bo;
    bo.G_rows_begin = row_begin;
    bo.G_rows_end = row_end;
    return build_gram(m, bo, fresh);
  } catch (const HipFail& e) {
    report(e, "SLIMGPU_MatrixGramBuildRows");
    return status_of(e);
  }
}

int32_t gram_view(slimgpu_matrix_t* m, void** dptr, int64_t* ld, int32_t* nrows) {
  if (!m || !m->ws_G.get() || m->G_ld <= 0) {
    set_error("SLIMGPU_MatrixGramView: no G on this handle (SLIMGPU_MatrixGramBuildRows first)");
    return SLIM_ERROR_INPUT;
  }
  if (dptr) *dptr = m->ws_G.get();
  if (ld) *ld = m->G_ld;
  if (nrows) *nrows = m->ncols;
  return SLIM_OK;
}

int32_t gram_commit(slimgpu_matrix_t* m) {
  if (!m || !m->ws_G.get() || m->G_ld <= 0) {
    set_error("SLIMGPU_MatrixGramCommit: no G on this handle");
    return SLIM_ERROR_INPUT;
  }
  try {
    HIP_TRY(hipSetDevice(m->device));
    HIP_TRY(hipStreamSynchronize(m->stream));
    m->G_ready = true;
    m->Gp_ready = false;
    m->Gp_tried = false;
    m->Gf_dropped = false;
    (void)pack_gram(m);
    drop_float_gram(m);
    return SLIM_OK;
  } catch (const HipFail& e) {
    report(e, "SLIMGPU_MatrixGramCommit");
    return status_of(e);
  }
}

int32_t gram_planes(slimgpu_matrix_t* m, slimgpu_gram_planes_t* out) {
  if (!m || !out || !m->Gp_ready) {
    set_error("SLIMGPU_MatrixGramPlanes: no byte planes on this handle (no G committed, or a G that could not be packed)");
    return SLIM_ERROR_INPUT;
// ... 20 lines not shown
```

Measured before the change: 2272.

## Compact kept coefficients before output, gather columns on device, lean binary sort

The kernel's output phase now builds a compacted list of kept column ids while counting nonzeros, so it iterates only over nonzeros instead of rescanning all ncols. The per-entry error sum is stored per block and reduced afterwards with a broadcast loop. Separately, host-bound models are gathered into contiguous columns on the device before D2H, and binary matrices use a narrower 32-bit payload sort that skips the key copy and unpack kernel. These cut redundant column scans and host-side assembly work, at the cost of extra per-block scratch memory and a serial broadcast loop in the error reduction.

```diff
diff --git a/slim_amd/csrc/cd_gramr.hpp b/slim_amd/csrc/cd_gramr.hpp
--- a/slim_amd/csrc/cd_gramr.hpp
+++ b/slim_amd/csrc/cd_gramr.hpp
@@ -169,6 +169,8 @@
 #endif
   float4* const gl4 = reinterpret_cast<float4*>(g_lds);
   const int64_t* __restrict__ colptr = A.colptr;
+  double* const out_sum = reinterpret_cast<double*>(S.out_list + (int64_t)blockIdx.x * 12 * S.ncols_pad);
+  int* const out_ids = reinterpret_cast<int*>(out_sum + S.ncols_pad);
 
   GramrRegs<KRA> gr;
 
@@ -553,12 +555,13 @@
       __builtin_amdgcn_global_load_lds(P.meta + i_n, hb + 256, 16, 0, 0);
       hw ^= 1;
     };
-    int ib = 0, wpos = 0, nz = 0;
+    int ib = 0, nz = 0;
     unsigned long long off = 0;
     bool fits = false;
     unsigned long long Uu = 0;
 #if SLIM_GRAMR_PROF
     unsigned long long pt_fetch = 0, pt_dec = 0, pt_apply = 0;
+    unsigned long long pt_out0 = 0;
     pt_first_v = 0;
     pt_export_v = 0;
 #define SLIM_PT(acc) { const unsigned long long now_ = __builtin_readcyclecounter(); acc += now_ - pt_mark; pt_mark = now_; }
@@ -572,7 +575,6 @@
       uint4 mrow = make_uint4(0u, 0u, 0u, 0u);
       float xi = kInactive;
       bool part = false, keep = false;
-      uint64_t mkeep = 0;
       if (phase == 1) {
         i = i_n;
         __builtin_amdgcn_s_waitcnt(0 | (7 << 4) | (15 << 8));
@@ -593,18 +595,9 @@
         header_a(p0 + 128);
         want = part;
       } else if (phase == 2) {
-        i = ib + lane;
-        xi = i < ncols ? x[i] : kInactive;
-        const bool act = tile_active(xi);
-        keep = act && fabsf(xi) > kEps;
-        if (act && wave == 0)
-          s_reg[lane] += 0.5 * (double)l2 * (double)xi * (double)xi + (double)l1 * (double)fabsf(xi);
-        mkeep = __ballot(keep);
-        if (mkeep == 0) {
-          ib += 64;
-          if (ib >= ncols) break;
-          continue;
-        }
+        keep = ib + lane < nz;
+        i = keep ? out_ids[ib + lane] : 0;
+        xi = keep ? x[i] : kInactive;
         r = keep ? (int)(P.meta[i].x & 0x1FFFFu) : 0;
         want = keep;
       }
@@ -612,6 +605,10 @@
       pt_mark = __builtin_readcyclecounter();
 #endif
       const float g0 = fetch_g(want, r);
+#if SLIM_GRAMR_PROF
+      if (phase == 2) pt_mark = __builtin_readcyclecounter();
+      else
+#endif
       SLIM_PT(pt_fetch)
       float gi = g0;
       uint64_t pend = 0;
@@ -736,19 +733,18 @@
             if (j1) aty = fmaf(256.0f, (float)phi0[r], aty);
             if (j2) aty = fmaf(65536.0f, (float)ph20[r], aty);
           }
-          if (wave == 0) s_e2[lane] += (double)xi * ((double)aty + (double)g0);
+          if (wave == 0) out_sum[ib + lane] = (double)aty + (double)g0;
 #else
-          if (wave == 0) s_e2[lane] += (double)xi * ((double)arow[i] + (double)g0);
+          if (wave == 0) out_sum[ib + lane] = (double)arow[i] + (double)g0;
 #endif
           if (fits && wave == 0) {
-            const int64_t dst = (int64_t)off + wpos + __popcll(mkeep & ((1ull << lane) - 1ull));
+            const int64_t dst = (int64_t)off + ib + lane;
             S.out_ind[dst] = i;
             S.out_val[dst] = xi;
           }
         }
-        wpos += __popcll(mkeep);
         ib += 64;
-        if (ib >= ncols) break;
+        if (ib >= nz) break;
         continue;
       }
       bool sweep = false;
@@ -773,12 +769,29 @@
         header_a(64);
         continue;
       }
+#if SLIM_GRAMR_PROF
+      pt_out0 = __builtin_readcyclecounter();
+#endif
       if (wave == 0) {
         int cnt = 0;
-        for (int jb = 0; jb < ncols; jb += 64) {
-          const int j = jb + lane;
-          const float xv = j < ncols ? x[j] : kInactive;
-          cnt += __popcll(__ballot(tile_active(xv) && fabsf(xv) > kEps));
+        constexpr int CB = 4;
+        for (int jb = 0; jb < ncols; jb += 64 * CB) {
+          float xv[CB];
+#pragma unroll
+          for (int u = 0; u < CB; ++u) {
+            const int j = jb + 64 * u + lane;
+            xv[u] = j < ncols ? x[j] : kInactive;
+          }
+#pragma unroll
+          for (int u = 0; u < CB; ++u) {
+            const float xj = xv[u];
+            const bool act = tile_active(xj);
+            const bool kp = act && fabsf(xj) > kEps;
+            if (act) s_reg[lane] += 0.5 * (double)l2 * (double)xj * (double)xj + (double)l1 * (double)fabsf(xj);
+            const uint64_t mk = __ballot(kp);
+            if (kp) out_ids[cnt + __popcll(mk & ((1ull << lane) - 1ull))] = jb + 64 * u + lane;
+            cnt += __popcll(mk);
+          }
         }
         if (lane == 0) {
           s_off = atomicAdd(S.out_cursor, (unsigned long long)cnt);
@@ -791,9 +804,11 @@
       fits = (int64_t)(off + (unsigned long long)nz) <= S.out_cap;
       phase = 2;
       ib = 0;
-      wpos = 0;
-      if (ncols <= 0) break;
-    }
+      if (nz <= 0) break;
+    }
+#if SLIM_GRAMR_PROF
+    const unsigned long long pt_out = pt_out0 ? __builtin_readcyclecounter() - pt_out0 : 0ull;
+#endif
     if (kCarry && S.g_save != nullptr) {
       float4* __restrict__ gs = reinterpret_cast<float4*>(S.g_save + (int64_t)item * S.g_stride);
       static_for<KRA>([&](auto kc) __attribute__((always_inline)) {
@@ -809,7 +824,23 @@
         for (int j = 0; j < 4; ++j) gs[((KRA + k) * NT + tid) * 4 + j] = gl4[(k * 4 + j) * NT + tid];
     }
     if (wave == 0) {
-      double e2 = s_e2[lane], reg = s_reg[lane];
+      __builtin_amdgcn_s_waitcnt(0 | (7 << 4) | (15 << 8));
+      asm volatile("" ::: "memory");
+      double e2 = s_e2[lane];
+      for (int c0 = 0; c0 < nz; c0 += 64) {
+        const bool have = c0 + lane < nz;
+        const int id = have ? out_ids[c0 + lane] : 0;
+        const double sm = have ? out_sum[c0 + lane] : 0.0;
+        const float xk = have ? x[id] : 0.0f;
+        const int n = nz - c0 < 64 ? nz - c0 : 64;
+        for (int b = 0; b < n; ++b) {
+          const int id_b = lane_bcast(id, b);
+          const double sm_b = __hiloint2double(lane_bcast(__double2hiint(sm), b), lane_bcast(__double2loint(sm), b));
+          const float x_b = lane_bcast(xk, b);
+          if (lane == (id_b & 63)) e2 = __builtin_fma((double)x_b, sm_b, e2);
+        }
+      }
+      double reg = s_reg[lane];
       for (int o = 32; o > 0; o >>= 1) {
         e2 += __shfl_xor(e2, o);
         reg += __shfl_xor(reg, o);
@@ -828,6 +859,7 @@
         S.st_B[item] = (int64_t)pt_apply;
         S.st_G[item] = (int)(pt_first_v >> 8);
         S.st_na[item] = (int)(pt_export_v >> 8);
+        S.st_conv[item] = (int)(pt_out >> 8);
 #else
         S.st_D[item] = (int64_t)s_D * (int64_t)(conv ? niters : maxit);
         S.st_U[item] = (int64_t)Uu;
diff --git a/slim_amd/csrc/cd_wave.hpp b/slim_amd/csrc/cd_wave.hpp
--- a/slim_amd/csrc/cd_wave.hpp
+++ b/slim_amd/csrc/cd_wave.hpp
@@ -96,6 +96,7 @@
   int64_t* st_B;
   float* st_err;
   float* st_obj;
+  char* out_list;
 };
 
 constexpr float kEps = 1e-7f;
diff --git a/slim_amd/csrc/engine.hip b/slim_amd/csrc/engine.hip
--- a/slim_amd/csrc/engine.hip
+++ b/slim_amd/csrc/engine.hip
@@ -99,6 +99,7 @@
   DeviceBuffer<uint32_t> ws_tkeys[2];
   DeviceBuffer<uint64_t> ws_tpay[2];
   DeviceBuffer<uint8_t> ws_ttmp;
+  DeviceBuffer<char> ws_outlist;
 
   ~slimgpu_matrix() {
     (void)hipSetDevice(device);
@@ -235,11 +236,15 @@
 constexpr int kBadColumn = 2;
 constexpr int kDupEntry = 4;
 
+inline __device__ uint32_t user_of(uint64_t p) { return (uint32_t)(p >> 32); }
+inline __device__ uint32_t user_of(uint32_t p) { return p; }
+
+template <class Pay>
 __global__ void k_pack_rows(int32_t nrows, int32_t ncols, int64_t nnz,
                             const int64_t* __restrict__ rowptr,
                             const int32_t* __restrict__ rowind,
                             const float* __restrict__ rowval, uint32_t* __restrict__ keys,
-                            uint64_t* __restrict__ payload, int32_t* __restrict__ flags) {
+                            Pay* __restrict__ payload, int32_t* __restrict__ flags) {
   const int lane = threadIdx.x & 63;
   const int64_t wave = ((int64_t)blockIdx.x * blockDim.x + threadIdx.x) >> 6;
   const int64_t nwaves = ((int64_t)gridDim.x * blockDim.x) >> 6;
@@ -251,9 +256,13 @@
     }
     for (int64_t k = s + lane; k < e; k += 64) {
       if ((uint32_t)rowind[k] >= (uint32_t)ncols) atomicOr(flags, kBadColumn);
-      keys[k] = (uint32_t)rowind[k];
-      const uint32_t bits = rowval ? __float_as_uint(rowval[k]) : 0x3F800000u;
-      payload[k] = ((uint64_t)(uint32_t)u << 32) | bits;
+      if constexpr (sizeof(Pay) == 8) {
+        keys[k] = (uint32_t)rowind[k];
+        const uint32_t bits = rowval ? __float_as_uint(rowval[k]) : 0x3F800000u;
+        payload[k] = ((uint64_t)(uint32_t)u << 32) | bits;
+      } else {
+        payload[k] = (uint32_t)u;
+      }
     }
   }
 }
@@ -268,11 +277,12 @@
   }
 }
 
+template <class Pay>
 __global__ void k_check_dups(int64_t nnz, const uint32_t* __restrict__ keys,
-                             const uint64_t* __restrict__ payload, int32_t* __restrict__ flags) {
+                             const Pay* __restrict__ payload, int32_t* __restrict__ flags) {
   for (int64_t k = (int64_t)blockIdx.x * blockDim.x + threadIdx.x + 1; k < nnz;
        k += (int64_t)gridDim.x * blockDim.x)
-    if (keys[k] == keys[k - 1] && (payload[k] >> 32) == (payload[k - 1] >> 32))
+    if (keys[k] == keys[k - 1] && user_of(payload[k]) == user_of(payload[k - 1]))
       atomicOr(flags, kDupEntry);
 }
 
@@ -383,21 +393,24 @@
   HIP_TRY(hipStreamCreateWithFlags(&m->stream, hipStreamNonBlocking));
 }
 
+template <class Pay>
 struct SortBufs {
-  uint32_t *keys_in, *keys_out;
-  uint64_t *pay_in, *pay_out;
+  const uint32_t* keys_in;
+  uint32_t* keys_out;
+  Pay *pay_in, *pay_out;
 };
 
+template <class Pay>
 void pack_entries(slimgpu_matrix* m, int32_t n, int32_t ncols, int64_t nnz, const int64_t* ptr,
-                  const int32_t* ind, const float* val, const SortBufs& b, int32_t* flags) {
-  hipLaunchKernelGGL(k_pack_rows, dim3(grid_for((int64_t)n * 64, 256, m->num_cus * 16)), dim3(256), 0,
-                     m->stream, n, ncols, nnz, ptr, ind, val, b.keys_in, b.pay_in, flags);
+                  const int32_t* ind, const float* val, uint32_t* keys, const SortBufs<Pay>& b, int32_t* flags) {
+  hipLaunchKernelGGL(k_pack_rows<Pay>, dim3(grid_for((int64_t)n * 64, 256, m->num_cus * 16)), dim3(256), 0,
+                     m->stream, n, ncols, nnz, ptr, ind, val, keys, b.pay_in, flags);
   HIP_TRY(hipGetLastError());
 }
 
-template <class TmpFor>
-void sort_entries(slimgpu_matrix* m, int32_t ncols, int64_t nnz, const SortBufs& b, TmpFor&& tmp_for,
-                  int32_t* dups, int64_t* o_ptr, int32_t* o_ind, float* o_val) {
+template <class Pay, class TmpFor>
+void sort_entries(slimgpu_matrix* m, int32_t ncols, int64_t nnz, const SortBufs<Pay>& b, TmpFor&& tmp_for,
+                  int32_t* dups, int64_t* o_ptr, int32_t* o_ind, float* o_val, double* t_sorted = nullptr) {
   hipStream_t st = m->stream;
   const int cap = m->num_cus * 16;
   unsigned bits = 1;
@@ -408,55 +421,106 @@
   void* tmp = tmp_for(tmp_bytes ? tmp_bytes : 1);
   HIP_TRY(rocprim::radix_sort_pairs(tmp, tmp_bytes, b.keys_in, b.keys_out, b.pay_in, b.pay_out,
                                     (size_t)nnz, 0u, bits, st));
+  if (t_sorted) {
+    HIP_TRY(hipStreamSynchronize(st));
+    *t_sorted = now_ms();
+  }
   if (dups) {
-    hipLaunchKernelGGL(k_check_dups, dim3(grid_for(nnz, 256, cap)), dim3(256), 0, st, nnz,
+    hipLaunchKernelGGL(k_check_dups<Pay>, dim3(grid_for(nnz, 256, cap)), dim3(256), 0, st, nnz,
                        b.keys_out, b.pay_out, dups);
     HIP_TRY(hipGetLastError());
   }
-  hipLaunchKernelGGL(k_unpack_cols, dim3(grid_for(nnz, 256, cap)), dim3(256), 0, st, nnz,
-                     b.pay_out, o_ind, o_val);
-  HIP_TRY(hipGetLastError());
+  if constexpr (sizeof(Pay) == 8) {
+    hipLaunchKernelGGL(k_unpack_cols, dim3(grid_for(nnz, 256, cap)), dim3(256), 0, st, nnz,
+                       b.pay_out, o_ind, o_val);
+    HIP_TRY(hipGetLastError());
+  }
   hipLaunchKernelGGL(k_col_offsets, dim3(grid_for(nnz + 1, 256, cap)), dim3(256), 0, st, nnz,
                      ncols, b.keys_out, o_ptr);
   HIP_TRY(hipGetLastError());
 }
 
+struct StageTimes {
+  bool on = false;
+  double alloc = 0, pack = 0, sort = 0, checks = 0, release = 0, scalars = 0;
+  size_t tmp_bytes = 0;
+};
+
+template <class Pay>
+void sort_rows_to_columns(slimgpu_matrix* m, StageTimes& T) {
+  constexpr bool kWide = sizeof(Pay) == 8;
+  hipStream_t st = m->stream;
+  const int64_t nnz = m->nnz;
+  double t0 = now_ms();
+  {
+    DeviceBuffer<uint32_t> keys_in, keys_out((size_t)nnz);
+    DeviceBuffer<Pay> pay_in((size_t)nnz), pay_out;
+    if (kWide) {
+      keys_in = DeviceBuffer<uint32_t>((size_t)nnz);
+      pay_out = DeviceBuffer<Pay>((size_t)nnz);
+    }
+    const SortBufs<Pay> b{kWide ? keys_in.get() : reinterpret_cast<const uint32_t*>(m->d_rowind), keys_out.get(),
+                          pay_in.get(), kWide ? pay_out.get() : reinterpret_cast<Pay*>(m->d_colind.get())};
+    DeviceBuffer<int32_t> d_flags(1);
+    T.alloc += now_ms() - t0;
+    t0 = now_ms();
+    HIP_TRY(hipMemsetAsync(d_flags.get(), 0, sizeof(int32_t), st));
+    pack_entries(m, m->nrows, m->ncols, nnz, m->d_rowptr, m->d_rowind, m->d_rowval, keys_in.get(), b, d_flags.get());
+    int32_t h_flags = 0;
+    HIP_TRY(hipMemcpyAsync(&h_flags, d_flags.get(), sizeof(int32_t), hipMemcpyDeviceToHost, st));
+    HIP_TRY(hipStreamSynchronize(st));
+    T.pack = now_ms() - t0;
+    if (h_flags)
+      throw InputError{h_flags & kBadRowptr
+                           ? "rowptr is not a non-decreasing offset array ending at nnz"
+                           : "item id outside [0, ncols)"};
+    t0 = now_ms();
+    double t_sorted = t0;
+    DeviceBuffer<uint8_t> tmp;
+    sort_entries(m, m->ncols, nnz, b,
+                 [&](size_t bytes) {
+                   T.tmp_bytes = bytes;
+                   return (tmp = DeviceBuffer<uint8_t>(bytes)).get();
+                 },
+                 d_flags.get(), m->d_colptr.get(), m->d_colind.get(), m->d_colval.get(), T.on ? &t_sorted : nullptr);
+    HIP_TRY(hipMemcpyAsync(&h_flags, d_flags.get(), sizeof(int32_t), hipMemcpyDeviceToHost, st));
+    HIP_TRY(hipStreamSynchronize(st));
+    T.sort = t_sorted - t0;
+    T.checks = now_ms() - t_sorted;
+    if (h_flags & kDupEntry)
+      throw InputError{"duplicate (user, item) entries in the rating matrix (SLIM_GPU_DUPLICATES=sum "
+                       "merges them while a host matrix is staged)"};
+    t0 = now_ms();
+  }
+  T.release = now_ms() - t0;
+}
+
 void build_column_view(slimgpu_matrix* m) {
   hipStream_t st = m->stream;
   const int64_t nnz = m->nnz;
+  StageTimes T;
+  if (const char* te = std::getenv("SLIM_GPU_TRACE"); te && std::atoi(te) >= 1) T.on = true;
+  double t0 = now_ms();
   m->d_colptr = DeviceBuffer<int64_t>((size_t)m->ncols + 1);
   m->d_colind = DeviceBuffer<int32_t>((size_t)nnz + 64);
   if (!m->binary) m->d_colval = DeviceBuffer<float>((size_t)nnz);
   m->d_cnorm = DeviceBuffer<float>((size_t)m->ncols);
   m->d_csq = DeviceBuffer<float>((size_t)m->ncols);
   DeviceBuffer<int64_t> d_cost((size_t)m->ncols);
-
+  T.alloc = now_ms() - t0;
+
+  bool lean = m->binary;
+  if (const char* e = std::getenv("SLIM_GPU_STAGE_WIDE"); e && std::atoi(e) != 0) lean = false;
   if (nnz > 0) {
     if (nnz > 0xFFFFFFF0ll) throw HipFail{hipErrorInvalidValue, "nnz >= 2^32 not supported"};
-    DeviceBuffer<uint32_t> keys_in((size_t)nnz), keys_out((size_t)nnz);
-    DeviceBuffer<uint64_t> pay_in((size_t)nnz), pay_out((size_t)nnz);
-    const SortBufs b{keys_in.get(), keys_out.get(), pay_in.get(), pay_out.get()};
-    DeviceBuffer<int32_t> d_flags(1);
-    HIP_TRY(hipMemsetAsync(d_flags.get(), 0, sizeof(int32_t), st));
-    pack_entries(m, m->nrows, m->ncols, nnz, m->d_rowptr, m->d_rowind, m->d_rowval, b, d_flags.get());
-    int32_t h_flags = 0;
-    HIP_TRY(hipMemcpyAsync(&h_flags, d_flags.get(), sizeof(int32_t), hipMemcpyDeviceToHost, st));
-    HIP_TRY(hipStreamSynchronize(st));
-    if (h_flags)
-      throw InputError{h_flags & kBadRowptr
-                           ? "rowptr is not a non-decreasing offset array ending at nnz"
-                           : "item id outside [0, ncols)"};
-    DeviceBuffer<uint8_t> tmp;
-    sort_entries(m, m->ncols, nnz, b, [&](size_t bytes) { return (tmp = DeviceBuffer<uint8_t>(bytes)).get(); },
-                 d_flags.get(), m->d_colptr.get(), m->d_colind.get(), m->d_colval.get());
-    HIP_TRY(hipMemcpyAsync(&h_flags, d_flags.get(), sizeof(int32_t), hipMemcpyDeviceToHost, st));
-    HIP_TRY(hipStreamSynchronize(st));
-    if (h_flags & kDupEntry)
-      throw InputError{"duplicate (user, item) entries in the rating matrix (SLIM_GPU_DUPLICATES=sum "
-                       "merges them while a host matrix is staged)"};
+    if (lean)
+      sort_rows_to_columns<uint32_t>(m, T);
+    else
+      sort_rows_to_columns<uint64_t>(m, T);
   } else {
     HIP_TRY(hipMemsetAsync(m->d_colptr.get(), 0, sizeof(int64_t) * ((size_t)m->ncols + 1), st));
   }
+  t0 = now_ms();
   DeviceBuffer<int32_t> d_inexact(1);
   HIP_TRY(hipMemsetAsync(d_inexact.get(), 0, sizeof(int32_t), st));
   hipLaunchKernelGGL(k_col_scalars, dim3(grid_for((int64_t)m->ncols * 64, 256, m->num_cus * 16)),
@@ -471,6 +535,14 @@
   HIP_TRY(hipStreamSynchronize(st));
   m->exact_gram = (h_inexact & 1) != 0;
   m->nonpositive = (h_inexact & 2) != 0;
+  T.scalars = now_ms() - t0;
+  if (T.on)
+    std::fprintf(stderr, "[slim_gpu trace] staging: %lld entries, %s payload: allocation %.1f ms, pack + checks %.1f ms, "
+                 "sort %.1f ms (%.2f GB of temporaries), duplicates + offsets%s %.1f ms, release %.1f ms, "
+                 "scalars %.1f ms\n",
+                 (long long)nnz, lean ? "32-bit" : "64-bit", T.alloc, T.pack, T.sort,
+                 1e-9 * ((double)T.tmp_bytes + (lean ? 8.0 : 24.0) * (double)nnz), lean ? "" : " + unpack", T.checks,
+                 T.release, T.scalars);
 }
 
 void transpose_on_device(slimgpu_matrix* m, int32_t n, int64_t nnz, const int64_t* d_ptr,
@@ -485,10 +557,11 @@
   }
   if (nnz > 0xFFFFFFF0ll) throw HipFail{hipErrorInvalidValue, "model nnz >= 2^32 not supported"};
   const auto evict = evict_cache(m);
-  const SortBufs b{m->ws_tkeys[0].reserve((size_t)nnz, evict), m->ws_tkeys[1].reserve((size_t)nnz, evict),
-                   m->ws_tpay[0].reserve((size_t)nnz, evict), m->ws_tpay[1].reserve((size_t)nnz, evict)};
+  uint32_t* const keys = m->ws_tkeys[0].reserve((size_t)nnz, evict);
+  const SortBufs<uint64_t> b{keys, m->ws_tkeys[1].reserve((size_t)nnz, evict),
+                             m->ws_tpay[0].reserve((size_t)nnz, evict), m->ws_tpay[1].reserve((size_t)nnz, evict)};
   int32_t* d_flags = m->ws_misc.reserve(16, evict);
-  pack_entries(m, n, n, nnz, d_ptr, d_ind, d_val, b, d_flags);
+  pack_entries(m, n, n, nnz, d_ptr, d_ind, d_val, keys, b, d_flags);
   sort_entries(m, n, nnz, b, [&](size_t bytes) { return m->ws_ttmp.reserve(bytes, evict); }, nullptr,
                o_ptr.get(), o_ind.get(), o_val.get());
 }
@@ -531,10 +604,13 @@
 
 void destroy(slimgpu_matrix* m) {
   if (!m) return;
+  const double t0 = now_ms();
   for (slimgpu_matrix* r : m->replicas) destroy(r);
   (void)hipSetDevice(m->device);
   if (m->stream) (void)hipStreamDestroy(m->stream);
   delete m;
+  if (const char* te = std::getenv("SLIM_GPU_TRACE"); te && std::atoi(te) >= 1)
+    std::fprintf(stderr, "[slim_gpu trace] handle freed in %.1f ms\n", now_ms() - t0);
 }
 
 }
@@ -1475,6 +1551,7 @@
 
 struct Slabs {
   float *slab = nullptr, *xslab = nullptr, *part = nullptr;
+  char* out_list = nullptr;
   int32_t *ulist = nullptr, *nunion = nullptr;
   unsigned long long* mailbox = nullptr;
   size_t mailbox_words = 0;
@@ -1512,6 +1589,7 @@
     const size_t ngroups0 = ((size_t)nwork + 31) / 32;
     s.xslab = m->ws_xslab.reserve((size_t)p.ncols_pad * (size_t)nwaves, evict);
     if (p.gram_v == 0) s.slab = m->ws_slab.reserve((size_t)p.ncols_pad * (size_t)nwaves, evict);
+    if (p.use_gramr) s.out_list = m->ws_outlist.reserve(12 * (size_t)p.ncols_pad * (size_t)nwaves, evict);
     s.ulist = m->ws_ulist.reserve((size_t)p.ncols_pad * ngroups0, evict);
     s.nunion = m->ws_nunion.reserve(ngroups0, evict);
   } else if (p.use_tile) {
@@ -1697,6 +1775,7 @@
   S.nrows_pad = p.nrows_pad;
   S.ncols_pad = p.ncols_pad;
   S.xslab = L.s.xslab;
+  S.out_list = L.s.out_list;
   S.x_stride = (int64_t)t.tile_x;
   S.ulist = L.s.ulist;
   S.u_stride = (int64_t)t.tile_u;
@@ -1927,9 +2006,10 @@
   std::vector<float> val;
   std::vector<ArenaSeg> segs;
   double kernel_ms = 0, d2h_ms = 0;
+  int pieces = 0;
 };
 
-Entries run_launches(slimgpu_matrix* m, const LearnOptions& opt, const std::vector<int32_t>& order, bool resident,
+Entries run_launches(slimgpu_matrix* m, const LearnOptions& opt, const std::vector<int32_t>& order, bool keep_arena,
                      Launch& L) {
   const int32_t ncols = m->ncols;
   hipStream_t stream = m->stream;
@@ -2130,7 +2210,7 @@
     const int64_t used = std::min<int64_t>((int64_t)cursor, L.arena_cap);
     const int64_t base = E.total;
     const double t_d2h = now_ms();
-    if (resident) {
+    if (keep_arena) {
       E.segs.push_back({d_ai, d_av, used, {}, {}});
     } else {
       E.ind.resize((size_t)(base + used));
@@ -2143,6 +2223,7 @@
     }
     E.d2h_ms += now_ms() - t_d2h;
     E.total += used;
+    if (used > 0) ++E.pieces;
 
     std::vector<int32_t> again;
     int64_t need = 0;
@@ -2157,7 +2238,7 @@
     }
     pending.swap(again);
     if (!pending.empty()) L.arena_cap = std::max<int64_t>(L.arena_cap, need + 1024);
-    if (resident && !pending.empty() && used > 0) {
+    if (keep_arena && !pending.empty() && used > 0) {
       ArenaSeg& sg = E.segs.back();
       sg.own_i = DeviceBuffer<int32_t>((size_t)used);
       sg.own_v = DeviceBuffer<float>((size_t)used);
@@ -2233,17 +2314,10 @@
   return model_from_columns(ncols, colptr, colind, colval, row_view);
 }
 
-std::unique_ptr<slimgpu_model> assemble_resident_model(slimgpu_matrix* m, const LearnOptions& opt, Entries& E,
-                                                       int64_t tnnz, Launch& L, bool row_view,
-                                                       double* t_columns_done) {
+void gather_columns_on_device(slimgpu_matrix* m, const Entries& E, int64_t tnnz, const int64_t* h_colptr,
+                              int64_t* d_colptr, int32_t* d_colind, float* d_colval) {
   const int32_t ncols = m->ncols;
   hipStream_t stream = m->stream;
-  std::unique_ptr<slimgpu_model> dm(new slimgpu_model());
-  dm->device = m->device;
-  dm->n = ncols;
-  dm->nnz = tnnz;
-  std::vector<int64_t> h_colptr((size_t)ncols + 1, 0);
-  for (int32_t c = 0; c < ncols; ++c) h_colptr[(size_t)c + 1] = h_colptr[(size_t)c] + E.cnt[(size_t)c];
   const int32_t* src_i = E.segs.empty() ? nullptr : E.segs[0].ind;
   const float* src_v = E.segs.empty() ? nullptr : E.segs[0].val;
   DeviceBuffer<int32_t> cat_i;
@@ -2262,19 +2336,63 @@
     src_i = cat_i.get();
     src_v = cat_v.get();
   }
+  int64_t* d_src = m->ws_off.reserve((size_t)ncols, evict_cache(m));
+  HIP_TRY(hipMemcpyAsync(d_colptr, h_colptr, sizeof(int64_t) * ((size_t)ncols + 1), hipMemcpyHostToDevice, stream));
+  HIP_TRY(hipMemcpyAsync(d_src, E.off.data(), sizeof(int64_t) * (size_t)ncols, hipMemcpyHostToDevice, stream));
+  if (tnnz > 0) {
+    hipLaunchKernelGGL(k_gather_columns, dim3(grid_for((int64_t)ncols * 64, 256, m->num_cus * 16)), dim3(256),
+                       0, stream, ncols, d_colptr, d_src, src_i, src_v, d_colind, d_colval);
+    HIP_TRY(hipGetLastError());
+  }
+  HIP_TRY(hipStreamSynchronize(stream));
+}
+
+slim_csr_t* assemble_host_model_from_arena(slimgpu_matrix* m, const Entries& E, int64_t tnnz, bool row_view,
+                                           double* d2h_ms) {
+  const int32_t ncols = m->ncols;
+  struct Free {
+    void operator()(void* p) const { std::free(p); }
+  };
+  const size_t nz = (size_t)std::max<int64_t>(tnnz, 1);
+  std::unique_ptr<ssize_t, Free> colptr(static_cast<ssize_t*>(std::malloc(sizeof(ssize_t) * ((size_t)ncols + 1))));
+  std::unique_ptr<int32_t, Free> colind(static_cast<int32_t*>(std::malloc(sizeof(int32_t) * nz)));
+  std::unique_ptr<float, Free> colval(static_cast<float*>(std::malloc(sizeof(float) * nz)));
+  if (!colptr || !colind || !colval)
+    throw Refusal{SLIM_ERROR_MEMORY, "SLIMGPU_Learn: out of host memory for the model"};
+  ssize_t* const cp = colptr.get();
+  cp[0] = 0;
+  for (int32_t c = 0; c < ncols; ++c) cp[c + 1] = cp[c] + E.cnt[(size_t)c];
+  if (tnnz > 0) {
+    static_assert(sizeof(ssize_t) == sizeof(int64_t), "LP64 expected");
+    DeviceBuffer<int64_t> d_colptr((size_t)ncols + 1);
+    DeviceBuffer<int32_t> d_colind(nz);
+    DeviceBuffer<float> d_colval(nz);
+    gather_columns_on_device(m, E, tnnz, reinterpret_cast<const int64_t*>(cp), d_colptr.get(), d_colind.get(),
+                             d_colval.get());
+    const double t0 = now_ms();
+    HIP_TRY(hipMemcpyAsync(colind.get(), d_colind.get(), sizeof(int32_t) * (size_t)tnnz, hipMemcpyDeviceToHost, m->stream));
+    HIP_TRY(hipMemcpyAsync(colval.get(), d_colval.get(), sizeof(float) * (size_t)tnnz, hipMemcpyDeviceToHost, m->stream));
+    HIP_TRY(hipStreamSynchronize(m->stream));
+    *d2h_ms += now_ms() - t0;
+  }
+  return model_from_columns(ncols, colptr.release(), colind.release(), colval.release(), row_view);
+}
+
+std::unique_ptr<slimgpu_model> assemble_resident_model(slimgpu_matrix* m, const LearnOptions& opt, Entries& E,
+                                                       int64_t tnnz, Launch& L, bool row_view,
+                                                       double* t_columns_done) {
+  const int32_t ncols = m->ncols;
+  hipStream_t stream = m->stream;
+  std::unique_ptr<slimgpu_model> dm(new slimgpu_model());
+  dm->device = m->device;
+  dm->n = ncols;
+  dm->nnz = tnnz;
+  std::vector<int64_t> h_colptr((size_t)ncols + 1, 0);
+  for (int32_t c = 0; c < ncols; ++c) h_colptr[(size_t)c + 1] = h_colptr[(size_t)c] + E.cnt[(size_t)c];
   dm->d_colptr = DeviceBuffer<int64_t>((size_t)ncols + 1);
   dm->d_colind = DeviceBuffer<int32_t>((size_t)std::max<int64_t>(tnnz, 1));
   dm->d_colval = DeviceBuffer<float>((size_t)std::max<int64_t>(tnnz, 1));
-  int64_t* d_src = m->ws_off.reserve((size_t)ncols, evict_cache(m));
-  HIP_TRY(hipMemcpyAsync(dm->d_colptr.get(), h_colptr.data(), sizeof(int64_t) * ((size_t)ncols + 1),
-                         hipMemcpyHostToDevice, stream));
-  HIP_TRY(hipMemcpyAsync(d_src, E.off.data(), sizeof(int64_t) * (size_t)ncols, hipMemcpyHostToDevice, stream));
-  if (tnnz > 0) {
-    hipLaunchKernelGGL(k_gather_columns, dim3(grid_for((int64_t)ncols * 64, 256, m->num_cus * 16)), dim3(256),
-                       0, stream, ncols, dm->d_colptr.get(), d_src, src_i, src_v, dm->d_colind.get(),
-                       dm->d_colval.get());
-    HIP_TRY(hipGetLastError());
-  }
+  gather_columns_on_device(m, E, tnnz, h_colptr.data(), dm->d_colptr.get(), dm->d_colind.get(), dm->d_colval.get());
   *t_columns_done = now_ms();
   if (row_view) {
     transpose_on_device(m, ncols, tnnz, dm->d_colptr.get(), dm->d_colind.get(), dm->d_colval.get(), dm->d_rowptr,
@@ -2423,7 +2541,10 @@
     prepare_launch(m, opt, requested, imodel, warm_dev, resident, columns == nullptr, L);
     const double t_prep_done = now_ms();
 
-    Entries E = run_launches(m, opt, requested, resident, L);
+    bool host_columns = false;
+    if (const char* e = std::getenv("SLIM_GPU_HOST_COLUMNS")) host_columns = std::atoi(e) != 0;
+    const bool keep_arena = resident || !host_columns;
+    Entries E = run_launches(m, opt, requested, keep_arena, L);
     const double t_kernel_done = now_ms();
     ColumnStats& cs = g_colstats;
     const Counters k = read_counters(m, L, requested, cs);
@@ -2432,17 +2553,26 @@
     for (int32_t c = 0; c < m->ncols; ++c) tnnz += E.cnt[c];
     slim_csr_t* model = nullptr;
     double t_columns_done = t_counters_done;
+    double model_d2h_ms = 0;
     if (resident) {
       *rio->out = assemble_resident_model(m, opt, E, tnnz, L, row_view, &t_columns_done).release();
     } else {
-      model = assemble_host_model(m->ncols, E, tnnz, row_view);
+      const double d2h_before = E.d2h_ms;
+      model = keep_arena ? assemble_host_model_from_arena(m, E, tnnz, row_view, &E.d2h_ms)
+                         : assemble_host_model(m->ncols, E, tnnz, row_view);
       t_columns_done = now_ms();
+      model_d2h_ms = E.d2h_ms - d2h_before;
     }
     if (L.p.trace_level >= 1)
       std::fprintf(stderr, "[slim_gpu trace] host phases: prep %.0f ms, launches + D2H %.0f ms (kernel %.0f, D2H of "
                    "%lld entries %.0f), counters %.0f ms, columns %.0f ms, row view %.0f ms\n",
-                   t_prep_done - t_begin, t_kernel_done - t_prep_done, E.kernel_ms, (long long)E.total, E.d2h_ms,
-                   t_counters_done - t_kernel_done, t_columns_done - t_counters_done, now_ms() - t_columns_done);
+                   t_prep_done - t_begin, t_kernel_done - t_prep_done, E.kernel_ms, (long long)E.total,
+                   E.d2h_ms - model_d2h_ms, t_counters_done - t_kernel_done, t_columns_done - t_counters_done,
+                   now_ms() - t_columns_done);
+    if (L.p.trace_level >= 1 && !resident && !opt.build_G)
+      std::fprintf(stderr, "[slim_gpu trace] model to host: %d arena piece(s), %s, D2H %.1f ms + columns %.1f ms = %.1f ms\n",
+                   E.pieces, keep_arena ? "gathered on the device" : "columns on the host", E.d2h_ms,
+                   (t_columns_done - t_counters_done) - model_d2h_ms, E.d2h_ms + (t_columns_done - t_counters_done) - model_d2h_ms);
     if ((opt.dbglvl & SLIM_DBG_PROGRESS) && model) print_progress(m, model, requested, cs, k);
 
     slimgpu_stats_t st = solve_stats(m, L, E, k, cs, requested, tnnz);
```

Result: slower. 1978 (-12.9%).
